# POSTECH-CVLab/PyTorch-StudioGAN

Hardware: AMD Instinct MI355X
Metric: images/sec (G+D step) BigGAN ImageNet-128 bs256 (higher is better)
Workload: dtype bf16

## Files before the change

include/sgamd.h:

```cpp
#ifndef SGAMD_H
#define SGAMD_H
#include <stdint.h>
#ifdef __cplusplus
extern "C" {
#endif

typedef void* sg_stream_t;

#define SG_DTYPE_F32 0
#define SG_DTYPE_BF16 1
#define SG_DTYPE_F64 2

#define SG_PIX_RELU 1
#define SG_PIX_UPSAMPLE 2
#define SG_PIX_QUAD 4
#define SG_PIX_TRANSPOSED 8
#define SG_EPI_OUT_F32 1
#define SG_EPI_ATOMIC 2
#define SG_EPI_POOL 4
#define SG_EPI_RELU 8
#define SG_EPI_RES_F32 16

const char* sg_last_error(void);
int sg_version(void);
int sg_prof_enable(int on);
int sg_prof_collect(double* out, int nkinds);

typedef struct {
  int dtype;
  int N, Hs, Ws, C, ldx;
  int Ho, Wo, Cout;
  int R, S, stride, pad_h, pad_w;
  int pix_flags, epi_flags;
  float alpha, beta;
  const void* x; const void* w;
  const float* bias; const void* res; const void* mask; void* out; const float* alpha_ptr;
  int ldo, ldr, ldm;
} sg_conv_fwd_desc;
int sg_conv2d_fwd(const sg_conv_fwd_desc* d, sg_stream_t stream);
int sg_set_f32_mode(int mode);
int sg_get_f32_mode(void);
long long sg_f32_split_launches(int mode);
long long sg_ew_vec_launches(void);

typedef struct {
  sg_conv_fwd_desc main;
  const void* x2; const void* w2; const float* bias2;
  int C2, ldx2, x2_up;
  float* stats;
} sg_conv_skip_desc;
int sg_conv2d_fwd_skip_stat_rows(const sg_conv_skip_desc* d);
int sg_conv2d_fwd_skip(const sg_conv_skip_desc* d, sg_stream_t stream);
int sg_conv2d_fwd_skip_ok(const sg_conv_skip_desc* d);
long long sg_conv_rs_launches(void);

typedef struct {
  sg_conv_fwd_desc conv;
  const float* pre; const float* post; const float* noise;
  long long noise_stride;
} sg_modconv_desc;
int sg_modconv2d_fwd(const sg_modconv_desc* d, sg_stream_t stream);
int sg_modconv2d_ok(const sg_modconv_desc* d);
long long sg_modconv_launches(void);
int sg_modconv_dcoef(const float* w, const float* s, float* Q, float* d, int N, int C, int Cout, int RS, sg_stream_t stream);
int sg_modconv_reduce_slabs(int P);
int sg_modconv_reduce(int dtype, const void* a, const void* b, const float* rowsub, long long rowsub_stride, const float* scale, void* out, float* part,
                      float* rowsum, int N, int P, int C, int lda, int ldb, sg_stream_t stream);

#define SG_Q_POOL 0
#define SG_Q_UP 1
typedef struct {
  int dtype, form;
  int N, Hl, Wl;
  int C, ldx, Cout;
  int pix_flags, epi_flags;
  float alpha, beta;
  const void* x; const void* wq;
  const float* bias; const void* res; const void* mask; void* out; const float* alpha_ptr;
  int ldo, ldr, ldm;
  const void* x2; const void* w2q; const float* bias2;
  int C2, ldx2;
  float* stats;
  int x2_norelu;
} sg_convq_desc;
int sg_conv2d_q_stat_rows(const sg_convq_desc* d);
int sg_conv2d_q(const sg_convq_desc* d, sg_stream_t stream);
int sg_conv2d_q_ok(const sg_convq_desc* d);
int sg_quad_pack(int dtype, int mode, const void* src, void* dst, int M, int Cs, sg_stream_t stream);
typedef struct { const void* src; void* dst; int M, Cs, mode, pad_; } sg_quad_item;
int sg_quad_pack_batch(int dtype, const sg_quad_item* items_dev, const sg_quad_item* items_host, int n, sg_stream_t stream);
typedef struct {
  int dtype, form;
  int N, Hl, Wl;
  int C, ldx, x_flags;
  int Cout, ldg;
  float alpha; const float* alpha_ptr;
  const void* x; const void* dy; float* dw; float* dbias;
  float* work; long long work_floats;
  int splits;
} sg_convq_wgrad_desc;
int sg_conv2d_q_wgrad_plan(const sg_convq_wgrad_desc* d, int* splits, long long* work_floats);
int sg_conv2d_q_wgrad(const sg_convq_wgrad_desc* d, sg_stream_t stream);
int sg_prof_collect_ex(double* out, int nkinds);
int sg_prof_collect_tags(double* out, int ntags);

typedef struct {
  int dtype;
  int N;
  int xHs, xWs, C, ldx, x_flags;
  int gHs, gWs, Cout, ldg, g_flags;
  int Ho, Wo;
  int R, S, stride, pad_h, pad_w;
  float alpha;
  const void* x; const void* dy; float* dw;
  const float* alpha_ptr;
  int splits;
// ... 319 lines not shown
```

pytorch-studiogan_amd/_lib.py:

```python
import ctypes as C
import os
import subprocess
import sys

import torch

_HERE = os.path.dirname(os.path.abspath(__file__))
LIB_PATH = os.path.join(_HERE, "libsgamd.so")
if os.environ.get("SG_LIBSGAMD"):
    LIB_PATH = os.path.abspath(os.environ["SG_LIBSGAMD"])
CSRC = os.path.join(_HERE, "csrc")

F32, BF16, F64 = 0, 1, 2
PIX_RELU, PIX_UPSAMPLE, PIX_QUAD, PIX_TRANSPOSED = 1, 2, 4, 8
Q_POOL, Q_UP = 0, 1
EPI_OUT_F32, EPI_ATOMIC, EPI_POOL, EPI_RELU, EPI_RES_F32 = 1, 2, 4, 8, 16

_vp, _i, _f, _ll = C.c_void_p, C.c_int, C.c_float, C.c_longlong


class ConvFwdDesc(C.Structure):
    _fields_ = [("dtype", _i), ("N", _i), ("Hs", _i), ("Ws", _i), ("C", _i), ("ldx", _i), ("Ho", _i), ("Wo", _i), ("Cout", _i),
                ("R", _i), ("S", _i), ("stride", _i), ("pad_h", _i), ("pad_w", _i), ("pix_flags", _i), ("epi_flags", _i),
                ("alpha", _f), ("beta", _f), ("x", _vp), ("w", _vp), ("bias", _vp), ("res", _vp), ("mask", _vp), ("out", _vp),
                ("alpha_ptr", _vp), ("ldo", _i), ("ldr", _i), ("ldm", _i)]


class ConvSkipDesc(C.Structure):
    _fields_ = [("main", ConvFwdDesc), ("x2", _vp), ("w2", _vp), ("bias2", _vp), ("C2", _i), ("ldx2", _i), ("x2_up", _i), ("stats", _vp)]


class ModConvDesc(C.Structure):
    _fields_ = [("conv", ConvFwdDesc), ("pre", _vp), ("post", _vp), ("noise", _vp), ("noise_stride", _ll)]


class ConvWgradDesc(C.Structure):
    _fields_ = [("dtype", _i), ("N", _i), ("xHs", _i), ("xWs", _i), ("C", _i), ("ldx", _i), ("x_flags", _i), ("gHs", _i), ("gWs", _i),
                ("Cout", _i), ("ldg", _i), ("g_flags", _i), ("Ho", _i), ("Wo", _i), ("R", _i), ("S", _i), ("stride", _i),
                ("pad_h", _i), ("pad_w", _i), ("alpha", _f), ("x", _vp), ("dy", _vp), ("dw", _vp), ("alpha_ptr", _vp),
                ("splits", _i), ("no_tr", _i), ("work", _vp), ("work_floats", _ll), ("dbias", _vp)]


class ConvQDesc(C.Structure):
    _fields_ = [("dtype", _i), ("form", _i), ("N", _i), ("Hl", _i), ("Wl", _i), ("C", _i), ("ldx", _i), ("Cout", _i),
                ("pix_flags", _i), ("epi_flags", _i), ("alpha", _f), ("beta", _f), ("x", _vp), ("wq", _vp), ("bias", _vp), ("res", _vp),
                ("mask", _vp), ("out", _vp), ("alpha_ptr", _vp), ("ldo", _i), ("ldr", _i), ("ldm", _i),
                ("x2", _vp), ("w2q", _vp), ("bias2", _vp), ("C2", _i), ("ldx2", _i), ("stats", _vp), ("x2_norelu", _i)]


class ConvQWgradDesc(C.Structure):
    _fields_ = [("dtype", _i), ("form", _i), ("N", _i), ("Hl", _i), ("Wl", _i), ("C", _i), ("ldx", _i), ("x_flags", _i), ("Cout", _i),
                ("ldg", _i), ("alpha", _f), ("alpha_ptr", _vp), ("x", _vp), ("dy", _vp), ("dw", _vp), ("dbias", _vp), ("work", _vp),
                ("work_floats", _ll), ("splits", _i)]


class QuadItem(C.Structure):
    _fields_ = [("src", _vp), ("dst", _vp), ("M", _i), ("Cs", _i), ("mode", _i), ("pad_", _i)]


class LinearItem(C.Structure):
    _fields_ = [("w", _vp), ("y", _vp), ("bias", _vp), ("out", _vp), ("rows", _i), ("K", _i), ("ldy", _i), ("ldo", _i)]


class LinearItemScaled(C.Structure):
    _fields_ = [("w", _vp), ("y", _vp), ("bias", _vp), ("out", _vp), ("rows", _i), ("K", _i), ("ldy", _i), ("ldo", _i),
                ("wscale", _f), ("bscale", _f), ("oscale", _f), ("pad_", _i)]


class GemmDesc(C.Structure):
    _fields_ = [("dtype", _i), ("p_form", _i), ("q_form", _i), ("I", _i), ("J", _i), ("K", _i), ("batch", _i),
                ("p", _vp), ("p_bstride", _ll), ("ldp", _i), ("q", _vp), ("q_bstride", _ll), ("ldq", _i),
                ("out", _vp), ("out_bstride", _ll), ("ldo", _i), ("bias", _vp), ("res", _vp), ("res_bstride", _ll), ("ldr", _i),
                ("beta", _f), ("alpha", _f), ("alpha_ptr", _vp), ("epi_flags", _i), ("splits", _i), ("no_tr", _i)]


class SnLayer(C.Structure):
    _fields_ = [("w", _vp), ("u", _vp), ("v", _vp), ("sigma", _vp), ("u_snap", _vp), ("v_snap", _vp), ("w_fwd", _vp), ("w_dgrad", _vp),
                ("w_f32", _vp), ("rows", _i), ("cols", _i), ("Cin", _i), ("RS", _i), ("do_power_iter", _i), ("apply_sn", _i),
                ("rows_pad", _i), ("work_off", _ll), ("trans", _i), ("dgrad_noflip", _i), ("Cin_pad", _i)]

# ... 1 lines not shown
class SnBwdLayer(C.Structure):
    _fields_ = [("dwt", _vp), ("w", _vp), ("u", _vp), ("v", _vp), ("sigma", _vp), ("dw", _vp), ("rows", _i), ("cols", _i),
                ("Cin", _i), ("RS", _i), ("natural", _i), ("apply_sn", _i), ("trans", _i), ("Cin_pad", _i)]


class AugDesc(C.Structure):
    _fields_ = [("N", _i), ("C", _i), ("H", _i), ("W", _i), ("ops", _i), ("cut_h", _i), ("cut_w", _i), ("max_t", _i), ("color", _vp), ("geom", _vp)]


AUG_BRIGHTNESS, AUG_SATURATION, AUG_CONTRAST, AUG_FLIP, AUG_TRANSLATE, AUG_TRANSLATE_REFLECT, AUG_CUTOUT = 1, 2, 4, 8, 16, 32, 64

_lib = None


def build(force=False, verbose=False):
    cmd = ["make", "-C", CSRC, "-j", str(max(2, os.cpu_count() or 2))]
    if force:
        subprocess.run(["make", "-C", CSRC, "clean"], check=True, stdout=subprocess.DEVNULL)
    res = subprocess.run(cmd, stdout=subprocess.PIPE, stderr=subprocess.STDOUT, text=True)
    if verbose or res.returncode != 0:
        sys.stderr.write(res.stdout)
    if res.returncode != 0:
        raise RuntimeError("building libsgamd.so failed")
    return LIB_PATH


_PROTOS = {
    "sg_prof_enable": [_i],
    "sg_prof_collect": [C.POINTER(C.c_double), _i],
    "sg_conv2d_fwd": [C.POINTER(ConvFwdDesc), _vp],
    "sg_conv2d_fwd_skip": [C.POINTER(ConvSkipDesc), _vp],
    "sg_conv2d_fwd_skip_ok": [C.POINTER(ConvSkipDesc)],
    "sg_conv_rs_launches": [],
    "sg_modconv2d_fwd": [C.POINTER(ModConvDesc), _vp],
    "sg_modconv2d_ok": [C.POINTER(ModConvDesc)],
    "sg_modconv_launches": [],
    "sg_modconv_dcoef": [_vp, _vp, _vp, _vp, _i, _i, _i, _i, _vp],
    "sg_modconv_reduce_slabs": [_i],
    "sg_modconv_reduce": [_i, _vp, _vp, _vp, _ll, _vp, _vp, _vp, _vp, _i, _i, _i, _i, _i, _vp],
    "sg_conv2d_q": [C.POINTER(ConvQDesc), _vp],
    "sg_conv2d_q_ok": [C.POINTER(ConvQDesc)],
    "sg_conv2d_q_stat_rows": [C.POINTER(ConvQDesc)],
    "sg_conv2d_fwd_skip_stat_rows": [C.POINTER(ConvSkipDesc)],
    "sg_bn_stats_from_tiles": [_vp, _i, _i, _vp, _vp],
    "sg_quad_pack": [_i, _i, _vp, _vp, _i, _i, _vp],
    "sg_quad_pack_batch": [_i, _vp, C.POINTER(QuadItem), _i, _vp],
    "sg_linear_group": [_vp, C.POINTER(LinearItem), _i, _i, _vp],
    "sg_linear_group_scaled": [_vp, C.POINTER(LinearItemScaled), _i, _i, _vp],
    "sg_linear_group_scaled_launches": [],
    "sg_conv2d_q_wgrad_plan": [C.POINTER(ConvQWgradDesc), C.POINTER(_i), C.POINTER(_ll)],
    "sg_conv2d_q_wgrad": [C.POINTER(ConvQWgradDesc), _vp],
    "sg_prof_collect_ex": [C.POINTER(C.c_double), _i],
    "sg_prof_collect_tags": [C.POINTER(C.c_double), _i],
    "sg_conv2d_wgrad": [C.POINTER(ConvWgradDesc), _vp],
    "sg_conv2d_wgrad_plan": [C.POINTER(ConvWgradDesc), C.POINTER(_i), C.POINTER(_ll)],
    "sg_conv2d_wgrad_fuses_bias": [C.POINTER(ConvWgradDesc)],
    "sg_gemm": [C.POINTER(GemmDesc), _vp],
    "sg_nchw_to_nhwc": [_i, _vp, _vp, _i, _i, _i, _i, _i, _vp],
    "sg_nhwc_to_nchw": [_i, _vp, _vp, _i, _i, _i, _i, _i, _i, _vp],
    "sg_nchw_grad_to_nhwc": [_i, _vp, _vp, _vp, _i, _i, _i, _i, _i, _i, _vp],
    "sg_avgpool2_fwd": [_i, _vp, _vp, _i, _i, _i, _i, _vp],
    "sg_avgpool2_bwd": [_i, _vp, _vp, _i, _i, _i, _i, _vp],
    "sg_maxpool2_fwd": [_i, _vp, _i, _vp, _i, _vp, _i, _i, _i, _i, _vp],
    "sg_maxpool2_bwd": [_i, _vp, _i, _vp, _vp, _i, _i, _i, _i, _i, _vp],
    "sg_softmax_rows": [_i, _vp, _vp, _ll, _i, _vp],
    "sg_softmax_rows_bwd": [_i, _vp, _vp, _vp, _ll, _i, _vp],
# ... 141 lines not shown
    "sg_tanh_bwd2": [_vp, _vp, _vp, _vp, _ll, _vp],
    "sg_clamp_flat": [_vp, _ll, _f, _f, _vp],
    "sg_select_rows": [_vp, _vp, _vp, _vp, _i, _ll, _vp],
    "sg_sign_count": [_vp, _i, _vp, _vp],
    "sg_reflect_pad2d_fwd": [_vp, _vp, _i, _i, _i, _i, _i, _i, _i, _vp],
    "sg_reflect_pad2d_bwd": [_vp, _vp, _i, _i, _i, _i, _i, _i, _i, _vp],
    "sg_affine_sample_fwd": [_vp, _vp, _vp, _i, _i, _i, _i, _i, _i, _vp],
    "sg_affine_sample_bwd": [_vp, _vp, _vp, _i, _i, _i, _i, _i, _i, _vp],
    "sg_color_affine": [_vp, _vp, _vp, _i, _i, _i, _i, _vp],
    "sg_fir_reflect": [_vp, _vp, _vp, _i, _i, _i, _i, _i, _i, _i, _vp],
    "sg_ada_noise_cutout": [_vp, _vp, _vp, _vp, _vp, _i, _i, _i, _i, _vp],
}


def exported_symbols():
    return sorted(list(_PROTOS.keys()) + ["sg_last_error", "sg_version"])


def lib():
    global _lib
    if _lib is None:
        if not os.path.exists(LIB_PATH):
            raise RuntimeError(
                f"{LIB_PATH} is missing: run `python -c 'import __graft_entry__ as g; g.build()'` (make -C {CSRC}). "
                "There is no CPU/eager fallback on the product path.")
        l = C.CDLL(LIB_PATH)
        l.sg_last_error.restype = C.c_char_p
        l.sg_version.restype = _i
        for name, args in _PROTOS.items():
            fn = getattr(l, name)
            fn.argtypes = args
            fn.restype = _i
        l.sg_conv_rs_launches.restype = _ll
        l.sg_modconv_launches.restype = _ll
        l.sg_tok_gemm_launches.restype = _ll
        l.sg_mha_launches.restype = _ll
        l.sg_f32_split_launches.restype = _ll
        l.sg_ew_vec_launches.restype = _ll
        l.sg_bn_path_launches.restype = _ll
        l.sg_linear_group_scaled_launches.restype = _ll
        l.sg_fir_bias_act_launches.restype = _ll
        l.sg_act_fir_launches.restype = _ll
        l.sg_mbstd_launches.restype = _ll
        f32_mode = {"bf16x3": 3, "bf16x6": 6}.get(os.environ.get("SG_F32_MODE", "exact"), 0)
        if f32_mode:
            l.sg_set_f32_mode(f32_mode)
        _lib = l
    return _lib


def check(rc, name=""):
    if rc != 0:
        raise RuntimeError(f"{name}: {lib().sg_last_error().decode()} (rc={rc})")


_STATE_WRITERS = frozenset(("sg_adam_ema", "sg_ema_lerp", "sg_allreduce_flat", "sg_clamp_flat", "sg_allgather_flat"))
write_epoch = [0]


def call(name, *args):
    if name in _STATE_WRITERS:
        write_epoch[0] += 1
    rc = getattr(lib(), name)(*args)
    if rc != 0:
        raise RuntimeError(f"{name}: {lib().sg_last_error().decode()} (rc={rc})")

# ... 33 lines not shown
```

pytorch-studiogan_amd/backbones/big_resnet.py:

```python
import torch
import torch.nn as nn

from .. import functional as F
from .. import ops
from ..bank import get_bank
from .heads import build_heads, apply_heads


def _dtype(mixed_precision):
    return torch.bfloat16 if mixed_precision else torch.float32


def _need_graph(module, *inputs):
    if not torch.is_grad_enabled():
        return False
    for t in inputs:
        if torch.is_tensor(t) and t.requires_grad:
            return True
    return any(p.requires_grad for p in module.parameters())


class GenBlock(nn.Module):
    def __init__(self, in_channels, out_channels, g_cond_mtd, affine_input_dim, MODULES):
        super().__init__()
# ... 119 lines not shown
        nxt = bank.boundaries(self.blocks) if bank.exchange is not None else None
        with ops.bump_batches_tracked(self):
            for bi, blocklist in enumerate(self.blocks):
                for block in blocklist:
                    if isinstance(block, ops.SelfAttention):
                        act = block.forward_nhwc(act, slot)
                    else:
                        act = block.forward_nhwc(act, affines[counter], slot)
                        counter += 1
                if nxt is not None:
                    act = bank.mark(act, nxt[bi])
                act = ops.block_boundary(self, bi, act)
            act = self.bn4.forward_nhwc(act, relu=True)
        act = self.conv2d5.forward_nhwc(act, slot)
        return F.NhwcToNchwFn.apply(act, True, 3)


class DiscOptBlock(nn.Module):
    def __init__(self, in_channels, out_channels, apply_d_sn, MODULES):
        super().__init__()
        self.apply_d_sn = apply_d_sn
        self.conv2d0 = MODULES.d_conv2d(in_channels=in_channels, out_channels=out_channels, kernel_size=1, stride=1, padding=0)
        self.conv2d1 = MODULES.d_conv2d(in_channels=in_channels, out_channels=out_channels, kernel_size=3, stride=1, padding=1)
        self.conv2d2 = MODULES.d_conv2d(in_channels=out_channels, out_channels=out_channels, kernel_size=3, stride=1, padding=1)
        if not apply_d_sn:
            self.bn0 = MODULES.d_bn(in_features=in_channels)
            self.bn1 = MODULES.d_bn(in_features=out_channels)
        self.activation = MODULES.d_act_fn
        self.average_pooling = nn.AvgPool2d(2)
        self.cpad = 8 if (apply_d_sn and in_channels < 8) else 0
        if self.cpad:
            self.conv2d1._sg_cin_pad = self.conv2d0._sg_cin_pad = self.cpad

    def forward_nhwc(self, x, slot):
        h = self.conv2d1.forward_nhwc(x, slot)
        if not self.apply_d_sn:
            h = self.bn1.forward_nhwc(h, relu=True)
            h = self.conv2d2.forward_nhwc(h, slot, out_pool=True)
        else:
            if self.cpad == 8 and h.dtype == torch.bfloat16 and not x.requires_grad:
                return ops.conv_skip_nhwc(self.conv2d2, self.conv2d0, h, x, slot, in_relu=True, out_pool=True, skip_relu=False)
            h = self.conv2d2.forward_nhwc(h, slot, in_relu=True, out_pool=True)
        x0 = F.AvgPool2Fn.apply(x)
        if not self.apply_d_sn:
            x0 = self.bn0.forward_nhwc(x0)
        return self.conv2d0.forward_nhwc(x0, slot, res=h)


class DiscBlock(nn.Module):
    def __init__(self, in_channels, out_channels, apply_d_sn, MODULES, downsample=True):
        super().__init__()
        self.apply_d_sn = apply_d_sn
        self.downsample = downsample
        self.activation = MODULES.d_act_fn
        self.ch_mismatch = in_channels != out_channels
        if self.ch_mismatch or downsample:
            self.conv2d0 = MODULES.d_conv2d(in_channels=in_channels, out_channels=out_channels, kernel_size=1, stride=1, padding=0)
            if not apply_d_sn:
                self.bn0 = MODULES.d_bn(in_features=in_channels)
        self.conv2d1 = MODULES.d_conv2d(in_channels=in_channels, out_channels=out_channels, kernel_size=3, stride=1, padding=1)
        self.conv2d2 = MODULES.d_conv2d(in_channels=out_channels, out_channels=out_channels, kernel_size=3, stride=1, padding=1)
        if not apply_d_sn:
            self.bn1 = MODULES.d_bn(in_features=in_channels)
            self.bn2 = MODULES.d_bn(in_features=out_channels)
        self.average_pooling = nn.AvgPool2d(2)

    def forward_nhwc(self, x, slot):
        if self.apply_d_sn:
            if self.downsample or self.ch_mismatch:
                link = F.GradLink()
                h = self.conv2d1.forward_nhwc(x, slot, in_relu=True, link=link)
                return ops.conv_skip_nhwc(self.conv2d2, self.conv2d0, h, x, slot, in_relu=True, out_pool=self.downsample, link=link)
            h = self.conv2d1.forward_nhwc(x, slot, in_relu=True)
            h = self.conv2d2.forward_nhwc(h, slot, in_relu=True, out_pool=False)
            return F.AddReluFn.apply(h, x)
        h = self.bn1.forward_nhwc(x, relu=True)
        h = self.conv2d1.forward_nhwc(h, slot)
        h = self.bn2.forward_nhwc(h, relu=True)
        h = self.conv2d2.forward_nhwc(h, slot, out_pool=self.downsample)
        if self.downsample or self.ch_mismatch:
            x0 = self.bn0.forward_nhwc(x)
            return self.conv2d0.forward_nhwc(x0, slot, out_pool=self.downsample, res=h)
        return F.AddFn.apply(h, x)


class Discriminator(nn.Module):
    def __init__(self, img_size, d_conv_dim, apply_d_sn, apply_attn, attn_d_loc, d_cond_mtd, aux_cls_type, d_embed_dim, normalize_d_embed,
                 num_classes, d_init, d_depth, mixed_precision, MODULES, MODEL):
        super().__init__()
        d_in_dims_collection = {
            "32": [3] + [d_conv_dim * 2, d_conv_dim * 2, d_conv_dim * 2],
            "64": [3] + [d_conv_dim, d_conv_dim * 2, d_conv_dim * 4, d_conv_dim * 8],
            "128": [3] + [d_conv_dim, d_conv_dim * 2, d_conv_dim * 4, d_conv_dim * 8, d_conv_dim * 16],
            "256": [3] + [d_conv_dim, d_conv_dim * 2, d_conv_dim * 4, d_conv_dim * 8, d_conv_dim * 8, d_conv_dim * 16],
            "512": [3] + [d_conv_dim, d_conv_dim, d_conv_dim * 2, d_conv_dim * 4, d_conv_dim * 8, d_conv_dim * 8, d_conv_dim * 16]
        }
        d_out_dims_collection = {
            "32": [d_conv_dim * 2, d_conv_dim * 2, d_conv_dim * 2, d_conv_dim * 2],
            "64": [d_conv_dim, d_conv_dim * 2, d_conv_dim * 4, d_conv_dim * 8, d_conv_dim * 16],
            "128": [d_conv_dim, d_conv_dim * 2, d_conv_dim * 4, d_conv_dim * 8, d_conv_dim * 16, d_conv_dim * 16],
            "256": [d_conv_dim, d_conv_dim * 2, d_conv_dim * 4, d_conv_dim * 8, d_conv_dim * 8, d_conv_dim * 16, d_conv_dim * 16],
            "512": [d_conv_dim, d_conv_dim, d_conv_dim * 2, d_conv_dim * 4, d_conv_dim * 8, d_conv_dim * 8, d_conv_dim * 16, d_conv_dim * 16]
        }
        d_down = {
            "32": [True, True, False, False],
            "64": [True, True, True, True, False],
            "128": [True, True, True, True, True, False],
            "256": [True, True, True, True, True, True, False],
            "512": [True, True, True, True, True, True, True, False]
        }
        self.d_cond_mtd = d_cond_mtd
        self.aux_cls_type = aux_cls_type
        self.normalize_d_embed = normalize_d_embed
        self.num_classes = num_classes
        self.mixed_precision = mixed_precision
        self.in_dims = d_in_dims_collection[str(img_size)]
        self.out_dims = d_out_dims_collection[str(img_size)]
        self.MODEL = MODEL
        down = d_down[str(img_size)]

        blocks = []
        for index in range(len(self.in_dims)):
            if index == 0:
                blocks += [[DiscOptBlock(in_channels=self.in_dims[index], out_channels=self.out_dims[index], apply_d_sn=apply_d_sn, MODULES=MODULES)]]
            else:
                blocks += [[DiscBlock(in_channels=self.in_dims[index], out_channels=self.out_dims[index], apply_d_sn=apply_d_sn,
                                      MODULES=MODULES, downsample=down[index])]]
            if index + 1 in attn_d_loc and apply_attn:
                blocks += [[ops.SelfAttention(self.out_dims[index], is_generator=False, MODULES=MODULES)]]
        self.blocks = nn.ModuleList([nn.ModuleList(block) for block in blocks])
        self.activation = MODULES.d_act_fn
        build_heads(self, MODULES, self.out_dims[-1], d_cond_mtd, aux_cls_type, d_embed_dim, num_classes, MODEL)
        if d_init:
            ops.init_weights(self.modules, d_init)
        ops.adopt(self, _dtype(mixed_precision))

    def forward(self, x, label, eval=False, adc_fake=False):
        dtype = self.compute_dtype
        bank = get_bank(self, dtype)
        slot = bank.begin_forward(_need_graph(self, x))
        h = ops.to_nhwc(x, dtype, self.blocks[0][0].cpad)
        nxt = bank.boundaries(self.blocks) if bank.exchange is not None else None
        for bi, blocklist in enumerate(self.blocks):
            for block in blocklist:
                h = block.forward_nhwc(h, slot)
            if nxt is not None:
                h = bank.mark(h, nxt[bi])
            h = ops.block_boundary(self, bi, h)
        hw = h.shape[1] * h.shape[2]
        h = F.ReluSumFn.apply(h)
        return apply_heads(self, h, label, slot, adc_fake, hw=hw)
```

pytorch-studiogan_amd/csrc/common.h:

```cpp
#pragma once
#include <hip/hip_runtime.h>
#include <stdint.h>
#include <type_traits>

typedef uint16_t bf16_t;
typedef __attribute__((ext_vector_type(4))) uint32_t u32x4;
typedef __attribute__((ext_vector_type(2))) uint32_t u32x2;
typedef __attribute__((ext_vector_type(4))) float f32x4;
typedef __attribute__((ext_vector_type(16))) float f32x16;
typedef __attribute__((ext_vector_type(8))) __bf16 bf16x8_t;
typedef __attribute__((ext_vector_type(4))) short s16x4;
typedef __attribute__((ext_vector_type(8))) short s16x8;

#define SG_PRIO_UP() __builtin_amdgcn_s_setprio(1)
#define SG_PRIO_DOWN() __builtin_amdgcn_s_setprio(0)

#define SG_DTYPE_F32 0
#define SG_DTYPE_BF16 1

__device__ __forceinline__ float bf2f(bf16_t v) { return __uint_as_float(((uint32_t)v) << 16); }
__device__ __forceinline__ bf16_t f2bf(float f) {
  uint32_t u = __float_as_uint(f);
  if ((u & 0x7fffffffu) > 0x7f800000u) return (bf16_t)((u >> 16) | 0x40u);
  u += 0x7fffu + ((u >> 16) & 1u);
  return (bf16_t)(u >> 16);
}

typedef __bf16 sg_bf16x2_t __attribute__((ext_vector_type(2)));
typedef float sg_f32x2_t __attribute__((ext_vector_type(2)));
__device__ __forceinline__ uint32_t pack2bf(float a, float b) {
  sg_f32x2_t v = {a, b};
  return __builtin_bit_cast(uint32_t, __builtin_convertvector(v, sg_bf16x2_t));
}

template <typename T> __device__ __forceinline__ float to_f(T v);
template <> __device__ __forceinline__ float to_f<float>(float v) { return v; }
template <> __device__ __forceinline__ float to_f<bf16_t>(bf16_t v) { return bf2f(v); }
template <typename T> __device__ __forceinline__ T from_f(float v);
template <> __device__ __forceinline__ float from_f<float>(float v) { return v; }
template <> __device__ __forceinline__ bf16_t from_f<bf16_t>(float v) { return f2bf(v); }

template <typename T> struct ET;
template <> struct ET<float> { static constexpr int VEC = 4, BK = 16; };
template <> struct ET<bf16_t> { static constexpr int VEC = 8, BK = 32; };

__device__ __forceinline__ u32x4 zero16() { u32x4 z = {0u, 0u, 0u, 0u}; return z; }

template <typename T> __device__ __forceinline__ void unpack16(u32x4 v, float* o);
template <> __device__ __forceinline__ void unpack16<float>(u32x4 v, float* o) {
#pragma unroll
  for (int i = 0; i < 4; i++) o[i] = __uint_as_float(v[i]);
}
template <> __device__ __forceinline__ void unpack16<bf16_t>(u32x4 v, float* o) {
#pragma unroll
  for (int i = 0; i < 4; i++) { o[2 * i] = __uint_as_float(v[i] << 16); o[2 * i + 1] = __uint_as_float(v[i] & 0xffff0000u); }
}
template <typename T> __device__ __forceinline__ u32x4 pack16(const float* o);
template <> __device__ __forceinline__ u32x4 pack16<float>(const float* o) {
  u32x4 v;
#pragma unroll
  for (int i = 0; i < 4; i++) v[i] = __float_as_uint(o[i]);
  return v;
}
template <> __device__ __forceinline__ u32x4 pack16<bf16_t>(const float* o) {
  u32x4 v;
#pragma unroll
  for (int i = 0; i < 4; i++) v[i] = (uint32_t)f2bf(o[2 * i]) | ((uint32_t)f2bf(o[2 * i + 1]) << 16);
  return v;
}
template <typename T, int V> using vec_t = std::conditional_t<V == 1, T, u32x4>;
// ... 117 lines not shown
```

pytorch-studiogan_amd/csrc/conv.hip:

```cpp
#include <type_traits>
#include "conv_common.h"
#include "conv_v2.h"

int g_sg_f32_mode = 0;
long long g_sg_f32_split_launches[2] = {0, 0};
extern "C" int sg_set_f32_mode(int mode) {
  SG_CHECK(mode == 0 || mode == 3 || mode == 6, "sg_set_f32_mode: 0 (exact fp32 MFMA), 3 (bf16x3 split) or 6 (bf16x6 split)");
  g_sg_f32_mode = mode;
  return 0;
}
extern "C" int sg_get_f32_mode() { return g_sg_f32_mode; }
extern "C" long long sg_f32_split_launches(int mode) {
  if (mode != 3 && mode != 6) return -1;
  return __atomic_load_n(&g_sg_f32_split_launches[mode == 6], __ATOMIC_RELAXED);
}

template <typename T, bool FAST>
static void conv_fwd_launch(const sg_conv_fwd_desc* d, const Epilogue<T>& e, int I, int J, int K, int pflags, hipStream_t st) {
  typedef StridedKC<T, FAST> LP;
  typedef ConvPixKC<T, FAST> LQ;
  LP lp;
  lp.base = (const T*)d->w; lp.bstride = 0; lp.ld = K; lp.rows = I; lp.K = K;
  lp.vec_ok = (K % ET<T>::VEC == 0) && aligned16(d->w);
  LQ lq;
  fill_geom<T>(lq.g, d->x, d->N, d->Hs, d->Ws, d->C, d->ldx, d->Ho, d->Wo, d->R, d->S, d->stride, d->pad_h, d->pad_w, pflags);
  lq.rows = J; lq.K = K;
  if constexpr (sizeof(T) == 4 && FAST) {
    const int mode = g_sg_f32_mode;
    if (mode == 3) { sg_f32_split_count(3); return conv_fwd_tiles<T, LP, LQ, 3>(lp, lq, e, I, J, K, st); }
    if (mode == 6) { sg_f32_split_count(6); return conv_fwd_tiles<T, LP, LQ, 6>(lp, lq, e, I, J, K, st); }
  }
  conv_fwd_tiles<T, LP, LQ, 0>(lp, lq, e, I, J, K, st);
}

static bool conv_fwd_v2_try(const ConvFwdProblem& pb, hipStream_t st) {
  const sg_conv_fwd_desc* d = pb.d;
  const int I = pb.I, J = pb.J, K = pb.K, pflags = pb.pflags;
  const char mode = env_mode("SG_CONV_V2");
  const bool force = mode == 'f';
  if (mode == '0' || (pflags & SG_PIX_TRANSPOSED)) return false;
  if (d->stride != 1 && (d->stride != 2 || (pflags & (SG_PIX_UPSAMPLE | SG_PIX_QUAD)))) return false;
  if (d->C % 8 || d->ldx % 8 || d->R * d->S > 25 || J < 256) return false;
  if (pb.xbytes >= (1ll << 31) || pb.wbytes >= (1ll << 30)) return false;
  if (!aligned16(d->x) || !aligned16(d->w)) return false;
// ... 41 lines not shown
  const int J = (int)Jll;
  int pflags = d->pix_flags;
  if (d->epi_flags & SG_EPI_POOL) {
    SG_CHECK((d->Ho % 2 == 0) && (d->Wo % 2 == 0), "sg_conv2d_fwd: pooled output needs even Ho, Wo");
    pflags |= SG_PIX_QUAD;
  } else {
    pflags &= ~SG_PIX_QUAD;
  }
  const bool w_vec = (K % ET<T>::VEC == 0) && aligned16(d->w);
  const bool x_vec = (d->C % ET<T>::VEC == 0) && (d->ldx % ET<T>::VEC == 0) && aligned16(d->x);
  const Epilogue<T> e = make_epilogue<T>(d, I, J);
  const int prof = sg_prof_begin(st, 2.0 * (double)I * (double)J * (double)K, 0);
  int eng = SG_ENG_CONV_GEMM;
  if constexpr (std::is_same_v<T, bf16_t>) {
    if (w_vec && x_vec) {
      const ConvFwdProblem pb = conv_fwd_problem(d, e, I, J, K, pflags);
      if (sg_conv_fwd_sk_try(pb, st)) eng = SG_ENG_CONV_SK;
      else if (sg_conv_fwd_rs_try(pb, st)) eng = SG_ENG_CONV_RS;
      else if (sg_conv_fwd_v4_try(pb, st)) eng = SG_ENG_CONV_V4;
      else if (sg_conv_fwd_v3_try(pb, st)) eng = SG_ENG_CONV_V3;
      else if (conv_fwd_v2_try(pb, st)) eng = SG_ENG_CONV_V2;
    }
  }
  if (eng == SG_ENG_CONV_GEMM) {
    if (w_vec && x_vec) conv_fwd_launch<T, true>(d, e, I, J, K, pflags, st);
    else conv_fwd_launch<T, false>(d, e, I, J, K, pflags, st);
  }
  {
    const double es = sizeof(T), jout = (d->epi_flags & SG_EPI_POOL) ? (double)J / 4.0 : (double)J;
    const double b = es * ((double)d->N * d->Hs * d->Ws * d->C + (double)I * K + jout * I * (1.0 + (d->mask ? 1.0 : 0.0) + (d->res ? 1.0 : 0.0)));
    sg_prof_tag(prof, eng, b);
  }
  sg_prof_end(st, prof);
  SG_LAUNCH_CHECK();
  return 0;
}

static int conv_fwd_skip(const sg_conv_skip_desc* sk, hipStream_t st, bool dry) {
  const sg_conv_fwd_desc* d = &sk->main;
  if (d->dtype != SG_DTYPE_BF16 || d->R != 3 || d->S != 3 || d->stride != 1 || (d->pix_flags & (SG_PIX_UPSAMPLE | SG_PIX_TRANSPOSED))) return 0;
  const int K = 9 * d->C, I = d->Cout;
  const long long Jll = (long long)d->N * d->Ho * d->Wo;
  if (Jll >= (1ll << 31) || (long long)d->N * d->Hs * d->Ws * d->ldx >= (1ll << 31)) return 0;
  const int J = (int)Jll;
  int pflags = d->pix_flags;
  if (d->epi_flags & SG_EPI_POOL) { if ((d->Ho & 1) || (d->Wo & 1)) return 0; pflags |= SG_PIX_QUAD; } else pflags &= ~SG_PIX_QUAD;
  const ConvFwdProblem pb = conv_fwd_problem(d, make_epilogue<bf16_t>(d, I, J), I, J, K, pflags);
  if (dry) return sg_conv_fwd_v4_skip_try(pb, sk, st, true) ? 1 : 0;
  const int prof = sg_prof_begin(st, 2.0 * (double)I * (double)J * ((double)K + (double)sk->C2), 0);
  const bool ok = sg_conv_fwd_v4_skip_try(pb, sk, st, false);
  {
    const double jout = (d->epi_flags & SG_EPI_POOL) ? (double)J / 4.0 : (double)J;
    const double x2 = (double)d->N * (sk->x2_up ? (d->Ho / 2) * (d->Wo / 2) : d->Ho * d->Wo) * sk->C2;
    sg_prof_tag(prof, SG_ENG_CONV_V4_SKIP, 2.0 * ((double)d->N * d->Hs * d->Ws * d->C + x2 + (double)I * (K + sk->C2) + jout * I));
  }
  sg_prof_end(st, prof);
  return ok ? 1 : 0;
}
extern "C" int sg_conv2d_fwd_skip_stat_rows(const sg_conv_skip_desc* d) {
  if (!d) return 0;
  const long long J = (long long)d->main.N * d->main.Ho * d->main.Wo;
  return (int)((J + 255) / 256);
}
extern "C" int sg_conv2d_fwd_skip_ok(const sg_conv_skip_desc* d) {
  if (!d || !d->main.x || !d->main.w || !d->main.out || !d->x2 || !d->w2) return 0;
  return conv_fwd_skip(d, nullptr, true);
}
extern "C" int sg_conv2d_fwd_skip(const sg_conv_skip_desc* d, sg_stream_t stream) {
  SG_CHECK(d && d->main.x && d->main.w && d->main.out && d->x2 && d->w2, "sg_conv2d_fwd_skip: null pointer");
  SG_CHECK(conv_fwd_skip(d, (hipStream_t)stream, false) == 1, "sg_conv2d_fwd_skip: problem not eligible for the fused kernel (ask sg_conv2d_fwd_skip_ok first)");
  SG_LAUNCH_CHECK();
  return 0;
}

extern "C" int sg_conv2d_fwd(const sg_conv_fwd_desc* d, sg_stream_t stream) {
  SG_CHECK(d && d->x && d->w && d->out, "sg_conv2d_fwd: null pointer");
  SG_CHECK(d->N > 0 && d->C > 0 && d->Cout > 0 && d->R > 0 && d->S > 0 && d->stride > 0, "sg_conv2d_fwd: bad shape");
  SG_CHECK(!(d->epi_flags & SG_EPI_ATOMIC), "sg_conv2d_fwd: atomic epilogue not supported");
  if (d->dtype == SG_DTYPE_F32) return conv_fwd_t<float>(d, (hipStream_t)stream);
  if (d->dtype == SG_DTYPE_BF16) return conv_fwd_t<bf16_t>(d, (hipStream_t)stream);
  sg_set_error("sg_conv2d_fwd: bad dtype");
  return -1;
}
```

pytorch-studiogan_amd/csrc/conv_common.h:

```cpp
#pragma once
#include <stdlib.h>
#include "gemm_core.h"
#include "../../include/sgamd.h"

static inline int ilog2_exact(int v) {
  if (v <= 0 || (v & (v - 1))) return -1;
  int s = 0;
  while ((1 << s) < v) s++;
  return s;
}
static inline bool aligned16(const void* p) { return (((uintptr_t)p) & 15) == 0; }

template <typename T>
static void fill_geom(PixGeom<T>& g, const void* x, int N, int Hs, int Ws, int C, int ldx, int Ho, int Wo, int R, int S,
                      int stride, int pad_h, int pad_w, int flags) {
  g.x = (const T*)x; g.N = N; g.Hs = Hs; g.Ws = Ws;
  const int up = (flags & SG_PIX_UPSAMPLE) ? 2 : 1;
  g.Hin = Hs * up; g.Win = Ws * up; g.C = C; g.ldx = ldx; g.Ho = Ho; g.Wo = Wo;
  g.R = R; g.S = S; g.stride = stride; g.pad_h = pad_h; g.pad_w = pad_w; g.flags = flags;
  g.vec_ok = (C % ET<T>::VEC == 0) && (ldx % ET<T>::VEC == 0) && aligned16(x);
  g.wshift = ilog2_exact(Wo); g.hshift = ilog2_exact(Ho);
}

static inline char env_mode(const char* name) { const char* m = getenv(name); return m ? m[0] : 0; }

static inline long long bf16_extent(long long npix, int ld, int C) { return ((npix - 1) * ld + C) * 2; }

template <typename D> static inline bool is_3x3_s1_p1(const D* d) { return d->R == 3 && d->S == 3 && d->stride == 1 && d->pad_h == 1 && d->pad_w == 1; }

static inline int cout_blocks(int Cout) { return Cout % 96 == 0 ? 3 : Cout % 64 == 0 ? 2 : 0; }

static const int kCoutTiles[3] = {192, 128, 96};
static inline int cout_tile_search(int I, int tj, int& best_tiles) {
  int best = 0;
  best_tiles = 0;
  for (int c = 0; c < 3; c++) {
    if (I % kCoutTiles[c]) continue;
    const int tiles = (I / kCoutTiles[c]) * tj;
    if (tiles >= 512) { best = kCoutTiles[c]; best_tiles = tiles; break; }
    if (tiles > best_tiles) { best = kCoutTiles[c]; best_tiles = tiles; }
  }
  return best;
}

template <typename T, class LP, class LQ, int SPLIT, class EPI = Epilogue<T>>
static void conv_fwd_tiles(const LP& lp, const LQ& lq, const EPI& e, int I, int J, int K, hipStream_t st) {
  if (I <= 32) sg_launch_gemm<T, LP, LQ, 32, 256, 1, 4, true, SPLIT, EPI>(lp, lq, e, I, J, K, 1, 1, st);
  else if (I % 128 != 0 && (I % 96 == 0 || (I < 128 && I > 64))) sg_launch_gemm<T, LP, LQ, 96, 256, 1, 4, true, SPLIT, EPI>(lp, lq, e, I, J, K, 1, 1, st);
  else sg_launch_gemm<T, LP, LQ, 128, 128, 2, 2, true, SPLIT, EPI>(lp, lq, e, I, J, K, 1, 1, st);
}

template <typename T, typename D> static Epilogue<T> make_epilogue(const D* d, int I, int J) {
  Epilogue<T> e;
  e.out = d->out; e.out_bstride = 0; e.ldo = d->ldo; e.bias = d->bias;
  e.res = d->res; e.res_bstride = 0; e.ldr = d->ldr; e.beta = d->beta;
  e.mask = (const T*)d->mask; e.mask_bstride = 0; e.ldm = d->ldm; e.split_stride = 0;
  e.alpha = d->alpha; e.alpha_ptr = d->alpha_ptr; e.flags = d->epi_flags; e.I = I; e.J = J;
  return e;
}
static inline bool epi_bf16_rows_ok(const Epilogue<bf16_t>& e) {
  if ((e.flags & (SG_EPI_ATOMIC | SG_EPI_OUT_F32)) || (e.ldo & 7) || !aligned16(e.out)) return false;
  if (e.mask && ((e.ldm & 7) || !aligned16(e.mask))) return false;
  if (e.res && ((e.flags & SG_EPI_RES_F32) || (e.ldr & 7) || !aligned16(e.res))) return false;
  return true;
}

struct ConvFwdProblem {
  const sg_conv_fwd_desc* d;
  Epilogue<bf16_t> e;
  int I, J, K, pflags;
  bool up, quad;
  int wshift, hshift;
  long long xbytes, wbytes;
  bool out_is_in_times_up() const { return d->Ho == d->Hs * (up ? 2 : 1) && d->Wo == d->Ws * (up ? 2 : 1); }
};
static inline ConvFwdProblem conv_fwd_problem(const sg_conv_fwd_desc* d, const Epilogue<bf16_t>& e, int I, int J, int K, int pflags) {
  ConvFwdProblem pb;
  pb.d = d; pb.e = e; pb.I = I; pb.J = J; pb.K = K; pb.pflags = pflags;
  pb.up = (pflags & SG_PIX_UPSAMPLE) != 0; pb.quad = (pflags & SG_PIX_QUAD) != 0;
  pb.wshift = ilog2_exact(d->Wo); pb.hshift = ilog2_exact(d->Ho);
  pb.xbytes = bf16_extent((long long)d->N * d->Hs * d->Ws, d->ldx, d->C); pb.wbytes = (long long)I * K * 2;
  return pb;
}

bool sg_conv_fwd_sk_try(const ConvFwdProblem& pb, hipStream_t st);
bool sg_conv_fwd_rs_try(const ConvFwdProblem& pb, hipStream_t st);
bool sg_conv_fwd_v4_try(const ConvFwdProblem& pb, hipStream_t st);
bool sg_conv_fwd_v3_try(const ConvFwdProblem& pb, hipStream_t st);
bool sg_conv_fwd_v4_skip_try(const ConvFwdProblem& pb, const sg_conv_skip_desc* sk, hipStream_t st, bool dry);
```

pytorch-studiogan_amd/csrc/conv_q.hip:

```cpp
#include "conv_common.h"
#include "conv_q.h"
#include "wgrad_q.h"

__device__ __host__ static inline int quad_pat(int pool_like, int a, int t) {
  const int P[2][2] = {{3, 4}, {1, 6}};
  const int U[2][2] = {{1, 6}, {3, 4}};
  return pool_like ? P[a][t] : U[a][t];
}
static inline bool quad_mode_pool_like(int mode) { return mode == 0 || mode == 3; }
static inline float quad_mode_scale(int mode) { return (mode == 0 || mode == 2) ? 0.25f : 1.f; }

template <typename T>
__global__ __launch_bounds__(256) void k_quad_pack(const T* src, T* dst, long long nvec, int cv, int pool_like, float scale) {
  constexpr int V = ET<T>::VEC;
  const long long i = (long long)blockIdx.x * 256 + threadIdx.x;
  if (i >= nvec) return;
  const long long m = i / cv;
  const int c = (int)(i - m * cv) * V;
  const int Cs = cv * V;
  const T* s0 = src + m * 9 * Cs + c;
  float w[9][V];
#pragma unroll
  for (int k = 0; k < 9; k++) unpack16<T>(*(const u32x4*)(s0 + (long long)k * Cs), w[k]);
  T* d0 = dst + m * 16 * Cs + c;
// ... 100 lines not shown
      }
#pragma unroll
  for (int e = 0; e < V; e++) o[e] *= scale;
  *(u32x4*)((T*)q.dst + (m * 16 + vt) * q.Cs + c) = pack16<T>(o);
}
extern "C" int sg_quad_pack_batch(int dtype, const sg_quad_item* items_dev, const sg_quad_item* items_host, int n, sg_stream_t stream) {
  SG_CHECK(items_dev && items_host && n > 0 && n <= 64, "sg_quad_pack_batch: bad arguments");
  const int V = dtype == SG_DTYPE_BF16 ? 8 : 4;
  long long blocks = 0;
  for (int i = 0; i < n; i++) {
    const sg_quad_item& q = items_host[i];
    SG_CHECK(q.src && q.dst && q.M > 0 && q.Cs > 0 && q.Cs % V == 0 && q.mode >= 0 && q.mode <= 5 && (q.mode != 5 || (q.Cs == 8 && dtype == SG_DTYPE_BF16)) && aligned16(q.src) && aligned16(q.dst), "sg_quad_pack_batch: bad item");
    blocks += ((q.mode == 5 ? (long long)q.M * 4 : (long long)q.M * (q.Cs / V) * (q.mode == 4 ? 1 : 16)) + 255) / 256;
  }
  hipStream_t st = (hipStream_t)stream;
  if (dtype == SG_DTYPE_BF16) hipLaunchKernelGGL(k_quad_pack_batch<bf16_t>, dim3((unsigned)blocks), dim3(256), 0, st, items_dev, n);
  else if (dtype == SG_DTYPE_F32) hipLaunchKernelGGL(k_quad_pack_batch<float>, dim3((unsigned)blocks), dim3(256), 0, st, items_dev, n);
  else { sg_set_error("sg_quad_pack_batch: bad dtype"); return -1; }
  SG_LAUNCH_CHECK();
  return 0;
}

static bool convq_plan(const sg_convq_desc* d, ConvQParams& p, Epilogue<bf16_t>& e, int& NB) {
  if (d->dtype != SG_DTYPE_BF16 || (d->form != SG_Q_POOL && d->form != SG_Q_UP)) return false;
  if (env_mode("SG_CONV_Q") == '0') return false;
  if (d->C < 32 || d->C % 32 || d->ldx % 8 || !aligned16(d->x) || !aligned16(d->wq)) return false;
  const int wlog = ilog2_exact(d->Wl), hlog = ilog2_exact(d->Hl);
  if (wlog < 2 || hlog < 1) return false;
  const long long J = (long long)d->N * d->Hl * d->Wl;
  const long long npix_x = d->form == SG_Q_POOL ? 4 * J : J;
  if (4 * J >= (1ll << 29)) return false;
  const long long xbytes = bf16_extent(npix_x, d->ldx, d->C), wbytes = (long long)d->Cout * 16 * d->C * 2;
  if (xbytes >= (1ll << 31) || wbytes >= (1ll << 31)) return false;
  if ((d->epi_flags & ~SG_EPI_RELU) || (d->pix_flags & ~SG_PIX_RELU)) return false;
  e = make_epilogue<bf16_t>(d, d->Cout, (int)J);
  if (!epi_bf16_rows_ok(e)) return false;
  NB = cout_blocks(d->Cout);
  if (!NB) return false;
  p.x = (const bf16_t*)d->x; p.w = (const bf16_t*)d->wq;
  p.form = d->form; p.Wl = d->Wl; p.wlog = wlog; p.hlog = hlog;
  p.C = d->C; p.ldx = d->ldx; p.I = d->Cout; p.J = (int)J; p.K = 16 * d->C; p.nslice = d->C / 32;
  {
    const int nph = d->form == SG_Q_POOL ? 1 : 4;
    const long long tiles256 = (long long)(d->Cout / (32 * NB)) * ((J + 255) / 256) * nph;
    p.bj = tiles256 < 512 ? 128 : 256;
    if (const char* bj = getenv("SG_CONV_Q_BJ")) { if (bj[0] == '1') p.bj = 128; else if (bj[0] == '2') p.bj = 256; }
  }
  p.npx = ((p.bj + 2 * d->Wl + 16) + 15) & ~15;
  p.gj = wbytes > (2ll << 20) ? 8 : 1;
  if (const char* gj = getenv("SG_CONV_Q_GJ")) { const int v = atoi(gj); if (v >= 1 && v <= 64) p.gj = v; }
  p.flags = d->pix_flags;
  p.xbytes = (unsigned)xbytes; p.wbytes = (unsigned)wbytes;
  p.wgt_off = p.zero_off = p.bias_off = 0;
  p.x2 = nullptr; p.w2 = nullptr; p.bias2 = nullptr; p.C2 = p.ldx2 = p.nslice2 = 0; p.x2bytes = p.w2bytes = 0; p.c2x8 = p.skip_norelu = 0;
  if (d->x2) {
    const bool c8 = d->C2 == 8;
    if (d->form != SG_Q_POOL || !d->w2q || (!c8 && (d->C2 < 32 || d->C2 % 32)) || d->ldx2 % 8 || !aligned16(d->x2) || !aligned16(d->w2q)) return false;
    if (d->bias2 && !d->bias) return false;
    const int c2w = c8 ? 32 : d->C2;
    const long long x2bytes = bf16_extent(4 * J, d->ldx2, d->C2), w2bytes = (long long)d->Cout * c2w * 2;
    if (x2bytes >= (1ll << 31) || w2bytes >= (1ll << 31)) return false;
    p.x2 = (const bf16_t*)d->x2; p.w2 = (const bf16_t*)d->w2q; p.bias2 = d->bias2;
    p.C2 = c2w; p.ldx2 = d->ldx2; p.nslice2 = c2w / 32; p.x2bytes = (unsigned)x2bytes; p.w2bytes = (unsigned)w2bytes;
    p.c2x8 = c8 ? 1 : 0; p.skip_norelu = d->x2_norelu ? 1 : 0;
  }
  p.stats = d->stats;
  return true;
}
extern "C" int sg_conv2d_q_ok(const sg_convq_desc* d) {
  if (!d || !d->x || !d->wq || !d->out) return 0;
  ConvQParams p; Epilogue<bf16_t> e; int NB;
  return convq_plan(d, p, e, NB) ? 1 : 0;
}
extern "C" int sg_conv2d_q_stat_rows(const sg_convq_desc* d) {
  if (!d || !d->x || !d->wq || !d->out) return 0;
  ConvQParams p; Epilogue<bf16_t> e; int NB;
  if (!convq_plan(d, p, e, NB)) return 0;
  const int sbj = p.bj > 256 ? 256 : p.bj;
  return ((p.J + sbj - 1) / sbj) * (d->form == SG_Q_POOL ? 1 : 4);
}
extern "C" int sg_conv2d_q(const sg_convq_desc* d, sg_stream_t stream) {
  SG_CHECK(d && d->x && d->wq && d->out, "sg_conv2d_q: null pointer");
  ConvQParams p; Epilogue<bf16_t> e; int NB = 0;
  SG_CHECK(convq_plan(d, p, e, NB), "sg_conv2d_q: problem not eligible for the quad kernel (ask sg_conv2d_q_ok first)");
  hipStream_t st = (hipStream_t)stream;
  const double c2 = d->x2 ? (double)d->C2 : 0.0;
  const int prof = sg_prof_begin_q(st, 2.0 * (double)d->Cout * 4.0 * (double)p.J * (9.0 * (double)d->C + c2), 0);
  sg_prof_set_executed(prof, 2.0 * (double)d->Cout * (double)p.J * (16.0 * (double)d->C + 4.0 * c2));
  const char* ev_db = getenv("SG_CONV_Q_DB");
  int db_mode = ev_db ? (ev_db[0] == '1' ? 1 : 0) : ((d->Wl == 4 && d->form == SG_Q_UP) ? 1 : 0);
  const int rc = NB == 3 ? sg_launch_conv_q<3>(p, e, db_mode, st) : sg_launch_conv_q<2>(p, e, db_mode, st);
  {
    const double J = (double)p.J, jin = d->form == SG_Q_POOL ? 4.0 * J : J, jout = d->form == SG_Q_POOL ? J : 4.0 * J;
    sg_prof_tag(prof, d->x2 ? SG_ENG_CONV_Q_SKIP : SG_ENG_CONV_Q,
                2.0 * (jin * d->C + (d->x2 ? 4.0 * J * d->C2 + (double)d->Cout * d->C2 : 0.0) + 16.0 * d->C * d->Cout + jout * d->Cout * (1.0 + (d->mask ? 1.0 : 0.0) + (d->res ? 1.0 : 0.0))));
  }
  sg_prof_end(st, prof);
  SG_CHECK(rc == 0, "sg_conv2d_q: launch failed");
  SG_LAUNCH_CHECK();
  return 0;
}

struct QPlan { bool ok; int NB, S, nci, nco, splits, nchunk; long long n, stride; };
static QPlan wgradq_plan(const sg_convq_wgrad_desc* d) {
  QPlan s; s.ok = false; s.NB = s.S = s.nci = s.nco = s.splits = s.nchunk = 0; s.n = s.stride = 0;
  if (env_mode("SG_WGRAD_Q") == '0') return s;
  if (d->dtype != SG_DTYPE_BF16 || (d->form != SG_Q_POOL && d->form != SG_Q_UP)) return s;
  if (ilog2_exact(d->Wl) < 2 || ilog2_exact(d->Hl) < 0) return s;
  if (d->Wl == 4 && (d->Hl != 4 || d->N % 4)) return s;
  if (d->Wl < 64 && d->Wl > 4 && d->Hl % (64 / d->Wl)) return s;
  if (d->C % 32 || d->ldx % 8 || d->ldg % 8 || !aligned16(d->x) || !aligned16(d->dy)) return s;
  if (d->x_flags & ~SG_PIX_RELU) return s;
  s.NB = cout_blocks(d->Cout);
  if (!s.NB) return s;
  const long long K = (long long)d->N * d->Hl * d->Wl;
  if (K % 64 || 4 * K >= (1ll << 29)) return s;
  const long long xpix = d->form == SG_Q_POOL ? 4 * K : K, gpix = d->form == SG_Q_POOL ? K : 4 * K;
  if (xpix * d->ldx * 2 >= (1ll << 31) || gpix * d->ldg * 2 >= (1ll << 31)) return s;
  s.S = (d->C % 64 == 0) ? 2 : 1;
  s.nci = d->C / (32 * s.S); s.nco = d->Cout / (32 * s.NB); s.nchunk = (int)(K / 64);
  s.n = 16ll * d->C * d->Cout;
  s.stride = s.n + (d->dbias ? 4ll * d->Cout : 0);
  const int tiles = 4 * s.nci * s.nco;
  int sp = d->splits > 0 ? d->splits : (512 >= tiles ? 512 / tiles : 1);
  const int maxs = s.nchunk / 8 > 0 ? s.nchunk / 8 : 1;
  if (sp > maxs) sp = maxs;
  if (sp > 512) sp = 512;
  s.splits = sp;
  s.ok = true;
  return s;
// ... 93 lines not shown
```

pytorch-studiogan_amd/csrc/conv_sk.h:

```cpp
#pragma once
#include "conv_v2.h"

struct ConvSkParams {
  const bf16_t* x; const bf16_t* w;
  int C, ldx, Hs, Ws;
  int Ho, Wo, wshift, hshift;
  int mode3;
  int flags;
  int I, J, K;
  unsigned xbytes;
  unsigned obytes, sbytes;
  int nrb;
};

template <int TI, int NP, int TJ, int KS, int NW, bool POOL>
__global__ __launch_bounds__(64 * NW) void sg_conv_sk_kernel(ConvSkParams p, Epilogue<bf16_t> epi) {
  constexpr int BI = TI * NP * 32;
  constexpr int NCH = 2 * KS;
  constexpr int WP = KS * 32 + 16;
  constexpr int CP = TI * 64 + 16;
  constexpr int ROWS = 32 * TJ;
  constexpr int CPR = TI * 4;
  extern __shared__ __attribute__((aligned(16))) char smem[];
  char* const wsm = smem;
  float* const sbias = (float*)(smem + BI * WP);
  const int tid = threadIdx.x, lane = tid & 63;
  const int wave = __builtin_amdgcn_readfirstlane(tid >> 6);
  char* const stg = smem + BI * WP + BI * 4 + wave * (ROWS * CP);
  const int i0 = blockIdx.y * BI;

  for (int idx = tid; idx < BI * NCH; idx += 64 * NW) {
    const int row = idx / NCH, c = idx - row * NCH;
    u32x4 v = {0u, 0u, 0u, 0u};
    if (i0 + row < p.I && c * 8 < p.K) v = *(const u32x4*)(p.w + (long long)(i0 + row) * p.K + c * 8);
    *(u32x4*)(wsm + row * WP + c * 16) = v;
  }
  for (int i = tid; i < BI; i += 64 * NW) sbias[i] = (epi.bias && i0 + i < epi.I) ? epi.bias[i0 + i] : 0.f;
  __syncthreads();

  const auto rsx = __builtin_amdgcn_make_buffer_rsrc((void*)p.x, 0, (int)p.xbytes, 0x00020000);
  const auto rso = __builtin_amdgcn_make_buffer_rsrc(epi.out, 0, (int)p.obytes, 0x00020000);
  const auto rss = __builtin_amdgcn_make_buffer_rsrc((void*)(epi.mask ? (const void*)epi.mask : epi.res), 0, (int)p.sbytes, 0x00020000);
  constexpr int NIT = ((POOL ? ROWS / 4 : ROWS) * CPR + 63) / 64;
  const int frow = lane & 31, fhi = lane >> 5;
  const unsigned ldx2 = 2u * (unsigned)p.ldx;
  const bool up = (p.flags & SG_PIX_UPSAMPLE) != 0, quad = (p.flags & SG_PIX_QUAD) != 0;
  typedef short s16x2_t __attribute__((ext_vector_type(2)));
  const short fl = (p.flags & SG_PIX_RELU) ? (short)0 : (short)-32768;
  const s16x2_t floor2 = {fl, fl};

  int ctr[KS], cts[KS];
  unsigned cdelta[KS];
  bool cok[KS];
#pragma unroll
  for (int ks = 0; ks < KS; ks++) {
    const int c = 2 * ks + fhi;
    const int tr3 = (c * 11) >> 5;
    const int ts3 = c - 3 * tr3;
    ctr[ks] = p.mode3 ? tr3 : 1;
    cts[ks] = p.mode3 ? ts3 : 1;
    cdelta[ks] = p.mode3 ? (unsigned)((tr3 - 1) * p.Ws + (ts3 - 1)) * ldx2 : (unsigned)c * 16u;
    cok[ks] = p.mode3 ? (c < 9) : (c * 8 < p.C);
  }

  auto fetch = [&](int rb, u32x4 (&q)[TJ][KS]) {
#pragma unroll
    for (int b = 0; b < TJ; b++) {
      const int row = rb * ROWS + b * 32 + frow;
      int n, ho, wo;
      if (quad) {
        const int qd = row >> 2, dy = (row >> 1) & 1, dx = row & 1;
        const int wq = qd & ((p.Wo >> 1) - 1);
        const int t = qd >> (p.wshift - 1);
        const int hq = t & ((p.Ho >> 1) - 1);
        n = t >> (p.hshift - 1);
        ho = 2 * hq + dy; wo = 2 * wq + dx;
// ... 121 lines not shown
              if (pre_mask) {
                const u32x2 m = *(const u32x2*)loc;
#pragma unroll
                for (int e = 0; e < 4; e++) { const bf16_t h = (bf16_t)((m[e >> 1] >> (16 * (e & 1))) & 0xffffu); if (!(bf2f(h) > 0.f)) v[e] = 0.f; }
              }
              if (pre_res) {
                const u32x2 r = *(const u32x2*)loc;
#pragma unroll
                for (int e = 0; e < 4; e++) { const bf16_t h = (bf16_t)((r[e >> 1] >> (16 * (e & 1))) & 0xffffu); v[e] += epi.beta * bf2f(h); }
              }
              if (relu_out) {
#pragma unroll
                for (int e = 0; e < 4; e++) v[e] = fmaxf(v[e], 0.f);
              }
              u32x2 t;
              t[0] = pack2bf(v[0], v[1]);
              t[1] = pack2bf(v[2], v[3]);
              *(u32x2*)loc = t;
            }
          }
        }
      asm volatile("s_waitcnt lgkmcnt(0)" ::: "memory");
#pragma unroll
      for (int it = 0; it < NIT; it++) {
        const int idx = lane + 64 * it;
        const int r = idx / CPR, c = idx - r * CPR;
        const int jg = jbase + r;
        const bool ok = idx < rows_out * CPR && jg < Jout && c < ncp;
        const unsigned off = ok ? ((unsigned)jg * (unsigned)epi.ldo + (unsigned)(i0 + ic0 + c * 8)) * 2u : 0x80000000u;
        const int rr = idx < rows_out * CPR ? r : 0;
        const u32x4 v = *(const u32x4*)(stg + rr * CP + c * 16);
        __builtin_amdgcn_raw_buffer_store_b128(v, rso, (int)off, 0, 0);
      }
    }
  };

  const int stride = gridDim.x * NW;
  int rb = blockIdx.x * NW + wave;
  u32x4 qa[TJ][KS], qb[TJ][KS];
  if (rb >= p.nrb) return;
  fetch(rb, qa);
#pragma unroll
  for (int it = 0; it < NP * NIT; it++) {
    const u32x4 z = {0u, 0u, 0u, 0u};
    __builtin_amdgcn_raw_buffer_store_b128(z, rso, (int)(0x80000000u + 16u * it), 0, 0);
  }
  while (true) {
    fetch(rb + stride, qb);
    compute_store(rb, qa);
    rb += stride;
    if (rb >= p.nrb) break;
    fetch(rb + stride, qa);
    compute_store(rb, qb);
    rb += stride;
    if (rb >= p.nrb) break;
  }
}

template <int TI, int NP, int TJ, int KS, bool POOL>
static inline int sg_launch_conv_sk_tp(ConvSkParams p, const Epilogue<bf16_t>& e, hipStream_t st) {
  constexpr int BI = TI * NP * 32, WP = KS * 32 + 16, CP = TI * 64 + 16, ROWS = 32 * TJ;
  constexpr int lds4 = BI * WP + BI * 4 + 4 * ROWS * CP;
  constexpr int NW = (2 * lds4 <= 160 * 1024) ? 4 : 8;
  constexpr int lds = BI * WP + BI * 4 + NW * ROWS * CP;
  static_assert(lds <= 160 * 1024, "LDS");
  static bool attr_done = false;
  if (!attr_done) {
    if (hipFuncSetAttribute((const void*)sg_conv_sk_kernel<TI, NP, TJ, KS, NW, POOL>, hipFuncAttributeMaxDynamicSharedMemorySize, lds) != hipSuccess) return -1;
    attr_done = true;
  }
  p.nrb = (p.J + ROWS - 1) / ROWS;
  const int tilesI = (p.I + BI - 1) / BI;
  int gx = (p.nrb + NW - 1) / NW;
  const int cap = (256 * (8 / NW) + tilesI - 1) / tilesI;
  if (gx > cap) gx = cap;
  hipLaunchKernelGGL((sg_conv_sk_kernel<TI, NP, TJ, KS, NW, POOL>), dim3(gx, tilesI), dim3(64 * NW), lds, st, p, e);
  return 0;
}
template <int TI, int NP, int TJ, int KS>
static inline int sg_launch_conv_sk_t(const ConvSkParams& p, const Epilogue<bf16_t>& e, hipStream_t st) {
  return (e.flags & SG_EPI_POOL) ? sg_launch_conv_sk_tp<TI, NP, TJ, KS, true>(p, e, st) : sg_launch_conv_sk_tp<TI, NP, TJ, KS, false>(p, e, st);
}

static inline int sg_launch_conv_sk(const ConvSkParams& p, const Epilogue<bf16_t>& e, hipStream_t st) {
  const int ti = p.I <= 32 ? 1 : p.I <= 64 ? 2 : p.I <= 96 ? 3 : p.I <= 128 ? 4 : 6;
  const int ks = p.K <= 16 ? 1 : p.K <= 48 ? 3 : p.K <= 96 ? 6 : 12;
#define SG_SK_CASE(T_, TI_, NP_, KS_, TJ_) if (ti == T_ && ks == KS_) return sg_launch_conv_sk_t<TI_, NP_, TJ_, KS_>(p, e, st);
  SG_SK_CASE(1, 1, 1, 1, 2) SG_SK_CASE(1, 1, 1, 3, 2) SG_SK_CASE(1, 1, 1, 6, 2) SG_SK_CASE(1, 1, 1, 12, 1)
  SG_SK_CASE(2, 2, 1, 1, 2) SG_SK_CASE(2, 2, 1, 3, 2) SG_SK_CASE(2, 2, 1, 6, 1) SG_SK_CASE(2, 2, 1, 12, 1)
  SG_SK_CASE(3, 3, 1, 1, 1) SG_SK_CASE(3, 3, 1, 3, 1) SG_SK_CASE(3, 3, 1, 6, 1) SG_SK_CASE(3, 3, 1, 12, 1)
  SG_SK_CASE(4, 2, 2, 1, 2) SG_SK_CASE(4, 2, 2, 3, 2) SG_SK_CASE(4, 2, 2, 6, 1) SG_SK_CASE(4, 2, 2, 12, 1)
  SG_SK_CASE(6, 3, 2, 1, 1) SG_SK_CASE(6, 3, 2, 3, 1) SG_SK_CASE(6, 3, 2, 6, 1) SG_SK_CASE(6, 2, 3, 12, 1)
#undef SG_SK_CASE
  return -1;
}
```

pytorch-studiogan_amd/csrc/conv_sk.hip:

```cpp
#include "conv_common.h"
#include "conv_sk.h"

bool sg_conv_fwd_sk_try(const ConvFwdProblem& pb, hipStream_t st) {
  const sg_conv_fwd_desc* d = pb.d;
  const Epilogue<bf16_t>& e = pb.e;
  const int I = pb.I, J = pb.J;
  const char mode = env_mode("SG_CONV_SK");
  if (mode == '0') return false;
  const bool force = mode == 'f';
  if (d->stride != 1 || (pb.pflags & SG_PIX_TRANSPOSED)) return false;
  const bool one = d->R == 1 && d->S == 1 && d->pad_h == 0 && d->pad_w == 0 && d->C <= 192;
  const bool stem = is_3x3_s1_p1(d) && d->C == 8 && !pb.up;
  if (!one && !stem) return false;
  if (d->C % 8 || d->ldx % 8 || I % 8 || I > 384 || !aligned16(d->x) || !aligned16(d->w)) return false;
  if (!pb.out_is_in_times_up()) return false;
  if (pb.wshift < 1 || pb.hshift < 1) return false;
  if (pb.xbytes >= (1ll << 31) || J >= (1 << 30)) return false;
  if (!epi_bf16_rows_ok(e) || (e.mask && e.res)) return false;
  if (J < 16384 && !force) return false;
  const long long jout = (e.flags & SG_EPI_POOL) ? (J >> 2) : J;
  const long long obytes = bf16_extent(jout, e.ldo, I);
  const long long sbytes = e.mask ? bf16_extent(jout, e.ldm, I) : (e.res ? bf16_extent(jout, e.ldr, I) : 16);
  if (obytes >= (1ll << 31) || sbytes >= (1ll << 31)) return false;
  ConvSkParams p;
  p.obytes = (unsigned)obytes; p.sbytes = (unsigned)sbytes;
  p.x = (const bf16_t*)d->x; p.w = (const bf16_t*)d->w;
  p.C = d->C; p.ldx = d->ldx; p.Hs = d->Hs; p.Ws = d->Ws;
  p.Ho = d->Ho; p.Wo = d->Wo; p.wshift = pb.wshift; p.hshift = pb.hshift;
  p.mode3 = stem ? 1 : 0; p.flags = pb.pflags;
  p.I = I; p.J = J; p.K = pb.K; p.xbytes = (unsigned)pb.xbytes; p.nrb = 0;
  return sg_launch_conv_sk(p, e, st) == 0;
}
```

pytorch-studiogan_amd/csrc/conv_v2.h:

```cpp
#pragma once
#include "gemm_core.h"

struct ConvV2Params {
  const bf16_t* x; const bf16_t* w;
  int N, Hs, Ws, C, ldx;
  int Hin, Win, Ho, Wo;
  int R, S, pad_h, pad_w;
  int stride;
  int flags;
  int I, J, K;
  int cpt;
  int ntap;
  unsigned xbytes, wbytes;
  int wshift, hshift;
};

typedef __attribute__((address_space(1))) const void* sg_gptr_t;
typedef __attribute__((address_space(3))) void* sg_lptr_t;

template <int BI, int BJ, int NW, int TI, int TJ, bool VMAP = false, bool NOSTORE = false>
__device__ __forceinline__ void sg_conv_epilogue(f32x16 (&acc)[TI][TJ], char* smem, const float* sbias, const Epilogue<bf16_t>& epi,
                                                 int i0, int j0, int wi0, int wj0, float al, int vlog = 0, int vadd = 0,
                                                 float* stats = nullptr, int stats_C = 0, int stats_row = 0) {
  auto grow = [&](int jg) -> long long {
    if (VMAP) return (long long)(((jg >> vlog) << (vlog + 2)) + ((jg & ((1 << vlog) - 1)) << 1) + vadd);
    return (long long)jg;
  };
  const int tid = threadIdx.x, lane = tid & 63;
  const bool pool = (epi.flags & SG_EPI_POOL) != 0;
  constexpr int CP = BI * 2 + 16;
  __syncthreads();
  const int rows_out = pool ? BJ / 4 : BJ;
  const int jbase = pool ? (j0 >> 2) : j0, Jout = pool ? (epi.J >> 2) : epi.J;
  constexpr int CPR = BI / 8;
  const bool pre_mask = epi.mask != nullptr, pre_res = epi.res != nullptr;
  const bool pre_both = pre_mask && pre_res;
  const int ncr = ((epi.I - i0 < BI ? epi.I - i0 : BI) + 7) >> 3;
  auto stage_tile = [&](const bf16_t* src, int ld) {
    for (int idx = tid; idx < rows_out * CPR; idx += 64 * NW) {
      const int r = idx / CPR, c = idx - r * CPR;
      const int jg = jbase + r;
      u32x4 t = {0u, 0u, 0u, 0u};
      if (jg < Jout && c < ncr) t = *(const u32x4*)(src + grow(jg) * ld + i0 + c * 8);
      *(u32x4*)(smem + r * CP + c * 16) = t;
    }
  };
  uint32_t mbits[TI * TJ];
#pragma unroll
  for (int q = 0; q < TI * TJ; q++) mbits[q] = 0u;
  if (pre_both) {
    stage_tile(epi.mask, epi.ldm);
    __syncthreads();
#pragma unroll
    for (int ta = 0; ta < TI; ta++)
#pragma unroll
      for (int tb = 0; tb < TJ; tb++) {
        const int jl = wj0 + tb * 32 + (lane & 31);
        const int jo = pool ? (jl >> 2) : jl;
        uint32_t bits = 0u;
#pragma unroll
        for (int g4 = 0; g4 < 4; g4++) {
          const int il = wi0 + ta * 32 + 8 * g4 + 4 * (lane >> 5);
          const u32x2 m = *(const u32x2*)(smem + jo * CP + il * 2);
#pragma unroll
          for (int e = 0; e < 4; e++) { const bf16_t h = (bf16_t)((m[e >> 1] >> (16 * (e & 1))) & 0xffffu); if (bf2f(h) > 0.f) bits |= 1u << (4 * g4 + e); }
        }
        mbits[ta * TJ + tb] = bits;
      }
    __syncthreads();
    stage_tile((const bf16_t*)epi.res, epi.ldr);
    __syncthreads();
  } else if (pre_mask || pre_res) {
    stage_tile(pre_mask ? epi.mask : (const bf16_t*)epi.res, pre_mask ? epi.ldm : epi.ldr);
    __syncthreads();
  }
  const bool relu_out = (epi.flags & SG_EPI_RELU) != 0;
#pragma unroll
  for (int ta = 0; ta < TI; ta++)
#pragma unroll
    for (int tb = 0; tb < TJ; tb++) {
      const int jl = wj0 + tb * 32 + (lane & 31);
#pragma unroll
      for (int g4 = 0; g4 < 4; g4++) {
        const int il = wi0 + ta * 32 + 8 * g4 + 4 * (lane >> 5);
        float v[4] = {acc[ta][tb][4 * g4 + 0], acc[ta][tb][4 * g4 + 1], acc[ta][tb][4 * g4 + 2], acc[ta][tb][4 * g4 + 3]};
        if (pool) {
#pragma unroll
          for (int e = 0; e < 4; e++) v[e] = quad_sum(v[e]);
        }
        const int jo = pool ? (jl >> 2) : jl;
        const bool act = (!pool || (lane & 3) == 0) && (jbase + jo < Jout);
        if (act) {
          char* loc = smem + jo * CP + il * 2;
#pragma unroll
          for (int e = 0; e < 4; e++) v[e] *= al;
          if (epi.bias) {
            const f32x4 b = *(const f32x4*)(sbias + il);
#pragma unroll
            for (int e = 0; e < 4; e++) v[e] += b[e];
          }
          if (pre_both) {
            const uint32_t bits = mbits[ta * TJ + tb] >> (4 * g4);
#pragma unroll
            for (int e = 0; e < 4; e++) if (!((bits >> e) & 1u)) v[e] = 0.f;
          } else if (pre_mask) {
            const u32x2 m = *(const u32x2*)loc;
#pragma unroll
            for (int e = 0; e < 4; e++) { const bf16_t h = (bf16_t)((m[e >> 1] >> (16 * (e & 1))) & 0xffffu); if (!(bf2f(h) > 0.f)) v[e] = 0.f; }
          }
          if (pre_res) {
            const u32x2 r = *(const u32x2*)loc;
#pragma unroll
            for (int e = 0; e < 4; e++) { const bf16_t h = (bf16_t)((r[e >> 1] >> (16 * (e & 1))) & 0xffffu); v[e] += epi.beta * bf2f(h); }
          }
          if (relu_out) {
#pragma unroll
            for (int e = 0; e < 4; e++) v[e] = fmaxf(v[e], 0.f);
          }
          u32x2 t;
          t[0] = pack2bf(v[0], v[1]);
          t[1] = pack2bf(v[2], v[3]);
          *(u32x2*)loc = t;
        }
      }
    }
  __syncthreads();
  if (stats) {
    constexpr int PWV = BI / 2 / NW, RG = 64 / PWV;
    const int wv = tid >> 6, pl = lane % PWV, rg = lane / PWV;
    int rows_valid = Jout - jbase;
    if (rows_valid > rows_out) rows_valid = rows_out;
    float s1a = 0.f, s2a = 0.f, s1b = 0.f, s2b = 0.f;
    const int c2 = wv * PWV + pl;
    if (rg < RG) {
      constexpr int NIT = (BJ + RG - 1) / RG;
      const char* base = smem + rg * CP + c2 * 4;
#pragma unroll 8
      for (int k = 0; k < NIT; k++) {
        const int r = rg + k * RG;
        uint32_t v = *(const uint32_t*)(base + (r < BJ ? k * (RG * CP) : 0));
        v = r < rows_valid ? v : 0u;
        const float a = __uint_as_float(v << 16), b = __uint_as_float(v & 0xffff0000u);
        s1a += a; s2a += a * a; s1b += b; s2b += b * b;
      }
    }
    float t1a = s1a, t2a = s2a, t1b = s1b, t2b = s2b;
#pragma unroll
    for (int k = 1; k < RG; k++) {
      t1a += __shfl(s1a, lane + k * PWV, 64); t2a += __shfl(s2a, lane + k * PWV, 64);
      t1b += __shfl(s1b, lane + k * PWV, 64); t2b += __shfl(s2b, lane + k * PWV, 64);
    }
    const int c = i0 + 2 * c2;
    if (rg == 0 && c < epi.I) {
      f32x4 o4 = {t1a, t2a, t1b, t2b};
      *(f32x4*)(stats + ((long long)stats_row * stats_C + c) * 2) = o4;
    }
  }
  {
    bf16_t* o = (bf16_t*)epi.out;
    for (int idx = tid; idx < rows_out * CPR; idx += 64 * NW) {
      const int r = idx / CPR, c = idx - r * CPR;
      const int jg = jbase + r;
      if (NOSTORE) {
        const u32x4 v = *(const u32x4*)(smem + r * CP + c * 16);
        if (v[0] == 0x12345678u && v[1] == 0x9abcdef0u) *(u32x4*)(o + grow(jg) * epi.ldo + i0 + c * 8) = v;
      } else if (jg < Jout && c < ncr) *(u32x4*)(o + grow(jg) * epi.ldo + i0 + c * 8) = *(const u32x4*)(smem + r * CP + c * 16);
    }
  }
}

template <int BI, int WJ, int WI, int BJ, int SCHED, bool RELU, bool UP>
__global__ __launch_bounds__(64 * WJ * WI) void sg_conv_v2_kernel(ConvV2Params p, Epilogue<bf16_t> epi, int tilesI, int tilesJ) {
  constexpr int NW = WJ * WI;
  constexpr int QB = BJ * 128, PB = BI * 128, BUF = QB + PB;
  constexpr int NQ = BJ / 8 / NW;
  constexpr int NPI = (BI / 8 + NW - 1) / NW;
  constexpr int TJ = BJ / WJ / 32, TI = BI / WI / 32;
  static_assert(NW == 8 || NW == 4, "4 or 8 waves");
  static_assert(BJ % (8 * NW) == 0, "pixel tile / DMA groups");
  static_assert(BJ % (WJ * 32) == 0 && BI % (WI * 32) == 0, "tile/wave mismatch");
  extern __shared__ __attribute__((aligned(16))) char smem[];

  const int tid = threadIdx.x, lane = tid & 63;
  const int wave = __builtin_amdgcn_readfirstlane(tid >> 6);
  const int bid = sg_xcd_tile(blockIdx.x, tilesI * tilesJ);
  const int tI = bid % tilesI, tJ = bid / tilesI;
  const int i0 = tI * BI, j0 = tJ * BJ;
  float* sbias = (float*)(smem + 2 * BUF);
  if (epi.bias) {
    for (int i = tid; i < BI; i += 64 * NW) sbias[i] = (i0 + i < epi.I) ? epi.bias[i0 + i] : 0.f;
  }

  const auto rsx = __builtin_amdgcn_make_buffer_rsrc((void*)p.x, 0, (int)p.xbytes, 0x00020000);
  const auto rsw = __builtin_amdgcn_make_buffer_rsrc((void*)p.w, 0, (int)p.wbytes, 0x00020000);
  const int sub = lane >> 3;
  const int lc = (lane & 7) ^ ((4 * wave + (lane >> 4)) & 7);
  const unsigned ldx2 = 2u * (unsigned)p.ldx;
  unsigned qoff[NQ];
  unsigned qinv[NQ];
  bool qph[NQ], qpw[NQ];
#pragma unroll
// ... 219 lines not shown
```

pytorch-studiogan_amd/csrc/conv_v3.h:

```cpp
#pragma once
#include <type_traits>
#include "halo_tile.h"

struct ConvV3Params {
  const bf16_t* x; const bf16_t* w;
  int W;
  int wlog;
  int C, ldx;
  int Ho, Wo, wshift, hshift;
  int flags;
  int I, J, K;
  int nslice;
  int npix_src;
  int npx;
  unsigned xbytes, wbytes;
  int zero_off, bias_off;
  int dump_off;
  int pm4, psh;
};

template <int BI, int WJ, int WI, int BJ, bool RELU, bool UP, bool PB2, bool W3 = false, int NKL = 0>
__global__ __launch_bounds__(64 * WJ * WI) void sg_conv_v3_kernel(ConvV3Params p, Epilogue<bf16_t> epi, int tilesI, int tilesJ) {
  static_assert(!W3 || PB2, "W3 needs the double patch buffer");
  constexpr int NW = WJ * WI;
// ... 168 lines not shown
              if (ks == 0 && a * TJ + b < NPI + 2) {
                __builtin_amdgcn_sched_barrier(0);
                dma_piece(a * TJ + b);
                __builtin_amdgcn_sched_barrier(0);
              }
            }
          if (ks == 0) {
#pragma unroll
            for (int k = TI * TJ; k < NPI + 2; k++) dma_piece(k);
          }
        }
        __builtin_amdgcn_sched_barrier(0);
      }
      if constexpr (W3) {
        if (t < 8) { tap_addresses(f, t + 1, poff_cur); load(f, 0, 0, pbufs + ((t + 1) % 3) * PB); }
        else if (next_slice) { tap_addresses(f, 0, poff_nxt); load(f, 0, 0, pbufs); }
      }
      __syncthreads();
    }
    if (!PB2 && next_slice) {
      for (int i = 0; i < npw; i++) patch_piece(0, s + 1, i, true);
      __syncthreads();
    }
  };
  if constexpr (NKL == 4) {
    for (int s = 0; s < nslice; s++) run_slice(s, std::integral_constant<int, 4>{});
  } else {
    for (int s = 0; s + 1 < nslice; s++) run_slice(s, std::integral_constant<int, 4>{});
    run_slice(nslice - 1, std::integral_constant<int, NKL>{});
  }

  float al = epi.alpha;
  if (epi.alpha_ptr) al *= *epi.alpha_ptr;
  sg_conv_epilogue<BI, BJ, NW, TI, TJ>(acc, smem, sbias, epi, i0, j0, wi0, wj0, al);
}

static inline int sg_conv_v3_lds(int BI, int BJ, int npx, bool pb2, bool w3 = false, int* zero_off = nullptr, int* bias_off = nullptr, int* dump_off = nullptr) {
  int body = (pb2 ? 2 : 1) * npx * 128 + (w3 ? 3 : 2) * BI * 128;
  const int stage = BJ * (BI * 2 + 16);
  if (stage > body) body = stage;
  if (zero_off) *zero_off = body;
  if (bias_off) *bias_off = body + 128;
  if (dump_off) *dump_off = body + 128 + BI * 4;
  const int lds = body + 128 + BI * 4 + 1024;
  return lds <= 160 * 1024 ? lds : -1;
}
template <int BI, int WJ, int WI, int BJ, bool RELU, bool UP, bool PB2, bool W3, int NKL>
static inline int sg_launch_conv_v3r(ConvV3Params p, const Epilogue<bf16_t>& e, hipStream_t st) {
  const int lds = sg_conv_v3_lds(BI, BJ, p.npx, PB2, W3, &p.zero_off, &p.bias_off, &p.dump_off);
  if (lds < 0) return -1;
  static bool attr_done = false;
  if (!ht_allow_lds(attr_done, sg_conv_v3_kernel<BI, WJ, WI, BJ, RELU, UP, PB2, W3, NKL>, 160 * 1024)) return -1;
  const int tilesI = (p.I + BI - 1) / BI, tilesJ = (p.J + BJ - 1) / BJ;
  hipLaunchKernelGGL((sg_conv_v3_kernel<BI, WJ, WI, BJ, RELU, UP, PB2, W3, NKL>), dim3(tilesI * tilesJ), dim3(64 * WJ * WI), lds, st, p, e, tilesI, tilesJ);
  return 0;
}
template <int BI, int WJ, int WI, int BJ, int NKL>
static inline int sg_launch_conv_v3(const ConvV3Params& p, const Epilogue<bf16_t>& e, hipStream_t st) {
  const bool up = (p.flags & SG_PIX_UPSAMPLE) != 0, relu = (p.flags & SG_PIX_RELU) != 0;
  const bool pb2 = p.nslice > 1 && sg_conv_v3_lds(BI, BJ, p.npx, true) > 0;
  if (!pb2 && sg_conv_v3_lds(BI, BJ, p.npx, false) < 0) return -1;
  if constexpr (BJ == 256 && (BI == 192 || BI == 128)) {
    if (pb2 && sg_conv_v3_lds(BI, BJ, p.npx, true, true) > 0 && (((p.npx >> 3) + WJ * WI - 1) / (WJ * WI) + 7) / 8 <= 2) {
      if (relu) return up ? sg_launch_conv_v3r<BI, WJ, WI, BJ, true, true, true, true, NKL>(p, e, st) : sg_launch_conv_v3r<BI, WJ, WI, BJ, true, false, true, true, NKL>(p, e, st);
      return up ? sg_launch_conv_v3r<BI, WJ, WI, BJ, false, true, true, true, NKL>(p, e, st) : sg_launch_conv_v3r<BI, WJ, WI, BJ, false, false, true, true, NKL>(p, e, st);
    }
  }
// ... 15 lines not shown
```

pytorch-studiogan_amd/csrc/conv_wgrad.hip:

```cpp
#include <type_traits>
#include "conv_common.h"
#include "wgrad_v2.h"
#include "wgrad_sk.h"
#include "wgrad_v3.h"

static bool wgrad_bf16_ok(const sg_conv_wgrad_desc* d) {
  if (d->dtype != SG_DTYPE_BF16 || d->stride != 1 || d->no_tr) return false;
  if ((d->x_flags | d->g_flags) & SG_PIX_TRANSPOSED) return false;
  return (long long)d->N * d->xHs * d->xWs * d->ldx * 2 < (1ll << 31) && (long long)d->N * d->gHs * d->gWs * d->ldg * 2 < (1ll << 31);
}
static inline unsigned wgrad_xbytes(const sg_conv_wgrad_desc* d) { return (unsigned)bf16_extent((long long)d->N * d->xHs * d->xWs, d->ldx, d->C); }
static inline unsigned wgrad_gbytes(const sg_conv_wgrad_desc* d) { return (unsigned)bf16_extent((long long)d->N * d->gHs * d->gWs, d->ldg, d->Cout); }

struct SkPlan { bool ok, taps; int NI, NJ, swap, nw; long long n; };
static SkPlan wgrad_sk_plan(const sg_conv_wgrad_desc* d) {
  SkPlan s; s.ok = false; s.taps = false; s.NI = s.NJ = s.swap = s.nw = 0; s.n = 0;
  if (env_mode("SG_WGRAD_SK") == '0' || !wgrad_bf16_ok(d)) return s;
  if (ilog2_exact(d->Wo) < 0 || ilog2_exact(d->Ho) < 0) return s;
  if (d->C % 8 || d->ldx % 8 || d->Cout % 8 || d->ldg % 8 || !aligned16(d->x) || !aligned16(d->dy)) return s;
  const long long K = (long long)d->N * d->Ho * d->Wo;
  if (K % 32 || K / 32 >= (1ll << 30)) return s;
  const bool xup = d->x_flags & SG_PIX_UPSAMPLE, gup = d->g_flags & SG_PIX_UPSAMPLE, xrelu = d->x_flags & SG_PIX_RELU;
  if (d->R == 1 && d->S == 1 && d->pad_h == 0 && d->pad_w == 0) {
    if (d->C > 192 || d->Cout > 96) return s;
// ... 250 lines not shown
  if constexpr (sizeof(T) == 4 && FAST) {
    const int mode = g_sg_f32_mode;
    if (mode == 3) { sg_f32_split_count(3); return conv_wgrad_tiles<T, LM, TR, 3>(lp, lq, e, I, J, K, BI, BJ, splits, st); }
    if (mode == 6) { sg_f32_split_count(6); return conv_wgrad_tiles<T, LM, TR, 6>(lp, lq, e, I, J, K, BI, BJ, splits, st); }
  }
  conv_wgrad_tiles<T, LM, TR, 0>(lp, lq, e, I, J, K, BI, BJ, splits, st);
}

template <typename T> static double wgrad_alg_bytes(const sg_conv_wgrad_desc* d) {
  return sizeof(T) * ((double)d->N * d->xHs * d->xWs * d->C + (double)d->N * d->gHs * d->gWs * d->Cout) + 8.0 * (double)d->R * d->S * d->C * d->Cout;
}
template <typename T, bool TR> static int conv_wgrad_t(const sg_conv_wgrad_desc* d, hipStream_t st) {
  const int I = d->R * d->S * d->C;
  const int J = d->Cout;
  const long long Kll = (long long)d->N * d->Ho * d->Wo;
  SG_CHECK(Kll < (1ll << 31), "sg_conv2d_wgrad: too many pixels");
  SG_CHECK((long long)d->N * d->xHs * d->xWs * d->ldx < (1ll << 31) && (long long)d->N * d->gHs * d->gWs * d->ldg < (1ll << 31),
           "sg_conv2d_wgrad: tensor too large for 32-bit element offsets");
  const int K = (int)Kll;
  const WgradChoice c = wgrad_choose(d, true);
  const int prof = sg_prof_begin(st, 2.0 * (double)I * (double)J * (double)K, 1);
  int eng = SG_ENG_WGRAD_GEMM;
  bool two_stage = true;
  if (c.engine == WG_SK) {
    if (wgrad_sk_launch(d, c.sk, st) != 0) { sg_set_error("sg_conv2d_wgrad: streaming kernel launch failed"); return -2; }
    eng = SG_ENG_WGRAD_SK;
  } else if (c.engine == WG_V3) {
    if (wgrad_v3_launch(d, c.v3, st) != 0) { sg_set_error("sg_conv2d_wgrad: halo kernel launch failed"); return -2; }
    eng = SG_ENG_WGRAD_V3;
  } else {
    two_stage = c.work_floats > 0 && d->work && d->work_floats >= c.work_floats;
    Epilogue<T> e;
    e.out = d->dw; e.out_bstride = 0; e.ldo = I; e.bias = nullptr; e.res = nullptr; e.res_bstride = 0; e.ldr = 0; e.beta = 0.f;
    e.mask = nullptr; e.mask_bstride = 0; e.ldm = 0; e.alpha = d->alpha; e.alpha_ptr = d->alpha_ptr; e.split_stride = 0;
    e.flags = SG_EPI_OUT_F32; e.I = I; e.J = J;
    if (c.splits == 1) { e.res = d->dw; e.ldr = I; e.beta = 1.f; e.flags |= SG_EPI_RES_F32; }
    else if (two_stage) { e.out = d->work; e.split_stride = c.n; }
    else e.flags |= SG_EPI_ATOMIC;
    if constexpr (std::is_same_v<T, bf16_t>) {
      if (c.engine == WG_V2 && wgrad_v2_launch(d, e, I, J, K, c.splits, st) == 0) eng = SG_ENG_WGRAD_V2;
    }
    if (eng == SG_ENG_WGRAD_GEMM) {
      const bool fast = (d->C % ET<T>::VEC == 0) && (d->ldx % ET<T>::VEC == 0) && aligned16(d->x) &&
                        (d->Cout % ET<T>::VEC == 0) && (d->ldg % ET<T>::VEC == 0) && aligned16(d->dy);
      if (fast) conv_wgrad_launch<T, TR, true>(d, e, I, J, K, c.BI, c.BJ, c.splits, st);
      else conv_wgrad_launch<T, TR, false>(d, e, I, J, K, c.BI, c.BJ, c.splits, st);
    }
  }
  if (two_stage) {
    splitk_reduce_launch((const float*)d->work, d->dw, c.splits, c.n, c.stride, c.fuses_bias ? d->dbias : nullptr, c.fuses_bias ? d->Cout : 0, st);
  }
  sg_prof_tag(prof, eng, wgrad_alg_bytes<T>(d));
  sg_prof_end(st, prof);
  SG_LAUNCH_CHECK();
  return 0;
}

extern "C" int sg_conv2d_wgrad(const sg_conv_wgrad_desc* d, sg_stream_t stream) {
  SG_CHECK(d && d->x && d->dy && d->dw, "sg_conv2d_wgrad: null pointer");
  SG_CHECK(d->N > 0 && d->C > 0 && d->Cout > 0 && d->R > 0 && d->S > 0 && d->stride > 0, "sg_conv2d_wgrad: bad shape");
  if (d->dtype == SG_DTYPE_F32) return conv_wgrad_t<float, true>(d, (hipStream_t)stream);
  if (d->dtype == SG_DTYPE_BF16) {
    if (d->no_tr) return conv_wgrad_t<bf16_t, false>(d, (hipStream_t)stream);
    return conv_wgrad_t<bf16_t, true>(d, (hipStream_t)stream);
  }
  sg_set_error("sg_conv2d_wgrad: bad dtype");
  return -1;
// ... 2 lines not shown
```

pytorch-studiogan_amd/csrc/gemm.hip:

```cpp
#include "gemm_core.h"
#include "../../include/sgamd.h"

static inline bool aligned16(const void* p) { return (((uintptr_t)p) & 15) == 0; }

template <typename T, class LP, class LQ, bool TR, int SPLIT>
static void gemm_tiles(const LP& lp, const LQ& lq, const Epilogue<T>& e, int I, int J, int K, int splits, int batch, hipStream_t st) {
  if (I <= 32) sg_launch_gemm<T, LP, LQ, 32, 256, 1, 4, TR, SPLIT>(lp, lq, e, I, J, K, splits, batch, st);
  else if (I % 128 != 0 && (I % 96 == 0 || (I < 128 && I > 64))) sg_launch_gemm<T, LP, LQ, 96, 256, 1, 4, TR, SPLIT>(lp, lq, e, I, J, K, splits, batch, st);
  else sg_launch_gemm<T, LP, LQ, 128, 128, 2, 2, TR, SPLIT>(lp, lq, e, I, J, K, splits, batch, st);
}

template <typename T, class LP, class LQ, bool TR, bool FAST>
static int gemm_launch(const LP& lp, const LQ& lq, const Epilogue<T>& e, const sg_gemm_desc* d, hipStream_t st) {
  const int I = d->I, J = d->J, K = d->K;
  const int splits = d->splits > 1 ? d->splits : 1;
  const int prof = sg_prof_begin(st, 2.0 * (double)I * (double)J * (double)K * (double)d->batch, 2);
  const int mode = (sizeof(T) == 4 && FAST && g_sg_f32_mode == 6) ? 6 : 0;
  if (mode == 6) {
    if constexpr (sizeof(T) == 4 && FAST) { sg_f32_split_count(6); gemm_tiles<T, LP, LQ, TR, 6>(lp, lq, e, I, J, K, splits, d->batch, st); }
  } else {
    gemm_tiles<T, LP, LQ, TR, 0>(lp, lq, e, I, J, K, splits, d->batch, st);
  }
  sg_prof_end(st, prof);
  SG_LAUNCH_CHECK();
// ... 1 lines not shown
}

template <typename T, bool F> static void fill_kc(StridedKC<T, F>& l, const void* p, long long bs, int ld, int rows, int K) {
  l.base = (const T*)p; l.bstride = bs; l.ld = ld; l.rows = rows; l.K = K;
  l.vec_ok = (K % ET<T>::VEC == 0) && (ld % ET<T>::VEC == 0) && (bs % ET<T>::VEC == 0) && aligned16(p);
}
template <typename T, bool F> static void fill_mc(StridedMC<T, F>& l, const void* p, long long bs, int ld, int rows, int K) {
  l.base = (const T*)p; l.bstride = bs; l.ld = ld; l.rows = rows; l.K = K;
  l.vec_ok = (rows % ET<T>::VEC == 0) && (ld % ET<T>::VEC == 0) && (bs % ET<T>::VEC == 0) && aligned16(p);
}

template <typename T, bool TR, bool FAST> static int gemm_forms(const Epilogue<T>& e, const sg_gemm_desc* d, hipStream_t st) {
  typedef StridedKC<T, FAST> KCL;
  typedef StridedMC<T, FAST> MCL;
  if (d->p_form == 0 && d->q_form == 0) {
    KCL lp, lq; fill_kc<T>(lp, d->p, d->p_bstride, d->ldp, d->I, d->K); fill_kc<T>(lq, d->q, d->q_bstride, d->ldq, d->J, d->K);
    return gemm_launch<T, KCL, KCL, TR, FAST>(lp, lq, e, d, st);
  } else if (d->p_form == 0 && d->q_form == 1) {
    KCL lp; MCL lq; fill_kc<T>(lp, d->p, d->p_bstride, d->ldp, d->I, d->K); fill_mc<T>(lq, d->q, d->q_bstride, d->ldq, d->J, d->K);
    return gemm_launch<T, KCL, MCL, TR, FAST>(lp, lq, e, d, st);
  } else if (d->p_form == 1 && d->q_form == 0) {
    MCL lp; KCL lq; fill_mc<T>(lp, d->p, d->p_bstride, d->ldp, d->I, d->K); fill_kc<T>(lq, d->q, d->q_bstride, d->ldq, d->J, d->K);
    return gemm_launch<T, MCL, KCL, TR, FAST>(lp, lq, e, d, st);
  } else {
    MCL lp, lq; fill_mc<T>(lp, d->p, d->p_bstride, d->ldp, d->I, d->K); fill_mc<T>(lq, d->q, d->q_bstride, d->ldq, d->J, d->K);
    return gemm_launch<T, MCL, MCL, TR, FAST>(lp, lq, e, d, st);
  }
}

template <typename T, bool TR> static int gemm_t(const sg_gemm_desc* d, hipStream_t st) {
  Epilogue<T> e;
  e.out = d->out; e.out_bstride = d->out_bstride; e.ldo = d->ldo; e.bias = d->bias;
  e.res = d->res; e.res_bstride = d->res_bstride; e.ldr = d->ldr; e.beta = d->beta;
  e.mask = nullptr; e.mask_bstride = 0; e.ldm = 0; e.split_stride = 0;
  e.alpha = d->alpha; e.alpha_ptr = d->alpha_ptr; e.flags = d->epi_flags; e.I = d->I; e.J = d->J;
  if (d->splits > 1) SG_CHECK(d->epi_flags & SG_EPI_ATOMIC, "sg_gemm: split-K needs the atomic epilogue");
  const int V = ET<T>::VEC;
  auto vec = [&](int form, const void* p, long long bs, int ld, int rows) {
    const bool common = (ld % V == 0) && (bs % V == 0) && aligned16(p);
    return common && (form == 0 ? (d->K % V == 0) : (rows % V == 0));
  };
  if (vec(d->p_form, d->p, d->p_bstride, d->ldp, d->I) && vec(d->q_form, d->q, d->q_bstride, d->ldq, d->J))
    return gemm_forms<T, TR, true>(e, d, st);
  return gemm_forms<T, TR, false>(e, d, st);
}

extern "C" int sg_gemm(const sg_gemm_desc* d, sg_stream_t stream) {
  SG_CHECK(d && d->p && d->q && d->out, "sg_gemm: null pointer");
  SG_CHECK(d->I > 0 && d->J > 0 && d->K > 0 && d->batch > 0, "sg_gemm: bad shape");
  SG_CHECK((d->p_form | d->q_form | 1) == 1, "sg_gemm: operand form must be 0 (KC) or 1 (MC)");
  SG_CHECK(!(d->epi_flags & SG_EPI_POOL), "sg_gemm: pooling epilogue is convolution-only");
  if (d->dtype == SG_DTYPE_F32) return gemm_t<float, true>(d, (hipStream_t)stream);
  if (d->dtype == SG_DTYPE_BF16) {
    if (d->no_tr) return gemm_t<bf16_t, false>(d, (hipStream_t)stream);
    return gemm_t<bf16_t, true>(d, (hipStream_t)stream);
  }
  sg_set_error("sg_gemm: bad dtype");
  return -1;
}
```

pytorch-studiogan_amd/csrc/gemm_core.h:

```cpp
#pragma once
#include "common.h"

#define SG_KC_STRIDE 80

__host__ __device__ constexpr int sg_mc_stride(int B, int es) {
  int s = B * es;
  if (es == 2) {
    while ((s % 128) != 64) s += 16;
    return s;
  }
  return s + 16;
}

template <typename T> __device__ __forceinline__ void set_elem(u32x4& v, int e, T x);
template <> __device__ __forceinline__ void set_elem<float>(u32x4& v, int e, float x) { v[e] = __float_as_uint(x); }
template <> __device__ __forceinline__ void set_elem<bf16_t>(u32x4& v, int e, bf16_t x) {
  v[e >> 1] |= ((uint32_t)x) << (16 * (e & 1));
}

template <typename T, bool FAST = false> struct StridedKC {
  static constexpr bool KC = true;
  static constexpr int VEC = ET<T>::VEC, BK = ET<T>::BK;
  const T* base; long long bstride; int ld; int rows; int K; int vec_ok;
  struct Chunk { const T* p; int k; bool valid; };
// ... 164 lines not shown
    int n, ho, wo;
    if (FAST || g.vec_ok) {
      const bool inb = ch.valid & (ch.pix < K);
      g.pix_decompose(inb ? ch.pix : 0, n, ho, wo);
      bool ok;
      const unsigned off = g.tap_off(n, ho, wo, ch.r, ch.s, ok);
      ok = ok & inb;
      const u32x4 t = *(const u32x4*)(g.x + (ok ? off + (unsigned)ch.c : 0u));
      v = ok ? t : v;
    } else if constexpr (!FAST) {
      if (!ch.valid || ch.pix >= K) return v;
      g.pix_decompose(ch.pix, n, ho, wo);
      int r = ch.r, s = ch.s, c = ch.c;
#pragma unroll
      for (int e = 0; e < VEC; e++) {
        if (r < g.R) {
          const T* p;
          if (g.tap(n, ho, wo, r, s, p)) set_elem<T>(v, e, p[c]);
        }
        c++; if (c == g.C) { c = 0; s++; if (s == g.S) { s = 0; r++; } }
      }
    }
    if (g.flags & SG_PIX_RELU) v = relu16<T>(v);
    return v;
  }
  __device__ __forceinline__ void advance(Chunk& ch) const { ch.pix += BK; }
};

#define SG_EPI_OUT_F32 1
#define SG_EPI_ATOMIC 2
#define SG_EPI_POOL 4
#define SG_EPI_RELU 8
#define SG_EPI_RES_F32 16

template <typename T> struct Epilogue {
  void* out; long long out_bstride; int ldo;
  const float* bias;
  const void* res; long long res_bstride; int ldr; float beta;
  const T* mask; long long mask_bstride; int ldm;
  float alpha; const float* alpha_ptr;
  int flags; int I; int J;
  long long split_stride;

  __device__ __forceinline__ void set_batch(int b) {
    if (flags & (SG_EPI_OUT_F32 | SG_EPI_ATOMIC)) out = (float*)out + (long long)b * out_bstride;
    else out = (T*)out + (long long)b * out_bstride;
    if (res) {
      if (flags & SG_EPI_RES_F32) res = (const float*)res + (long long)b * res_bstride;
      else res = (const T*)res + (long long)b * res_bstride;
    }
    if (mask) mask += (long long)b * mask_bstride;
  }

  __device__ __forceinline__ void store(int j, int i0, float v[4], float a) const {
    if (prep(j, i0, v, a)) write(j, i0, v);
  }
  __device__ __forceinline__ bool prep(int& j, int i0, float v[4], float a) const {
    const int lane = threadIdx.x & 63;
    if (flags & SG_EPI_POOL) {
#pragma unroll
      for (int e = 0; e < 4; e++) v[e] = quad_sum(v[e]);
      if (lane & 3) return false;
      j >>= 2;
    }
    const int Jout = (flags & SG_EPI_POOL) ? (J >> 2) : J;
    if (j >= Jout || i0 >= I) return false;
    const int ne = (I - i0) < 4 ? (I - i0) : 4;
#pragma unroll
    for (int e = 0; e < 4; e++) {
      float x = v[e] * a;
      if (bias && e < ne) x += bias[i0 + e];
      v[e] = x;
    }
    if (mask) {
      const T* m = mask + (long long)j * ldm + i0;
// ... 356 lines not shown
```

pytorch-studiogan_amd/functional/_base.py:

```python
import os

import torch
import torch.distributed as dist

from .. import _lib as L
from .. import comm as _comm
from ..bank import ensure_grad


_SECOND_ORDER = [0]
_SECOND_ORDER_LIFTS = ("act_fir", "conv2d_resample", "minibatch_std")


class second_order:

    def __enter__(self):
        _SECOND_ORDER[0] += 1
        return self

    def __exit__(self, *exc):
        _SECOND_ORDER[0] -= 1
        return False


# ... 43 lines not shown
    step = (nbytes + 255) & ~255
    if ent is None or ent[1] + step > _ZERO_POOL_BYTES:
        ent = _ZERO_POOL[key] = [torch.zeros(_ZERO_POOL_BYTES, dtype=torch.uint8, device=device), 0]
    off = ent[1]
    ent[1] = off + step
    return ent[0][off:off + nbytes].view(dtype).view(shape)


def zeros_like_small(t):
    return zeros_small(tuple(t.shape), t.dtype, t.device)


_SEQ = [0]
_STATS_OFFER = [None]
_BN_FUSED_STATS = [os.environ.get("SG_BN_FUSED_STATS", "1") != "0"]
_CBN_MERGED = [os.environ.get("SG_CBN_MERGED", "1") != "0"]


def _tick():
    _SEQ[0] += 1


def _offer_stats(out, st, rows, C):
    _STATS_OFFER[0] = (_SEQ[0], out.data_ptr(), tuple(out.shape), st, rows, C, out._version)


def _take_stats(x):
    ent, _STATS_OFFER[0] = _STATS_OFFER[0], None
    if ent is None or ent[0] != _SEQ[0] - 1 or ent[1] != x.data_ptr() or ent[2] != tuple(x.shape) or ent[5] != x.shape[3] or ent[6] != x._version:
        return None
    return ent[3], ent[4]


class f32_mode:
    MODES = {"exact": 0, "bf16x3": 3, "bf16x6": 6}

    def __init__(self, mode):
        if mode not in self.MODES:
            raise ValueError(f"f32_mode: {mode!r} (one of {sorted(self.MODES)})")
        self.mode = self.MODES[mode]

    def __enter__(self):
        self.saved = L.lib().sg_get_f32_mode()
        L.call("sg_set_f32_mode", self.mode)
        return self

    def __exit__(self, *exc):
        L.call("sg_set_f32_mode", self.saved)
        return False


def conv2d_raw(x, w_ptr, Cin, Cout, R, S, stride=1, pad_h=0, pad_w=0, pix_flags=0, epi_flags=0, bias=None, res=None, mask=None,
               alpha=1.0, beta=1.0, alpha_ptr=None, out=None, ldx=None, transposed_out_hw=None, out_coff=0, x_coff=0, desc=None):
    N, Hs, Ws = x.shape[0], x.shape[1], x.shape[2]
    ldx = x.shape[3] if ldx is None else ldx
    up = 2 if (pix_flags & L.PIX_UPSAMPLE) else 1
    Hin, Win = Hs * up, Ws * up
    if pix_flags & L.PIX_TRANSPOSED:
        Ho, Wo = transposed_out_hw
    else:
        Ho = (Hin + 2 * pad_h - R) // stride + 1
        Wo = (Win + 2 * pad_w - S) // stride + 1
    pool = bool(epi_flags & L.EPI_POOL)
    Hy, Wy = (Ho // 2, Wo // 2) if pool else (Ho, Wo)
    if out is None:
        odt = torch.float32 if (epi_flags & L.EPI_OUT_F32) else x.dtype
        out = torch.empty((N, Hy, Wy, Cout), dtype=odt, device=x.device)
    d = desc if desc is not None else L.ConvFwdDesc()
    d.dtype = L.dt(x)
    d.N, d.Hs, d.Ws, d.C, d.ldx = N, Hs, Ws, Cin, ldx
    d.Ho, d.Wo, d.Cout = Ho, Wo, Cout
    d.R, d.S, d.stride, d.pad_h, d.pad_w = R, S, stride, pad_h, pad_w
    d.pix_flags, d.epi_flags = pix_flags, epi_flags
    d.alpha, d.beta = alpha, beta
    d.x, d.w = L.ptr(x) + x_coff * x.element_size(), w_ptr
    d.bias = L.ptr(bias)
    d.res = L.ptr(res)
    d.mask = L.ptr(mask)
    d.out = L.ptr(out) + out_coff * out.element_size()
    d.alpha_ptr = L.ptr(alpha_ptr)
    d.ldo = out.shape[-1]
    d.ldr = res.shape[-1] if res is not None else 0
    d.ldm = mask.shape[-1] if mask is not None else 0
    if desc is not None:
        return out
    L.call("sg_conv2d_fwd", d, L.stream())
    return out


def conv2d_skip_raw(x, w_ptr, Cin, Cout, x2, w2_ptr, C2, x2_up=False, pix_flags=0, epi_flags=0, bias=None, bias2=None, alpha=1.0, dry=False, stats=False):
    sk = L.ConvSkipDesc()
    out = conv2d_raw(x, w_ptr, Cin, Cout, 3, 3, 1, 1, 1, pix_flags, epi_flags, bias=bias, alpha=alpha, desc=sk.main)
    sk.x2, sk.w2, sk.bias2 = L.ptr(x2), w2_ptr, L.ptr(bias2)
    sk.C2, sk.ldx2, sk.x2_up = C2, x2.shape[3], 1 if x2_up else 0
    if L.lib().sg_conv2d_fwd_skip_ok(L.C.byref(sk)) != 1:
        return None
    if dry:
        return out
    if stats and not (epi_flags & L.EPI_POOL):
        rows = L.lib().sg_conv2d_fwd_skip_stat_rows(L.C.byref(sk))
        st = torch.empty((rows, Cout, 2), dtype=torch.float32, device=x.device)
        sk.stats = st.data_ptr()
        L.call("sg_conv2d_fwd_skip", sk, L.stream())
        _offer_stats(out, st, rows, Cout)
        return out
    L.call("sg_conv2d_fwd_skip", sk, L.stream())
    return out


def conv2d_wgrad_raw(x, dy, dw_ptr, Cin, Cout, R, S, Ho, Wo, stride=1, pad_h=0, pad_w=0, x_flags=0, g_flags=0, alpha=1.0,
                     alpha_ptr=None, splits=0, no_tr=0, ldg=None, dy_coff=0, dbias=None):
    d = L.ConvWgradDesc()
    d.dtype = L.dt(x)
    d.N = x.shape[0]
    d.xHs, d.xWs, d.C, d.ldx, d.x_flags = x.shape[1], x.shape[2], Cin, x.shape[3], x_flags
    d.gHs, d.gWs, d.Cout, d.ldg, d.g_flags = dy.shape[1], dy.shape[2], Cout, (dy.shape[3] if ldg is None else ldg), g_flags
    d.Ho, d.Wo = Ho, Wo
    d.R, d.S, d.stride, d.pad_h, d.pad_w = R, S, stride, pad_h, pad_w
    d.alpha = alpha
    d.x, d.dy, d.dw = L.ptr(x), L.ptr(dy) + dy_coff * dy.element_size(), dw_ptr
    d.alpha_ptr = L.ptr(alpha_ptr)
    d.splits, d.no_tr = splits, no_tr
    fused = False
    if dbias is not None:
        d.dbias = L.ptr(dbias)
        fused = L.lib().sg_conv2d_wgrad_fuses_bias(L.C.byref(d)) == 1
        if not fused:
            d.dbias = None
    sp, wf = L.C.c_int(0), L.C.c_longlong(0)
    L.call("sg_conv2d_wgrad_plan", d, L.C.byref(sp), L.C.byref(wf))
    work = None
    if wf.value > 0:
        work = torch.empty(wf.value, dtype=torch.float32, device=x.device)
        d.splits, d.work, d.work_floats = sp.value, work.data_ptr(), wf.value
    L.call("sg_conv2d_wgrad", d, L.stream())
    return fused


def quad_pack_raw(src_ptr, dst, mode, M, Cs):
    L.call("sg_quad_pack", L.dt(dst), mode, src_ptr, L.ptr(dst), M, Cs, L.stream())
    return dst


def conv2d_q_raw(x, wq_ptr, form, Cin, Cout, pix_flags=0, epi_flags=0, bias=None, res=None, mask=None, alpha=1.0, beta=1.0, dry=False,
                 x2=None, w2q_ptr=None, bias2=None, stats=False, x2_norelu=False):
    N = x.shape[0]
    if form == L.Q_POOL:
        if x.shape[1] % 2 or x.shape[2] % 2:
            return None
        Hl, Wl = x.shape[1] // 2, x.shape[2] // 2
        oshape = (N, Hl, Wl, Cout)
    else:
        Hl, Wl = x.shape[1], x.shape[2]
        oshape = (N, 2 * Hl, 2 * Wl, Cout)
    if x.dtype != torch.bfloat16:
        return None
    d = L.ConvQDesc()
    d.dtype, d.form = L.dt(x), form
    d.N, d.Hl, d.Wl, d.C, d.ldx, d.Cout = N, Hl, Wl, Cin, x.shape[3], Cout
    d.pix_flags, d.epi_flags, d.alpha, d.beta = pix_flags, epi_flags, alpha, beta
    out = torch.empty(oshape, dtype=x.dtype, device=x.device)
    d.x, d.wq, d.bias, d.res, d.mask, d.out = L.ptr(x), wq_ptr, L.ptr(bias), L.ptr(res), L.ptr(mask), L.ptr(out)
    d.ldo = Cout
    d.ldr = res.shape[-1] if res is not None else 0
    d.ldm = mask.shape[-1] if mask is not None else 0
    if x2 is not None:
        d.x2, d.w2q, d.bias2, d.C2, d.ldx2 = L.ptr(x2), w2q_ptr, L.ptr(bias2), x2.shape[3], x2.shape[3]
        d.x2_norelu = 1 if x2_norelu else 0
    if L.lib().sg_conv2d_q_ok(L.C.byref(d)) != 1:
        return None
    if not dry:
        st = None
        if stats:
            rows = L.lib().sg_conv2d_q_stat_rows(L.C.byref(d))
            st = torch.empty((rows, Cout, 2), dtype=torch.float32, device=x.device)
            d.stats = st.data_ptr()
        L.call("sg_conv2d_q", d, L.stream())
        if st is not None:
            _offer_stats(out, st, rows, Cout)
    return out


def conv2d_q_wgrad_raw(x, dy, dw_ptr, form, Cin, Cout, x_flags=0, alpha=1.0, dbias=None, splits=0):
    if x.dtype != torch.bfloat16:
        return False
    d = L.ConvQWgradDesc()
    d.dtype, d.form = L.dt(x), form
    lo = dy if form == L.Q_POOL else x
    d.N, d.Hl, d.Wl = lo.shape[0], lo.shape[1], lo.shape[2]
    d.C, d.ldx, d.x_flags, d.Cout, d.ldg = Cin, x.shape[3], x_flags, Cout, dy.shape[3]
    d.alpha = alpha
    d.x, d.dy, d.dw, d.dbias = L.ptr(x), L.ptr(dy), dw_ptr, L.ptr(dbias)
    d.splits = splits
    sp, wf = L.C.c_int(0), L.C.c_longlong(0)
    L.call("sg_conv2d_q_wgrad_plan", d, L.C.byref(sp), L.C.byref(wf))
    if sp.value == 0:
        return False
    work = torch.empty(wf.value, dtype=torch.float32, device=x.device)
    d.work, d.work_floats, d.splits = work.data_ptr(), wf.value, sp.value
    L.call("sg_conv2d_q_wgrad", d, L.stream())
    return True


def gemm_raw(dtype, p, p_form, ldp, q, q_form, ldq, out, ldo, I, J, K, batch=1, p_bs=0, q_bs=0, out_bs=0, bias=None, res=None,
             res_bs=0, ldr=0, beta=1.0, alpha=1.0, alpha_ptr=None, epi_flags=0, splits=1, no_tr=0):
    d = L.GemmDesc()
    d.dtype, d.p_form, d.q_form = dtype, p_form, q_form
    d.I, d.J, d.K, d.batch = I, J, K, batch
    d.p = p if isinstance(p, int) else L.ptr(p)
    d.q = q if isinstance(q, int) else L.ptr(q)
    d.out = out if isinstance(out, int) else L.ptr(out)
    d.p_bstride, d.ldp, d.q_bstride, d.ldq, d.out_bstride, d.ldo = p_bs, ldp, q_bs, ldq, out_bs, ldo
    d.bias = bias if (bias is None or isinstance(bias, int)) else L.ptr(bias)
    d.res = res if (res is None or isinstance(res, int)) else L.ptr(res)
    d.res_bstride, d.ldr, d.beta = res_bs, ldr, beta
    d.alpha = alpha
    d.alpha_ptr = L.ptr(alpha_ptr)
    d.epi_flags, d.splits, d.no_tr = epi_flags, splits, no_tr
    L.call("sg_gemm", d, L.stream())


_DGRAD_SPLITK = [os.environ.get("SG_DGRAD_SPLITK", "1") != "0"]


def gemm_dgrad_rows(w_ptr, dy, dx, B, K, O):
    S = 1
    tiles = ((K + 127) // 128) * ((B + 127) // 128)
    if _DGRAD_SPLITK[0] and tiles < 64:
        while S < 32 and tiles * S < 256 and O % (2 * S) == 0 and O // (2 * S) >= 96:
            S *= 2
    if S == 1:
        gemm_raw(L.F32, w_ptr, 1, K, dy, 0, dy.shape[1] if torch.is_tensor(dy) else O, dx, K, K, B, O)
        return dx
    ldq = dy.shape[1]
    ws = torch.empty((S, B, K), dtype=torch.float32, device=dx.device)
    gemm_raw(L.F32, w_ptr, 1, K, dy, 0, ldq, ws, K, K, B, O // S, batch=S, p_bs=(O // S) * K, q_bs=O // S, out_bs=B * K)
    torch.sum(ws, dim=0, out=dx)
    return dx


__all__ = ['L', 'zeros_small', 'zeros_like_small', '_BN_FUSED_STATS', '_CBN_MERGED', '_DGRAD_SPLITK', '_SEQ', '_STATS_OFFER', '_c', '_comm', '_first_order_only', '_offer_stats', '_param_grad_wanted', '_take_stats', '_tick', 'conv2d_q_raw', 'conv2d_q_wgrad_raw', 'conv2d_raw', 'conv2d_skip_raw', 'conv2d_wgrad_raw', 'dist', 'ensure_grad', 'f32_mode', 'gemm_dgrad_rows', 'gemm_raw', 'os', 'quad_pack_raw', 'second_order', 'torch']
```

pytorch-studiogan_amd/functional/conv.py:

```python
import ctypes

from ._base import *

class ConvCfg:
    __slots__ = ("R", "S", "stride", "pad_h", "pad_w", "in_relu", "in_upsample", "out_pool", "stats")

    def __init__(self, R, S, stride=1, pad_h=0, pad_w=0, in_relu=False, in_upsample=False, out_pool=False, stats=False):
        self.R, self.S, self.stride, self.pad_h, self.pad_w = R, S, stride, pad_h, pad_w
        self.in_relu, self.in_upsample, self.out_pool = in_relu, in_upsample, out_pool
        self.stats = stats

    def out_hw(self, Hs, Ws):
        up = 2 if self.in_upsample else 1
        return (Hs * up + 2 * self.pad_h - self.R) // self.stride + 1, (Ws * up + 2 * self.pad_w - self.S) // self.stride + 1

    def pix_flags(self):
        return (L.PIX_RELU if self.in_relu else 0) | (L.PIX_UPSAMPLE if self.in_upsample else 0)

    def epi_flags(self):
        return L.EPI_POOL if self.out_pool else 0

    @property
    def scale(self):
        return 0.25 if self.out_pool else 1.0


class GradLink:
    __slots__ = ("dx", "chain", "pending")

    def __init__(self, chain=False):
        self.dx = None
        self.chain = chain
        self.pending = 0

    def take(self):
        t, self.dx = self.dx, None
        return t


_GRAD_LINK = [os.environ.get("SG_GRAD_LINK", "1") != "0"]


_QUAD = [os.environ.get("SG_QUAD", "1") != "0"]


def _quad_form(rt, cfg, x):
    if not _QUAD[0] or x.dtype != torch.bfloat16 or cfg.R != 3 or cfg.S != 3 or cfg.stride != 1 or cfg.pad_h != 1 or cfg.pad_w != 1:
        return None
    if cfg.out_pool == cfg.in_upsample or rt.trans or rt.RS != 9:
        return None
    if rt.cin_pad % 32 or (rt.rows_pad % 64 and rt.rows_pad % 96):
        return None
    return L.Q_POOL if cfg.out_pool else L.Q_UP


def _conv_fwd(x, rt, slot, cfg, bias, res=None, stats=False):
    bank = rt.bank()
    Cin = x.shape[3]
    form = _quad_form(rt, cfg, x)
    if form is not None:
        y = conv2d_q_raw(x, bank.w_quad(slot, rt, form), form, Cin, rt.rows_pad, L.PIX_RELU if cfg.in_relu else 0, 0, bias=bias, res=res,
                         stats=stats and _BN_FUSED_STATS[0] and rt.rows_pad == rt.rows)
        if y is not None:
            return y
    return conv2d_raw(x, bank.w_fwd(slot, rt), Cin, rt.rows_pad, cfg.R, cfg.S, cfg.stride, cfg.pad_h, cfg.pad_w, cfg.pix_flags(), cfg.epi_flags(),
                      bias=bias, res=res, alpha=cfg.scale)


def _conv_wgrad(x, dy, rt, slot, cfg, dbias=None):
    bank = rt.bank()
    N, Hs, Ws, Cin = x.shape
    form = _quad_form(rt, cfg, x)
    if form is not None and conv2d_q_wgrad_raw(x, dy, bank.dwt(slot, rt), form, Cin, rt.rows_pad, L.PIX_RELU if cfg.in_relu else 0, dbias=dbias):
        return dbias is not None
    Ho, Wo = cfg.out_hw(Hs, Ws)
    return conv2d_wgrad_raw(x, dy, bank.dwt(slot, rt), Cin, rt.rows_pad, cfg.R, cfg.S, Ho, Wo, cfg.stride, cfg.pad_h, cfg.pad_w, cfg.pix_flags(),
                            L.PIX_UPSAMPLE if cfg.out_pool else 0, alpha=cfg.scale, dbias=dbias)


def _conv_dgrad(dy, x, rt, slot, cfg, res=None):
    bank = rt.bank()
    N, Hs, Ws, Cin = x.shape
    form = _quad_form(rt, cfg, x)
    if form is not None and dy.shape[3] == rt.rows_pad:
        dx = conv2d_q_raw(dy, bank.w_quad(slot, rt, 2 + form), 1 - form, rt.rows_pad, Cin, 0, 0, mask=x if cfg.in_relu else None, res=res)
        if dx is not None:
            return dx
    up = 2 if cfg.in_upsample else 1
    Hin, Win = Hs * up, Ws * up
    pool = cfg.out_pool
    if cfg.stride != 1:
        assert not (pool or cfg.in_upsample), "upsample / pooling fusion is stride-1 only"
        return conv2d_raw(dy, bank.w_dgrad(slot, rt), rt.rows_pad, Cin, cfg.R, cfg.S, cfg.stride, cfg.pad_h, cfg.pad_w, L.PIX_TRANSPOSED, 0,
                          mask=x if cfg.in_relu else None, res=res, transposed_out_hw=(Hin, Win), ldx=dy.shape[3])
    pf = L.PIX_UPSAMPLE if pool else 0
    ef = L.EPI_POOL if cfg.in_upsample else 0
    return conv2d_raw(dy, bank.w_dgrad(slot, rt), rt.rows_pad, Cin, cfg.R, cfg.S, 1, cfg.R - 1 - cfg.pad_h, cfg.S - 1 - cfg.pad_w, pf, ef,
                      mask=x if cfg.in_relu else None, res=res, alpha=cfg.scale, ldx=dy.shape[3])


class ConvDgradFn(torch.autograd.Function):

    @staticmethod
    def forward(ctx, dy, x, weight, rt, slot, cfg):
        dy = _c(dy)
        ctx.save_for_backward(dy, x)
        ctx.rt, ctx.slot, ctx.cfg = rt, slot, cfg
        return _conv_dgrad(dy, x, rt, slot, cfg)

    @staticmethod
    def backward(ctx, ddx):
        dy, x = ctx.saved_tensors
        rt, slot, cfg = ctx.rt, ctx.slot, ctx.cfg
        bank = rt.bank()
        t = _c(ddx)
        if cfg.in_relu:
            m = torch.empty_like(t)
            L.call("sg_relu_mask", L.dt(t), L.ptr(t), L.ptr(x), L.ptr(m), t.numel(), L.stream())
            t = m
        N, Hs, Ws, Cin = x.shape
        Ho, Wo = cfg.out_hw(Hs, Ws)
        g_dy = None
        if ctx.needs_input_grad[0]:
            g_dy = conv2d_raw(t, bank.w_fwd(slot, rt), Cin, rt.rows_pad, cfg.R, cfg.S, cfg.stride, cfg.pad_h, cfg.pad_w,
                              L.PIX_UPSAMPLE if cfg.in_upsample else 0, cfg.epi_flags(), alpha=cfg.scale)
        if ctx.needs_input_grad[2]:
            conv2d_wgrad_raw(t, dy, bank.dwt(slot, rt), Cin, rt.rows_pad, cfg.R, cfg.S, Ho, Wo, cfg.stride, cfg.pad_h, cfg.pad_w,
                             L.PIX_UPSAMPLE if cfg.in_upsample else 0, L.PIX_UPSAMPLE if cfg.out_pool else 0, alpha=cfg.scale)
        return g_dy, None, None, None, None, None


class ConvFn(torch.autograd.Function):

    @staticmethod
    def forward(ctx, x, weight, bias, res, rt, slot, cfg, link=None):
        bank = rt.bank()
        x = _c(x)
        N, Hs, Ws, Cin = x.shape
        assert Cin == rt.cin_pad, f"conv input channels {Cin} != {rt.cin_pad}"
        ctx.link = link
        if link is not None and link.chain:
            link.pending += 1
        if res is not None:
            res = _c(res)
        bias_k = bias
        if bias is not None and rt.rows_pad != rt.rows:
            bias_k = zeros_small(rt.rows_pad, torch.float32, x.device)
            bias_k[:rt.rows].copy_(bias.detach())
        _tick()
        y = _conv_fwd(x, rt, slot, cfg, bias_k, res, stats=cfg.stats)
        ctx.save_for_backward(x)
        ctx.rt, ctx.slot, ctx.cfg = rt, slot, cfg
        ctx.bias = bias
        ctx.weight = weight
        ctx.has_res = res is not None
        return y

    @staticmethod
    def backward(ctx, dy):
        (x,) = ctx.saved_tensors
        rt, slot, cfg = ctx.rt, ctx.slot, ctx.cfg
        bank = rt.bank()
        if torch.is_grad_enabled():
            if _param_grad_wanted(ctx.weight, ctx.bias):
                raise NotImplementedError("create_graph=True is supported for input gradients only (WGAN-GP path)")
            dx = ConvDgradFn.apply(dy, x, ctx.weight, rt, slot, cfg) if ctx.needs_input_grad[0] else None
            return dx, None, None, (dy if ctx.has_res else None), None, None, None, None
        dy = _c(dy)
        dx = None
        skip_dx = ctx.link.take() if ctx.link is not None else None
        if ctx.needs_input_grad[0]:
            dx = _conv_dgrad(dy, x, rt, slot, cfg, res=skip_dx)
        elif skip_dx is not None:
            raise RuntimeError("GradLink: a skip gradient was handed over but this convolution's input needs no gradient")
        if ctx.link is not None and ctx.link.chain:
            ctx.link.pending -= 1
            if ctx.link.pending > 0 and dx is not None:
                ctx.link.dx, dx = dx, None
        want_db = ctx.bias is not None and ctx.needs_input_grad[2]
        db_done = False
        if ctx.needs_input_grad[1]:
            g = ensure_grad(ctx.bias) if (want_db and rt.rows_pad == rt.rows) else None
            db_done = _conv_wgrad(x, dy, rt, slot, cfg, dbias=g)
        if want_db and not db_done:
            g = ensure_grad(ctx.bias)
            rows = dy.shape[0] * dy.shape[1] * dy.shape[2]
            L.call("sg_colsum", L.dt(dy), L.ptr(dy), dy.shape[3], None, 0, rows, rt.rows, L.ptr(g), 1.0, L.stream())
        dres = dy if ctx.has_res else None
        return dx, None, None, dres, None, None, None, None


class ConvSkipFn(torch.autograd.Function):

    @staticmethod
    def forward(ctx, h, x, w2, b2, w0, b0, rt2, rt0, slot, cfg2, cfg0, link=None):
        bank = rt2.bank()
        ctx.link = link
        h, x = _c(h), _c(x)
        _tick()
        assert cfg2.R == 3 and cfg0.R == 1 and cfg2.out_pool == cfg0.out_pool and not cfg2.in_upsample and (cfg0.in_relu == cfg2.in_relu or not cfg0.in_relu)
        pf, ef, al = cfg2.pix_flags(), cfg2.epi_flags(), cfg2.scale
        same_relu = cfg0.in_relu == cfg2.in_relu
        y = None
        plain = rt2.rows_pad == rt2.rows and rt0.rows_pad == rt0.rows and b2 is not None and b0 is not None
        if plain and same_relu and h.dtype == torch.bfloat16 and _SKIP_FUSION[0] and (h.shape[1] >= 16 or _SKIP_FUSION[0] == "all") and _quad_form(rt2, cfg2, h) is None:
            y = conv2d_skip_raw(h, bank.w_fwd(slot, rt2), h.shape[3], rt2.rows, x, bank.w_fwd(slot, rt0), x.shape[3], cfg0.in_upsample, pf, ef,
                                bias=b2, bias2=b0, alpha=al, stats=cfg2.stats and _BN_FUSED_STATS[0])
        if y is None and plain and _quad_form(rt2, cfg2, h) == L.Q_POOL and _SKIP_FUSION[0] and (rt0.cin_pad % 32 == 0 or rt0.cin_pad == 8) and not cfg0.in_upsample:
            y = conv2d_q_raw(h, bank.w_quad(slot, rt2, L.Q_POOL), L.Q_POOL, h.shape[3], rt2.rows, pf, 0, bias=b2,
                             x2=x, w2q_ptr=bank.w_quad(slot, rt0, 5 if rt0.cin_pad == 8 else 4), bias2=b0, x2_norelu=not same_relu)
        if y is None:
            hh = _conv_fwd(h, rt2, slot, cfg2, b2)
            y = conv2d_raw(x, bank.w_fwd(slot, rt0), x.shape[3], rt0.rows_pad, 1, 1, 1, 0, 0, cfg0.pix_flags(), ef, bias=b0, res=hh, alpha=al)
        ctx.save_for_backward(h, x)
        ctx.rt2, ctx.rt0, ctx.slot, ctx.cfg2, ctx.cfg0 = rt2, rt0, slot, cfg2, cfg0
        ctx.w2, ctx.b2, ctx.w0, ctx.b0 = w2, b2, w0, b0
        return y

    @staticmethod
    def backward(ctx, dy):
        h, x = ctx.saved_tensors
        rt2, rt0, slot, cfg2, cfg0 = ctx.rt2, ctx.rt0, ctx.slot, ctx.cfg2, ctx.cfg0
        if torch.is_grad_enabled():
            if _param_grad_wanted(ctx.w2, ctx.b2, ctx.w0, ctx.b0):
                raise NotImplementedError("create_graph=True is supported for input gradients only (WGAN-GP path)")
            dh = ConvDgradFn.apply(dy, h, ctx.w2, rt2, slot, cfg2) if ctx.needs_input_grad[0] else None
            dx = ConvDgradFn.apply(dy, x, ctx.w0, rt0, slot, cfg0) if ctx.needs_input_grad[1] else None
            return (dh, dx) + (None,) * 10
        dy = _c(dy)
        bank = rt2.bank()
        outs = []
        want2 = ctx.b2 is not None and ctx.needs_input_grad[3]
        want0 = ctx.b0 is not None and ctx.needs_input_grad[5]
        shared_db = None
        if want2 and want0 and ctx.needs_input_grad[2] and ctx.needs_input_grad[4] and rt2.rows_pad == rt2.rows and rt0.rows == rt2.rows:
            shared_db = zeros_small(rt2.rows, torch.float32, dy.device)
        for inp, rt, cfg, w_i, b_i, wp, bp in ((h, rt2, cfg2, 2, 3, ctx.w2, ctx.b2), (x, rt0, cfg0, 4, 5, ctx.w0, ctx.b0)):
            k = 0 if inp is h else 1
            outs.append(_conv_dgrad(dy, inp, rt, slot, cfg) if ctx.needs_input_grad[k] else None)
            want_db = bp is not None and ctx.needs_input_grad[b_i]
            db_done = False
            if ctx.needs_input_grad[w_i]:
                g = ensure_grad(bp) if (want_db and rt.rows_pad == rt.rows) else None
                if k == 0 and shared_db is not None:
                    g = shared_db
                elif k == 1 and shared_db is not None:
                    g = None
                db_done = _conv_wgrad(inp, dy, rt, slot, cfg, dbias=g)
                if k == 0 and shared_db is not None:
                    if db_done:
                        for bq in (ctx.b2, ctx.b0):
                            L.call("sg_axpby", L.F32, L.ptr(shared_db), L.ptr(ensure_grad(bq)), rt2.rows, 1.0, 1.0, L.stream())
                        continue
                    shared_db = None
                elif k == 1 and shared_db is not None:
                    continue
            if want_db and not db_done:
                g = ensure_grad(bp)
                L.call("sg_colsum", L.dt(dy), L.ptr(dy), dy.shape[3], None, 0, dy.shape[0] * dy.shape[1] * dy.shape[2], rt.rows, L.ptr(g), 1.0, L.stream())
        if ctx.link is not None and outs[1] is not None and _GRAD_LINK[0]:
            ctx.link.dx = outs[1]
            outs[1] = None
        return (outs[0], outs[1]) + (None,) * 10


_SKIP_FUSION = [{"0": False, "all": "all"}.get(os.environ.get("SG_SKIP_FUSION", "1"), True)]


class SliceUpFn(torch.autograd.Function):

    @staticmethod
    def forward(ctx, x, C, up, link=None):
        x = _c(x)
        N, Hs, Ws, ld = x.shape
        ctx.dims = (N, Hs, Ws, ld, C, up)
        ctx.link = link
        if C == ld and up == 1:
            return x.view_as(x)
        y = torch.empty((N, Hs * up, Ws * up, C), dtype=x.dtype, device=x.device)
        L.call("sg_slice_up_fwd", L.dt(x), L.ptr(x), L.ptr(y), N, Hs, Ws, ld, C, up, L.stream())
        return y

    @staticmethod
    def backward(ctx, dy):
        N, Hs, Ws, ld, C, up = ctx.dims
        if torch.is_grad_enabled():
            return (dy if (C == ld and up == 1) else SliceUpBwdFn.apply(dy, ctx.dims)), None, None, None
        dy = _c(dy)
        if C == ld and up == 1:
            dx = dy
        else:
            dx = torch.empty((N, Hs, Ws, ld), dtype=dy.dtype, device=dy.device)
            L.call("sg_slice_up_bwd", L.dt(dy), L.ptr(dy), L.ptr(dx), N, Hs, Ws, ld, C, up, L.stream())
        if ctx.link is not None and _GRAD_LINK[0]:
            ctx.link.dx, dx = dx, None
        return dx, None, None, None
# ... 426 lines not shown
        (idx,) = ctx.saved_tensors
        w = ctx.weight
        if ctx.needs_input_grad[0]:
            g = ensure_grad(w)
            dout = _c(dout.float())
            L.call("sg_embedding_bwd", L.ptr(dout), L.ptr(idx), L.ptr(g), idx.numel(), w.shape[1], w.shape[0], L.stream())
        return None, None


class SNEmbeddingFn(torch.autograd.Function):

    @staticmethod
    def forward(ctx, weight, idx, rt, slot):
        bank = rt.bank()
        idx = _c(idx.long())
        B = idx.numel()
        out = torch.empty((B, rt.cols), dtype=torch.float32, device=weight.device)
        L.call("sg_embedding_fwd", bank.w_f32(slot, rt), L.ptr(idx), L.ptr(out), B, rt.cols, rt.rows, L.stream())
        ctx.save_for_backward(idx)
        ctx.rt, ctx.slot = rt, slot
        return out

    @staticmethod
    def backward(ctx, dout):
        _first_order_only("SNEmbeddingFn")
        (idx,) = ctx.saved_tensors
        rt, slot = ctx.rt, ctx.slot
        if ctx.needs_input_grad[0]:
            dout = _c(dout.float())
            L.call("sg_embedding_bwd", L.ptr(dout), L.ptr(idx), rt.bank().dwt(slot, rt), idx.numel(), rt.cols, rt.rows, L.stream())
        return None, None, None, None


__all__ = ['CatConvDgradFn', 'CatConvFn', 'CbnAffineDgradFn', 'CbnAffineFn', 'CbnAffineGroupFn', 'cbn_prefetch', '_CBN_GROUP', 'ConvCfg', 'ConvDgradFn', 'ConvFn', 'ConvSkipFn', 'ConvTransposeFn', 'EmbeddingFn', 'GradLink', 'LinearDgradFn', 'LinearFn', 'SNEmbeddingFn', 'SliceUpBwdFn', 'SliceUpFn', '_GRAD_LINK', '_QUAD', '_SKIP_FUSION', '_conv_dgrad', '_conv_fwd', '_conv_wgrad', '_quad_form']
```

pytorch-studiogan_amd/ops.py:

```python
import torch
import torch.nn as nn
from torch.nn import init
import torch.nn.functional as F_

from . import functional as F
from .bank import get_bank

COMPUTE_DTYPE = torch.float32


def to_nhwc(x, dtype, cpad=0):
    if x.dim() != 4:
        raise RuntimeError("expected a 4-D NCHW tensor")
    if x.dtype == torch.uint8:
        return F.u8_to_nhwc(x, dtype, max(cpad, 3))
    if cpad > x.shape[1]:
        return F.NchwToNhwcFn.apply(x.float(), dtype, cpad)
    if x.dtype == dtype and x.is_contiguous(memory_format=torch.channels_last) and not (x.shape[1] > 1 and x.is_contiguous() and x.shape[2] * x.shape[3] > 1):
        return x.permute(0, 2, 3, 1)
    if x.dtype == torch.float32 and x.is_contiguous():
        return F.NchwToNhwcFn.apply(x, dtype)
    y = x.permute(0, 2, 3, 1).contiguous()
    if y.dtype != dtype:
        y = F.ConvertFn.apply(y, dtype)
# ... 42 lines not shown
            w = self.weight
            del self._parameters["weight"]
            self.register_parameter("weight_orig", w)
            with torch.no_grad():
                mat = w.reshape(rows, cols)
                u = F_.normalize(w.new_empty(rows).normal_(0, 1), dim=0, eps=eps)
                v = F_.normalize(w.new_empty(cols).normal_(0, 1), dim=0, eps=eps)
            self.register_buffer("weight_u", u)
            self.register_buffer("weight_v", v)

    @property
    def master_weight(self):
        return self.weight_orig if self._sg_sn else self.weight

    def __getattr__(self, name):
        if name == "weight" and "weight_orig" in self.__dict__.get("_parameters", {}):
            return self._parameters["weight_orig"].data
        return super().__getattr__(name)


class Conv2d(_WeightLayerMixin, nn.Conv2d):
    def __init__(self, in_channels, out_channels, kernel_size, stride=1, padding=0, dilation=1, groups=1, bias=True, sn=False,
                 cout_pad=0):
        nn.Conv2d.__init__(self, in_channels, out_channels, kernel_size, stride, padding, dilation, groups, bias)
        if self.dilation != (1, 1) or self.groups != 1:
            raise NotImplementedError("dilation/groups are not on the StudioGAN hot path")
        if self.kernel_size[0] != self.kernel_size[1] and self.stride != (1, 1):
            raise NotImplementedError
        kh, kw = self.kernel_size
        self._sg_rows_pad = cout_pad
        self._sg_dgrad_noflip = self.stride[0] != 1
        self._sg_setup("conv", out_channels, in_channels * kh * kw, in_channels, kh * kw, sn)

    def forward_nhwc(self, x, slot=None, in_relu=False, in_upsample=False, out_pool=False, res=None, link=None, stats=False):
        rt = self._sg_rt
        slot = slot if slot is not None else rt.bank().current
        kh, kw = self.kernel_size
        cfg = F.ConvCfg(kh, kw, self.stride[0], self.padding[0], self.padding[1], in_relu, in_upsample, out_pool, stats and self.training)
        return F.ConvFn.apply(x, self.master_weight, self.bias, res, rt, slot, cfg, link)

    def forward(self, x):
        slot = _standalone_slot(self, x)
        _, bank = _root_and_bank(self)
        y = self.forward_nhwc(to_nhwc(x, bank.dtype, getattr(self, "_sg_cin_pad", 0)), slot)
        if self._sg_rows_pad and self._sg_rows_pad != self.out_channels:
            y = y[..., :self.out_channels]
        return to_nchw(y)


def conv_skip_nhwc(conv_main, conv_skip, h, x, slot=None, in_relu=False, out_pool=False, skip_upsample=False, link=None, stats=False, skip_relu=None):
    rt2, rt0 = conv_main._sg_rt, conv_skip._sg_rt
    slot = slot if slot is not None else rt2.bank().current
    cfg2 = F.ConvCfg(3, 3, 1, 1, 1, in_relu, False, out_pool, stats)
    cfg0 = F.ConvCfg(1, 1, 1, 0, 0, in_relu if skip_relu is None else skip_relu, skip_upsample, out_pool)
    return F.ConvSkipFn.apply(h, x, conv_main.master_weight, conv_main.bias, conv_skip.master_weight, conv_skip.bias, rt2, rt0, slot, cfg2, cfg0, link)


class ConvTranspose2d(_WeightLayerMixin, nn.ConvTranspose2d):

    def __init__(self, in_channels, out_channels, kernel_size, stride=2, padding=0, dilation=1, groups=1, bias=True, sn=False):
        nn.ConvTranspose2d.__init__(self, in_channels, out_channels, kernel_size, stride, padding, 0, groups, bias, dilation)
        if self.dilation != (1, 1) or self.groups != 1 or self.output_padding != (0, 0):
            raise NotImplementedError
        kh, kw = self.kernel_size
        self._sg_trans = True
        self._sg_dgrad_noflip = True
        self._sg_setup("conv", out_channels, in_channels * kh * kw, in_channels, kh * kw, sn)

    def forward_nhwc(self, x, slot=None):
        rt = self._sg_rt
        slot = slot if slot is not None else rt.bank().current
        kh, kw = self.kernel_size
        cfg = F.ConvCfg(kh, kw, self.stride[0], self.padding[0], self.padding[1])
        return F.ConvTransposeFn.apply(x, self.master_weight, self.bias, rt, slot, cfg)

    def forward(self, x, output_size=None):
        slot = _standalone_slot(self, x)
        _, bank = _root_and_bank(self)
        return to_nchw(self.forward_nhwc(to_nhwc(x, bank.dtype), slot))


class Linear(_WeightLayerMixin, nn.Linear):
    def __init__(self, in_features, out_features, bias=True, sn=False):
        nn.Linear.__init__(self, in_features, out_features, bias)
        self._sg_setup("linear", out_features, in_features, in_features, 1, sn)

    def forward_rt(self, x, slot=None, const_bias=None):
        rt = self._sg_rt
# ... 259 lines not shown
```

Baseline: 2070.

## Emit ReLU sign bit-planes in discriminator conv epilogues for backward masking

The forward conv epilogues in the discriminator now also write a packed 1-bit-per-element plane recording where each output is positive. The backward dgrad then reads these bits as the ReLU mask instead of re-reading the full bf16 activation. This is meant to cut memory traffic for the ReLU masking in backward. In exchange the forward kernels do extra stores, there are more kernel template variants, and plane lifetimes must be managed across D blocks.

```diff
diff --git a/include/sgamd.h b/include/sgamd.h
--- a/include/sgamd.h
+++ b/include/sgamd.h
@@ -20,6 +20,7 @@
 #define SG_EPI_POOL 4
 #define SG_EPI_RELU 8
 #define SG_EPI_RES_F32 16
+#define SG_EPI_PLANES 32
 
 const char* sg_last_error(void);
 int sg_version(void);
@@ -36,8 +37,11 @@
   const void* x; const void* w;
   const float* bias; const void* res; const void* mask; void* out; const float* alpha_ptr;
   int ldo, ldr, ldm;
+  const void* mask_bits; void* sign_out;
+  int ldmb, lds;
 } sg_conv_fwd_desc;
 int sg_conv2d_fwd(const sg_conv_fwd_desc* d, sg_stream_t stream);
+long long sg_sign_plane_launches(int what);
 int sg_set_f32_mode(int mode);
 int sg_get_f32_mode(void);
 long long sg_f32_split_launches(int mode);
@@ -82,6 +86,8 @@
   int C2, ldx2;
   float* stats;
   int x2_norelu;
+  const void* mask_bits; void* sign_out;
+  int ldmb, lds;
 } sg_convq_desc;
 int sg_conv2d_q_stat_rows(const sg_convq_desc* d);
 int sg_conv2d_q(const sg_convq_desc* d, sg_stream_t stream);
diff --git a/pytorch-studiogan_amd/_lib.py b/pytorch-studiogan_amd/_lib.py
--- a/pytorch-studiogan_amd/_lib.py
+++ b/pytorch-studiogan_amd/_lib.py
@@ -14,7 +14,7 @@
 F32, BF16, F64 = 0, 1, 2
 PIX_RELU, PIX_UPSAMPLE, PIX_QUAD, PIX_TRANSPOSED = 1, 2, 4, 8
 Q_POOL, Q_UP = 0, 1
-EPI_OUT_F32, EPI_ATOMIC, EPI_POOL, EPI_RELU, EPI_RES_F32 = 1, 2, 4, 8, 16
+EPI_OUT_F32, EPI_ATOMIC, EPI_POOL, EPI_RELU, EPI_RES_F32, EPI_PLANES = 1, 2, 4, 8, 16, 32
 
 _vp, _i, _f, _ll = C.c_void_p, C.c_int, C.c_float, C.c_longlong
 
@@ -23,7 +23,8 @@
     _fields_ = [("dtype", _i), ("N", _i), ("Hs", _i), ("Ws", _i), ("C", _i), ("ldx", _i), ("Ho", _i), ("Wo", _i), ("Cout", _i),
                 ("R", _i), ("S", _i), ("stride", _i), ("pad_h", _i), ("pad_w", _i), ("pix_flags", _i), ("epi_flags", _i),
                 ("alpha", _f), ("beta", _f), ("x", _vp), ("w", _vp), ("bias", _vp), ("res", _vp), ("mask", _vp), ("out", _vp),
-                ("alpha_ptr", _vp), ("ldo", _i), ("ldr", _i), ("ldm", _i)]
+                ("alpha_ptr", _vp), ("ldo", _i), ("ldr", _i), ("ldm", _i),
+                ("mask_bits", _vp), ("sign_out", _vp), ("ldmb", _i), ("lds", _i)]
 
 
 class ConvSkipDesc(C.Structure):
@@ -45,7 +46,8 @@
     _fields_ = [("dtype", _i), ("form", _i), ("N", _i), ("Hl", _i), ("Wl", _i), ("C", _i), ("ldx", _i), ("Cout", _i),
                 ("pix_flags", _i), ("epi_flags", _i), ("alpha", _f), ("beta", _f), ("x", _vp), ("wq", _vp), ("bias", _vp), ("res", _vp),
                 ("mask", _vp), ("out", _vp), ("alpha_ptr", _vp), ("ldo", _i), ("ldr", _i), ("ldm", _i),
-                ("x2", _vp), ("w2q", _vp), ("bias2", _vp), ("C2", _i), ("ldx2", _i), ("stats", _vp), ("x2_norelu", _i)]
+                ("x2", _vp), ("w2q", _vp), ("bias2", _vp), ("C2", _i), ("ldx2", _i), ("stats", _vp), ("x2_norelu", _i),
+                ("mask_bits", _vp), ("sign_out", _vp), ("ldmb", _i), ("lds", _i)]
 
 
 class ConvQWgradDesc(C.Structure):
@@ -113,6 +115,7 @@
     "sg_conv2d_fwd_skip": [C.POINTER(ConvSkipDesc), _vp],
     "sg_conv2d_fwd_skip_ok": [C.POINTER(ConvSkipDesc)],
     "sg_conv_rs_launches": [],
+    "sg_sign_plane_launches": [_i],
     "sg_modconv2d_fwd": [C.POINTER(ModConvDesc), _vp],
     "sg_modconv2d_ok": [C.POINTER(ModConvDesc)],
     "sg_modconv_launches": [],
@@ -320,6 +323,7 @@
             fn.argtypes = args
             fn.restype = _i
         l.sg_conv_rs_launches.restype = _ll
+        l.sg_sign_plane_launches.restype = _ll
         l.sg_modconv_launches.restype = _ll
         l.sg_tok_gemm_launches.restype = _ll
         l.sg_mha_launches.restype = _ll
diff --git a/pytorch-studiogan_amd/backbones/big_resnet.py b/pytorch-studiogan_amd/backbones/big_resnet.py
--- a/pytorch-studiogan_amd/backbones/big_resnet.py
+++ b/pytorch-studiogan_amd/backbones/big_resnet.py
@@ -175,19 +175,20 @@
         if self.cpad:
             self.conv2d1._sg_cin_pad = self.conv2d0._sg_cin_pad = self.cpad
 
-    def forward_nhwc(self, x, slot):
-        h = self.conv2d1.forward_nhwc(x, slot)
+    def forward_nhwc(self, x, slot, planes=False, x_plane=None, out_plane=None):
+        hp = F.SignPlane() if (planes and self.apply_d_sn) else None
+        h = self.conv2d1.forward_nhwc(x, slot, out_plane=hp)
         if not self.apply_d_sn:
             h = self.bn1.forward_nhwc(h, relu=True)
             h = self.conv2d2.forward_nhwc(h, slot, out_pool=True)
         else:
             if self.cpad == 8 and h.dtype == torch.bfloat16 and not x.requires_grad:
-                return ops.conv_skip_nhwc(self.conv2d2, self.conv2d0, h, x, slot, in_relu=True, out_pool=True, skip_relu=False)
-            h = self.conv2d2.forward_nhwc(h, slot, in_relu=True, out_pool=True)
+                return ops.conv_skip_nhwc(self.conv2d2, self.conv2d0, h, x, slot, in_relu=True, out_pool=True, skip_relu=False, h_plane=hp, out_plane=out_plane)
+            h = self.conv2d2.forward_nhwc(h, slot, in_relu=True, out_pool=True, x_plane=hp)
         x0 = F.AvgPool2Fn.apply(x)
         if not self.apply_d_sn:
             x0 = self.bn0.forward_nhwc(x0)
-        return self.conv2d0.forward_nhwc(x0, slot, res=h)
+        return self.conv2d0.forward_nhwc(x0, slot, res=h, out_plane=out_plane if self.apply_d_sn else None)
 
 
 class DiscBlock(nn.Module):
@@ -208,14 +209,16 @@
             self.bn2 = MODULES.d_bn(in_features=out_channels)
         self.average_pooling = nn.AvgPool2d(2)
 
-    def forward_nhwc(self, x, slot):
+    def forward_nhwc(self, x, slot, planes=False, x_plane=None, out_plane=None):
         if self.apply_d_sn:
+            hp = F.SignPlane() if planes else None
             if self.downsample or self.ch_mismatch:
                 link = F.GradLink()
-                h = self.conv2d1.forward_nhwc(x, slot, in_relu=True, link=link)
-                return ops.conv_skip_nhwc(self.conv2d2, self.conv2d0, h, x, slot, in_relu=True, out_pool=self.downsample, link=link)
-            h = self.conv2d1.forward_nhwc(x, slot, in_relu=True)
-            h = self.conv2d2.forward_nhwc(h, slot, in_relu=True, out_pool=False)
+                h = self.conv2d1.forward_nhwc(x, slot, in_relu=True, link=link, x_plane=x_plane, out_plane=hp)
+                return ops.conv_skip_nhwc(self.conv2d2, self.conv2d0, h, x, slot, in_relu=True, out_pool=self.downsample, link=link,
+                                          h_plane=hp, x_plane=x_plane, out_plane=out_plane)
+            h = self.conv2d1.forward_nhwc(x, slot, in_relu=True, x_plane=x_plane, out_plane=hp)
+            h = self.conv2d2.forward_nhwc(h, slot, in_relu=True, out_pool=False, x_plane=hp)
             return F.AddReluFn.apply(h, x)
         h = self.bn1.forward_nhwc(x, relu=True)
         h = self.conv2d1.forward_nhwc(h, slot)
@@ -281,12 +284,23 @@
     def forward(self, x, label, eval=False, adc_fake=False):
         dtype = self.compute_dtype
         bank = get_bank(self, dtype)
-        slot = bank.begin_forward(_need_graph(self, x))
+        need_graph = _need_graph(self, x)
+        slot = bank.begin_forward(need_graph)
         h = ops.to_nhwc(x, dtype, self.blocks[0][0].cpad)
         nxt = bank.boundaries(self.blocks) if bank.exchange is not None else None
+        planes = dtype == torch.bfloat16 and need_graph and F.sign_planes_on()
+        flat = [b for bl in self.blocks for b in bl]
+        plane, k = None, 0
         for bi, blocklist in enumerate(self.blocks):
             for block in blocklist:
-                h = block.forward_nhwc(h, slot)
+                if isinstance(block, ops.SelfAttention):
+                    h, plane = block.forward_nhwc(h, slot), None
+                else:
+                    follower = flat[k + 1] if k + 1 < len(flat) else None
+                    out_plane = F.SignPlane() if (planes and isinstance(follower, DiscBlock) and follower.apply_d_sn) else None
+                    h = block.forward_nhwc(h, slot, planes=True, x_plane=plane, out_plane=out_plane) if planes else block.forward_nhwc(h, slot)
+                    plane = out_plane
+                k += 1
             if nxt is not None:
                 h = bank.mark(h, nxt[bi])
             h = ops.block_boundary(self, bi, h)
diff --git a/pytorch-studiogan_amd/csrc/common.h b/pytorch-studiogan_amd/csrc/common.h
--- a/pytorch-studiogan_amd/csrc/common.h
+++ b/pytorch-studiogan_amd/csrc/common.h
@@ -36,6 +36,13 @@
 template <typename T> __device__ __forceinline__ float to_f(T v);
 template <> __device__ __forceinline__ float to_f<float>(float v) { return v; }
 template <> __device__ __forceinline__ float to_f<bf16_t>(bf16_t v) { return bf2f(v); }
+__device__ __forceinline__ bool sg_relu_pos(bf16_t h) { return bf2f(h) > 0.f; }
+__device__ __forceinline__ uint32_t sg_relu_pos8(u32x4 v) {
+  uint32_t b = 0u;
+#pragma unroll
+  for (int e = 0; e < 8; e++) b |= sg_relu_pos((bf16_t)((v[e >> 1] >> (16 * (e & 1))) & 0xffffu)) ? (1u << e) : 0u;
+  return b;
+}
 template <typename T> __device__ __forceinline__ T from_f(float v);
 template <> __device__ __forceinline__ float from_f<float>(float v) { return v; }
 template <> __device__ __forceinline__ bf16_t from_f<bf16_t>(float v) { return f2bf(v); }
diff --git a/pytorch-studiogan_amd/csrc/conv.hip b/pytorch-studiogan_amd/csrc/conv.hip
--- a/pytorch-studiogan_amd/csrc/conv.hip
+++ b/pytorch-studiogan_amd/csrc/conv.hip
@@ -10,6 +10,11 @@
   return 0;
 }
 extern "C" int sg_get_f32_mode() { return g_sg_f32_mode; }
+long long g_sg_sign_plane_launches[3] = {0, 0, 0};
+extern "C" long long sg_sign_plane_launches(int what) {
+  if (what < 0 || what > 2) return -1;
+  return __atomic_load_n(&g_sg_sign_plane_launches[what], __ATOMIC_RELAXED);
+}
 extern "C" long long sg_f32_split_launches(int mode) {
   if (mode != 3 && mode != 6) return -1;
   return __atomic_load_n(&g_sg_f32_split_launches[mode == 6], __ATOMIC_RELAXED);
@@ -117,6 +122,7 @@
     sg_prof_tag(prof, eng, b);
   }
   sg_prof_end(st, prof);
+  if constexpr (std::is_same_v<T, bf16_t>) sg_sign_plane_count(e, eng == SG_ENG_CONV_V4 || (eng == SG_ENG_CONV_V3 && I > 32) || eng == SG_ENG_CONV_V2, eng == SG_ENG_CONV_SK);
   SG_LAUNCH_CHECK();
   return 0;
 }
@@ -140,6 +146,7 @@
     sg_prof_tag(prof, SG_ENG_CONV_V4_SKIP, 2.0 * ((double)d->N * d->Hs * d->Ws * d->C + x2 + (double)I * (K + sk->C2) + jout * I));
   }
   sg_prof_end(st, prof);
+  if (ok) sg_sign_plane_count(pb.e, true);
   return ok ? 1 : 0;
 }
 extern "C" int sg_conv2d_fwd_skip_stat_rows(const sg_conv_skip_desc* d) {
diff --git a/pytorch-studiogan_amd/csrc/conv_common.h b/pytorch-studiogan_amd/csrc/conv_common.h
--- a/pytorch-studiogan_amd/csrc/conv_common.h
+++ b/pytorch-studiogan_amd/csrc/conv_common.h
@@ -1,5 +1,6 @@
 #pragma once
 #include <stdlib.h>
+#include <type_traits>
 #include "gemm_core.h"
 #include "../../include/sgamd.h"
 
@@ -55,8 +56,19 @@
   e.out = d->out; e.out_bstride = 0; e.ldo = d->ldo; e.bias = d->bias;
   e.res = d->res; e.res_bstride = 0; e.ldr = d->ldr; e.beta = d->beta;
   e.mask = (const T*)d->mask; e.mask_bstride = 0; e.ldm = d->ldm; e.split_stride = 0;
-  e.alpha = d->alpha; e.alpha_ptr = d->alpha_ptr; e.flags = d->epi_flags; e.I = I; e.J = J;
+  e.alpha = d->alpha; e.alpha_ptr = d->alpha_ptr; e.flags = d->epi_flags & ~SG_EPI_PLANES; e.I = I; e.J = J;
+  const bool planes = std::is_same_v<T, bf16_t> && (d->epi_flags & SG_EPI_PLANES);
+  const int nw = (I + 31) >> 5;
+  const bool mb = planes && d->mask && d->mask_bits && d->ldmb >= nw && !((uintptr_t)d->mask_bits & 3);
+  const bool so = planes && d->sign_out && d->lds >= nw && !((uintptr_t)d->sign_out & 3);
+  e.mask_bits = mb ? (const uint32_t*)d->mask_bits : nullptr; e.ldmb = mb ? d->ldmb : 0;
+  e.sign_out = so ? (uint32_t*)d->sign_out : nullptr; e.lds = so ? d->lds : 0;
   return e;
+}
+extern long long g_sg_sign_plane_launches[3];
+static inline void sg_sign_plane_count(const Epilogue<bf16_t>& e, bool epilogue_planes, bool writes_only = false) {
+  if (e.sign_out && (epilogue_planes || writes_only)) __atomic_fetch_add(&g_sg_sign_plane_launches[0], 1, __ATOMIC_RELAXED);
+  if (e.mask) __atomic_fetch_add(&g_sg_sign_plane_launches[(e.mask_bits && epilogue_planes) ? 1 : 2], 1, __ATOMIC_RELAXED);
 }
 static inline bool epi_bf16_rows_ok(const Epilogue<bf16_t>& e) {
   if ((e.flags & (SG_EPI_ATOMIC | SG_EPI_OUT_F32)) || (e.ldo & 7) || !aligned16(e.out)) return false;
diff --git a/pytorch-studiogan_amd/csrc/conv_q.hip b/pytorch-studiogan_amd/csrc/conv_q.hip
--- a/pytorch-studiogan_amd/csrc/conv_q.hip
+++ b/pytorch-studiogan_amd/csrc/conv_q.hip
@@ -156,7 +156,7 @@
   if (4 * J >= (1ll << 29)) return false;
   const long long xbytes = bf16_extent(npix_x, d->ldx, d->C), wbytes = (long long)d->Cout * 16 * d->C * 2;
   if (xbytes >= (1ll << 31) || wbytes >= (1ll << 31)) return false;
-  if ((d->epi_flags & ~SG_EPI_RELU) || (d->pix_flags & ~SG_PIX_RELU)) return false;
+  if ((d->epi_flags & ~(SG_EPI_RELU | SG_EPI_PLANES)) || (d->pix_flags & ~SG_PIX_RELU)) return false;
   e = make_epilogue<bf16_t>(d, d->Cout, (int)J);
   if (!epi_bf16_rows_ok(e)) return false;
   NB = cout_blocks(d->Cout);
@@ -220,6 +220,7 @@
                 2.0 * (jin * d->C + (d->x2 ? 4.0 * J * d->C2 + (double)d->Cout * d->C2 : 0.0) + 16.0 * d->C * d->Cout + jout * d->Cout * (1.0 + (d->mask ? 1.0 : 0.0) + (d->res ? 1.0 : 0.0))));
   }
   sg_prof_end(st, prof);
+  if (rc == 0) sg_sign_plane_count(e, true);
   SG_CHECK(rc == 0, "sg_conv2d_q: launch failed");
   SG_LAUNCH_CHECK();
   return 0;
diff --git a/pytorch-studiogan_amd/csrc/conv_sk.h b/pytorch-studiogan_amd/csrc/conv_sk.h
--- a/pytorch-studiogan_amd/csrc/conv_sk.h
+++ b/pytorch-studiogan_amd/csrc/conv_sk.h
@@ -10,10 +10,11 @@
   int I, J, K;
   unsigned xbytes;
   unsigned obytes, sbytes;
+  unsigned pbytes;
   int nrb;
 };
 
-template <int TI, int NP, int TJ, int KS, int NW, bool POOL>
+template <int TI, int NP, int TJ, int KS, int NW, bool POOL, bool PLANE = false>
 __global__ __launch_bounds__(64 * NW) void sg_conv_sk_kernel(ConvSkParams p, Epilogue<bf16_t> epi) {
   constexpr int BI = TI * NP * 32;
   constexpr int NCH = 2 * KS;
@@ -42,6 +43,15 @@
   const auto rso = __builtin_amdgcn_make_buffer_rsrc(epi.out, 0, (int)p.obytes, 0x00020000);
   const auto rss = __builtin_amdgcn_make_buffer_rsrc((void*)(epi.mask ? (const void*)epi.mask : epi.res), 0, (int)p.sbytes, 0x00020000);
   constexpr int NIT = ((POOL ? ROWS / 4 : ROWS) * CPR + 63) / 64;
+  const auto rsp = __builtin_amdgcn_make_buffer_rsrc((void*)(PLANE ? epi.sign_out : nullptr), 0, PLANE ? (int)p.pbytes : 0, 0x00020000);
+  constexpr int NITP = ((POOL ? ROWS / 4 : ROWS) * TI + 63) / 64;
+  auto plane_store = [&](uint32_t w, unsigned off) {
+#if __has_builtin(__builtin_amdgcn_raw_buffer_store_b32)
+    __builtin_amdgcn_raw_buffer_store_b32(w, rsp, (int)off, 0, 0);
+#else
+    if (off < p.pbytes) *(uint32_t*)((char*)epi.sign_out + off) = w;
+#endif
+  };
   const int frow = lane & 31, fhi = lane >> 5;
   const unsigned ldx2 = 2u * (unsigned)p.ldx;
   const bool up = (p.flags & SG_PIX_UPSAMPLE) != 0, quad = (p.flags & SG_PIX_QUAD) != 0;
@@ -229,6 +239,24 @@
         const u32x4 v = *(const u32x4*)(stg + rr * CP + c * 16);
         __builtin_amdgcn_raw_buffer_store_b128(v, rso, (int)off, 0, 0);
       }
+#pragma unroll
+      for (int it = 0; it < (PLANE ? NITP : 0); it++) {
+        const int idx = lane + 64 * it;
+        const int r = idx / TI, k = idx - r * TI;
+        const int jg = jbase + r;
+        const bool ok = idx < rows_out * TI && jg < Jout && 4 * k < ncp;
+        const int rr = idx < rows_out * TI ? r : 0;
+        uint32_t w = 0u;
+#pragma unroll 1
+        for (int c = 0; c < 4; c++) {
+          const uint32_t b = sg_relu_pos8(*(const u32x4*)(stg + rr * CP + (4 * k + c) * 16));
+          w |= (4 * k + c < ncp) ? b << (8 * c) : 0u;
+        }
+        const int left = epi.I - (i0 + ic0 + 32 * k);
+        w = (left > 0 && left < 32) ? (w & ((1u << left) - 1u)) : w;
+        const unsigned off = ok ? ((unsigned)jg * (unsigned)epi.lds + (unsigned)((i0 + ic0) >> 5) + (unsigned)k) * 4u : 0x80000000u;
+        plane_store(w, off);
+      }
     }
   };
 
@@ -238,9 +266,14 @@
   if (rb >= p.nrb) return;
   fetch(rb, qa);
 #pragma unroll
-  for (int it = 0; it < NP * NIT; it++) {
-    const u32x4 z = {0u, 0u, 0u, 0u};
-    __builtin_amdgcn_raw_buffer_store_b128(z, rso, (int)(0x80000000u + 16u * it), 0, 0);
+  for (int it = 0; it < NP; it++) {
+#pragma unroll
+    for (int k = 0; k < NIT; k++) {
+      const u32x4 z = {0u, 0u, 0u, 0u};
+      __builtin_amdgcn_raw_buffer_store_b128(z, rso, (int)(0x80000000u + 16u * (it * NIT + k)), 0, 0);
+    }
+#pragma unroll
+    for (int k = 0; k < (PLANE ? NITP : 0); k++) plane_store(0u, 0x80000000u + 4u * (unsigned)(it * NITP + k));
   }
   while (true) {
     fetch(rb + stride, qb);
@@ -254,7 +287,7 @@
   }
 }
 
-template <int TI, int NP, int TJ, int KS, bool POOL>
+template <int TI, int NP, int TJ, int KS, bool POOL, bool PLANE>
 static inline int sg_launch_conv_sk_tp(ConvSkParams p, const Epilogue<bf16_t>& e, hipStream_t st) {
   constexpr int BI = TI * NP * 32, WP = KS * 32 + 16, CP = TI * 64 + 16, ROWS = 32 * TJ;
   constexpr int lds4 = BI * WP + BI * 4 + 4 * ROWS * CP;
@@ -263,7 +296,7 @@
   static_assert(lds <= 160 * 1024, "LDS");
   static bool attr_done = false;
   if (!attr_done) {
-    if (hipFuncSetAttribute((const void*)sg_conv_sk_kernel<TI, NP, TJ, KS, NW, POOL>, hipFuncAttributeMaxDynamicSharedMemorySize, lds) != hipSuccess) return -1;
+    if (hipFuncSetAttribute((const void*)sg_conv_sk_kernel<TI, NP, TJ, KS, NW, POOL, PLANE>, hipFuncAttributeMaxDynamicSharedMemorySize, lds) != hipSuccess) return -1;
     attr_done = true;
   }
   p.nrb = (p.J + ROWS - 1) / ROWS;
@@ -271,12 +304,13 @@
   int gx = (p.nrb + NW - 1) / NW;
   const int cap = (256 * (8 / NW) + tilesI - 1) / tilesI;
   if (gx > cap) gx = cap;
-  hipLaunchKernelGGL((sg_conv_sk_kernel<TI, NP, TJ, KS, NW, POOL>), dim3(gx, tilesI), dim3(64 * NW), lds, st, p, e);
+  hipLaunchKernelGGL((sg_conv_sk_kernel<TI, NP, TJ, KS, NW, POOL, PLANE>), dim3(gx, tilesI), dim3(64 * NW), lds, st, p, e);
   return 0;
 }
 template <int TI, int NP, int TJ, int KS>
 static inline int sg_launch_conv_sk_t(const ConvSkParams& p, const Epilogue<bf16_t>& e, hipStream_t st) {
-  return (e.flags & SG_EPI_POOL) ? sg_launch_conv_sk_tp<TI, NP, TJ, KS, true>(p, e, st) : sg_launch_conv_sk_tp<TI, NP, TJ, KS, false>(p, e, st);
+  if (e.sign_out) return (e.flags & SG_EPI_POOL) ? sg_launch_conv_sk_tp<TI, NP, TJ, KS, true, true>(p, e, st) : sg_launch_conv_sk_tp<TI, NP, TJ, KS, false, true>(p, e, st);
+  return (e.flags & SG_EPI_POOL) ? sg_launch_conv_sk_tp<TI, NP, TJ, KS, true, false>(p, e, st) : sg_launch_conv_sk_tp<TI, NP, TJ, KS, false, false>(p, e, st);
 }
 
 static inline int sg_launch_conv_sk(const ConvSkParams& p, const Epilogue<bf16_t>& e, hipStream_t st) {
diff --git a/pytorch-studiogan_amd/csrc/conv_sk.hip b/pytorch-studiogan_amd/csrc/conv_sk.hip
--- a/pytorch-studiogan_amd/csrc/conv_sk.hip
+++ b/pytorch-studiogan_amd/csrc/conv_sk.hip
@@ -21,9 +21,10 @@
   const long long jout = (e.flags & SG_EPI_POOL) ? (J >> 2) : J;
   const long long obytes = bf16_extent(jout, e.ldo, I);
   const long long sbytes = e.mask ? bf16_extent(jout, e.ldm, I) : (e.res ? bf16_extent(jout, e.ldr, I) : 16);
-  if (obytes >= (1ll << 31) || sbytes >= (1ll << 31)) return false;
+  const long long pbytes = e.sign_out ? ((jout - 1) * e.lds + ((I + 31) >> 5)) * 4 : 0;
+  if (obytes >= (1ll << 31) || sbytes >= (1ll << 31) || pbytes >= (1ll << 31)) return false;
   ConvSkParams p;
-  p.obytes = (unsigned)obytes; p.sbytes = (unsigned)sbytes;
+  p.obytes = (unsigned)obytes; p.sbytes = (unsigned)sbytes; p.pbytes = (unsigned)pbytes;
   p.x = (const bf16_t*)d->x; p.w = (const bf16_t*)d->w;
   p.C = d->C; p.ldx = d->ldx; p.Hs = d->Hs; p.Ws = d->Ws;
   p.Ho = d->Ho; p.Wo = d->Wo; p.wshift = pb.wshift; p.hshift = pb.hshift;
diff --git a/pytorch-studiogan_amd/csrc/conv_v2.h b/pytorch-studiogan_amd/csrc/conv_v2.h
--- a/pytorch-studiogan_amd/csrc/conv_v2.h
+++ b/pytorch-studiogan_amd/csrc/conv_v2.h
@@ -18,7 +18,7 @@
 typedef __attribute__((address_space(1))) const void* sg_gptr_t;
 typedef __attribute__((address_space(3))) void* sg_lptr_t;
 
-template <int BI, int BJ, int NW, int TI, int TJ, bool VMAP = false, bool NOSTORE = false>
+template <int BI, int BJ, int NW, int TI, int TJ, bool VMAP = false, bool NOSTORE = false, bool PLANES = true>
 __device__ __forceinline__ void sg_conv_epilogue(f32x16 (&acc)[TI][TJ], char* smem, const float* sbias, const Epilogue<bf16_t>& epi,
                                                  int i0, int j0, int wi0, int wj0, float al, int vlog = 0, int vadd = 0,
                                                  float* stats = nullptr, int stats_C = 0, int stats_row = 0) {
@@ -29,7 +29,6 @@
   const int tid = threadIdx.x, lane = tid & 63;
   const bool pool = (epi.flags & SG_EPI_POOL) != 0;
   constexpr int CP = BI * 2 + 16;
-  __syncthreads();
   const int rows_out = pool ? BJ / 4 : BJ;
   const int jbase = pool ? (j0 >> 2) : j0, Jout = pool ? (epi.J >> 2) : epi.J;
   constexpr int CPR = BI / 8;
@@ -48,7 +47,23 @@
   uint32_t mbits[TI * TJ];
 #pragma unroll
   for (int q = 0; q < TI * TJ; q++) mbits[q] = 0u;
-  if (pre_both) {
+  const bool plane = PLANES && pre_mask && epi.mask_bits != nullptr;
+  if (plane) {
+#pragma unroll
+    for (int ta = 0; ta < TI; ta++)
+#pragma unroll
+      for (int tb = 0; tb < TJ; tb++) {
+        const int jl = wj0 + tb * 32 + (lane & 31);
+        const int jg = jbase + (pool ? (jl >> 2) : jl);
+        const int ib = i0 + wi0 + ta * 32;
+        uint32_t w = 0u;
+        if (jg < Jout && ib < epi.I) w = epi.mask_bits[grow(jg) * epi.ldmb + (ib >> 5)];
+        w >>= 4 * (lane >> 5);
+        mbits[ta * TJ + tb] = (w & 0xfu) | ((w >> 4) & 0xf0u) | ((w >> 8) & 0xf00u) | ((w >> 12) & 0xf000u);
+      }
+  }
+  __syncthreads();
+  if (pre_both && !plane) {
     stage_tile(epi.mask, epi.ldm);
     __syncthreads();
 #pragma unroll
@@ -63,15 +78,16 @@
           const int il = wi0 + ta * 32 + 8 * g4 + 4 * (lane >> 5);
           const u32x2 m = *(const u32x2*)(smem + jo * CP + il * 2);
 #pragma unroll
-          for (int e = 0; e < 4; e++) { const bf16_t h = (bf16_t)((m[e >> 1] >> (16 * (e & 1))) & 0xffffu); if (bf2f(h) > 0.f) bits |= 1u << (4 * g4 + e); }
+          for (int e = 0; e < 4; e++) { const bf16_t h = (bf16_t)((m[e >> 1] >> (16 * (e & 1))) & 0xffffu); if (sg_relu_pos(h)) bits |= 1u << (4 * g4 + e); }
         }
         mbits[ta * TJ + tb] = bits;
       }
     __syncthreads();
     stage_tile((const bf16_t*)epi.res, epi.ldr);
     __syncthreads();
-  } else if (pre_mask || pre_res) {
-    stage_tile(pre_mask ? epi.mask : (const bf16_t*)epi.res, pre_mask ? epi.ldm : epi.ldr);
+  } else if ((pre_mask && !plane) || pre_res) {
+    const bool sm = pre_mask && !plane;
+    stage_tile(sm ? epi.mask : (const bf16_t*)epi.res, sm ? epi.ldm : epi.ldr);
     __syncthreads();
   }
   const bool relu_out = (epi.flags & SG_EPI_RELU) != 0;
@@ -99,14 +115,14 @@
 #pragma unroll
             for (int e = 0; e < 4; e++) v[e] += b[e];
           }
-          if (pre_both) {
+          if (pre_both || plane) {
             const uint32_t bits = mbits[ta * TJ + tb] >> (4 * g4);
 #pragma unroll
             for (int e = 0; e < 4; e++) if (!((bits >> e) & 1u)) v[e] = 0.f;
           } else if (pre_mask) {
             const u32x2 m = *(const u32x2*)loc;
 #pragma unroll
-            for (int e = 0; e < 4; e++) { const bf16_t h = (bf16_t)((m[e >> 1] >> (16 * (e & 1))) & 0xffffu); if (!(bf2f(h) > 0.f)) v[e] = 0.f; }
+            for (int e = 0; e < 4; e++) { const bf16_t h = (bf16_t)((m[e >> 1] >> (16 * (e & 1))) & 0xffffu); if (!sg_relu_pos(h)) v[e] = 0.f; }
           }
           if (pre_res) {
             const u32x2 r = *(const u32x2*)loc;
@@ -167,6 +183,22 @@
       } else if (jg < Jout && c < ncr) *(u32x4*)(o + grow(jg) * epi.ldo + i0 + c * 8) = *(const u32x4*)(smem + r * CP + c * 16);
     }
   }
+  if (PLANES && epi.sign_out) {
+    constexpr int NWD = BI / 32;
+    const int nch = epi.I - i0 < BI ? epi.I - i0 : BI;
+    for (int idx = tid; idx < rows_out * NWD; idx += 64 * NW) {
+      const int r = idx / NWD, k = idx - r * NWD;
+      const int jg = jbase + r;
+      if (jg >= Jout || 4 * k >= ncr) continue;
+      uint32_t w = 0u;
+#pragma unroll 1
+      for (int c = 0; c < 4; c++)
+        if (4 * k + c < ncr) w |= sg_relu_pos8(*(const u32x4*)(smem + r * CP + (4 * k + c) * 16)) << (8 * c);
+      const int left = nch - 32 * k;
+      if (left < 32) w &= (1u << left) - 1u;
+      epi.sign_out[grow(jg) * epi.lds + (i0 >> 5) + k] = w;
+    }
+  }
 }
 
 template <int BI, int WJ, int WI, int BJ, int SCHED, bool RELU, bool UP>
diff --git a/pytorch-studiogan_amd/csrc/conv_v3.h b/pytorch-studiogan_amd/csrc/conv_v3.h
--- a/pytorch-studiogan_amd/csrc/conv_v3.h
+++ b/pytorch-studiogan_amd/csrc/conv_v3.h
@@ -224,7 +224,7 @@
 
   float al = epi.alpha;
   if (epi.alpha_ptr) al *= *epi.alpha_ptr;
-  sg_conv_epilogue<BI, BJ, NW, TI, TJ>(acc, smem, sbias, epi, i0, j0, wi0, wj0, al);
+  sg_conv_epilogue<BI, BJ, NW, TI, TJ, false, false, BI != 32>(acc, smem, sbias, epi, i0, j0, wi0, wj0, al);
 }
 
 static inline int sg_conv_v3_lds(int BI, int BJ, int npx, bool pb2, bool w3 = false, int* zero_off = nullptr, int* bias_off = nullptr, int* dump_off = nullptr) {
diff --git a/pytorch-studiogan_amd/csrc/conv_wgrad.hip b/pytorch-studiogan_amd/csrc/conv_wgrad.hip
--- a/pytorch-studiogan_amd/csrc/conv_wgrad.hip
+++ b/pytorch-studiogan_amd/csrc/conv_wgrad.hip
@@ -306,7 +306,7 @@
     two_stage = c.work_floats > 0 && d->work && d->work_floats >= c.work_floats;
     Epilogue<T> e;
     e.out = d->dw; e.out_bstride = 0; e.ldo = I; e.bias = nullptr; e.res = nullptr; e.res_bstride = 0; e.ldr = 0; e.beta = 0.f;
-    e.mask = nullptr; e.mask_bstride = 0; e.ldm = 0; e.alpha = d->alpha; e.alpha_ptr = d->alpha_ptr; e.split_stride = 0;
+    e.mask = nullptr; e.mask_bstride = 0; e.ldm = 0; e.alpha = d->alpha; e.alpha_ptr = d->alpha_ptr; e.split_stride = 0; e.mask_bits = nullptr; e.ldmb = 0; e.sign_out = nullptr; e.lds = 0;
     e.flags = SG_EPI_OUT_F32; e.I = I; e.J = J;
     if (c.splits == 1) { e.res = d->dw; e.ldr = I; e.beta = 1.f; e.flags |= SG_EPI_RES_F32; }
     else if (two_stage) { e.out = d->work; e.split_stride = c.n; }
diff --git a/pytorch-studiogan_amd/csrc/gemm.hip b/pytorch-studiogan_amd/csrc/gemm.hip
--- a/pytorch-studiogan_amd/csrc/gemm.hip
+++ b/pytorch-studiogan_amd/csrc/gemm.hip
@@ -57,7 +57,7 @@
   Epilogue<T> e;
   e.out = d->out; e.out_bstride = d->out_bstride; e.ldo = d->ldo; e.bias = d->bias;
   e.res = d->res; e.res_bstride = d->res_bstride; e.ldr = d->ldr; e.beta = d->beta;
-  e.mask = nullptr; e.mask_bstride = 0; e.ldm = 0; e.split_stride = 0;
+  e.mask = nullptr; e.mask_bstride = 0; e.ldm = 0; e.split_stride = 0; e.mask_bits = nullptr; e.ldmb = 0; e.sign_out = nullptr; e.lds = 0;
   e.alpha = d->alpha; e.alpha_ptr = d->alpha_ptr; e.flags = d->epi_flags; e.I = d->I; e.J = d->J;
   if (d->splits > 1) SG_CHECK(d->epi_flags & SG_EPI_ATOMIC, "sg_gemm: split-K needs the atomic epilogue");
   const int V = ET<T>::VEC;
diff --git a/pytorch-studiogan_amd/csrc/gemm_core.h b/pytorch-studiogan_amd/csrc/gemm_core.h
--- a/pytorch-studiogan_amd/csrc/gemm_core.h
+++ b/pytorch-studiogan_amd/csrc/gemm_core.h
@@ -220,6 +220,7 @@
 #define SG_EPI_POOL 4
 #define SG_EPI_RELU 8
 #define SG_EPI_RES_F32 16
+#define SG_EPI_PLANES 32
 
 template <typename T> struct Epilogue {
   void* out; long long out_bstride; int ldo;
@@ -229,6 +230,8 @@
   float alpha; const float* alpha_ptr;
   int flags; int I; int J;
   long long split_stride;
+  const uint32_t* mask_bits; int ldmb;
+  uint32_t* sign_out; int lds;
 
   __device__ __forceinline__ void set_batch(int b) {
     if (flags & (SG_EPI_OUT_F32 | SG_EPI_ATOMIC)) out = (float*)out + (long long)b * out_bstride;
diff --git a/pytorch-studiogan_amd/functional/_base.py b/pytorch-studiogan_amd/functional/_base.py
--- a/pytorch-studiogan_amd/functional/_base.py
+++ b/pytorch-studiogan_amd/functional/_base.py
@@ -99,6 +99,51 @@
     return ent[3], ent[4]
 
 
+def sign_planes_on():
+    return os.environ.get("SG_SIGN_PLANE", "1") != "0"
+
+
+class SignPlane:
+    __slots__ = ("bits", "ptr", "version", "shape")
+
+    def __init__(self):
+        self.bits = None
+
+    def fill(self, bits, t):
+        self.bits, self.ptr, self.version, self.shape = bits, t.data_ptr(), t._version, tuple(t.shape)
+
+    def bits_for(self, t):
+        if self.bits is None or t.dtype != torch.bfloat16 or self.ptr != t.data_ptr() or self.version != t._version or self.shape != tuple(t.shape):
+            return None
+        return self.bits
+
+
+def plane_like(N, H, W, C, device):
+    return torch.empty((N, H, W, (C + 31) // 32), dtype=torch.int32, device=device)
+
+
+def sign_plane_counts():
+    l = L.lib()
+    return tuple(int(l.sg_sign_plane_launches(k)) for k in range(3))
+
+
+def _plane_args(d, out_plane, out, mask, mask_bits):
+    bits = None
+    if out_plane is not None and out.dtype == torch.bfloat16 and sign_planes_on():
+        bits = plane_like(out.shape[0], out.shape[1], out.shape[2], out.shape[3], out.device)
+        d.sign_out, d.lds = bits.data_ptr(), bits.shape[3]
+        d.epi_flags |= L.EPI_PLANES
+    if mask is not None and mask_bits is not None:
+        d.mask_bits, d.ldmb = mask_bits.data_ptr(), mask_bits.shape[3]
+        d.epi_flags |= L.EPI_PLANES
+    return bits, (L.lib().sg_sign_plane_launches(0) if bits is not None else 0)
+
+
+def _plane_done(out_plane, bits, before, out):
+    if bits is not None and L.lib().sg_sign_plane_launches(0) > before:
+        out_plane.fill(bits, out)
+
+
 class f32_mode:
     MODES = {"exact": 0, "bf16x3": 3, "bf16x6": 6}
 
@@ -118,7 +163,7 @@
 
 
 def conv2d_raw(x, w_ptr, Cin, Cout, R, S, stride=1, pad_h=0, pad_w=0, pix_flags=0, epi_flags=0, bias=None, res=None, mask=None,
-               alpha=1.0, beta=1.0, alpha_ptr=None, out=None, ldx=None, transposed_out_hw=None, out_coff=0, x_coff=0, desc=None):
+               alpha=1.0, beta=1.0, alpha_ptr=None, out=None, ldx=None, transposed_out_hw=None, out_coff=0, x_coff=0, desc=None, mask_bits=None, out_plane=None):
     N, Hs, Ws = x.shape[0], x.shape[1], x.shape[2]
     ldx = x.shape[3] if ldx is None else ldx
     up = 2 if (pix_flags & L.PIX_UPSAMPLE) else 1
@@ -151,11 +196,13 @@
     d.ldm = mask.shape[-1] if mask is not None else 0
     if desc is not None:
         return out
+    bits, before = _plane_args(d, out_plane if out_coff == 0 else None, out, mask, mask_bits)
     L.call("sg_conv2d_fwd", d, L.stream())
+    _plane_done(out_plane, bits, before, out)
     return out
 
 
-def conv2d_skip_raw(x, w_ptr, Cin, Cout, x2, w2_ptr, C2, x2_up=False, pix_flags=0, epi_flags=0, bias=None, bias2=None, alpha=1.0, dry=False, stats=False):
+def conv2d_skip_raw(x, w_ptr, Cin, Cout, x2, w2_ptr, C2, x2_up=False, pix_flags=0, epi_flags=0, bias=None, bias2=None, alpha=1.0, dry=False, stats=False, out_plane=None):
     sk = L.ConvSkipDesc()
     out = conv2d_raw(x, w_ptr, Cin, Cout, 3, 3, 1, 1, 1, pix_flags, epi_flags, bias=bias, alpha=alpha, desc=sk.main)
     sk.x2, sk.w2, sk.bias2 = L.ptr(x2), w2_ptr, L.ptr(bias2)
@@ -164,14 +211,17 @@
         return None
     if dry:
         return out
+    bits, before = _plane_args(sk.main, out_plane, out, None, None)
     if stats and not (epi_flags & L.EPI_POOL):
         rows = L.lib().sg_conv2d_fwd_skip_stat_rows(L.C.byref(sk))
         st = torch.empty((rows, Cout, 2), dtype=torch.float32, device=x.device)
         sk.stats = st.data_ptr()
         L.call("sg_conv2d_fwd_skip", sk, L.stream())
         _offer_stats(out, st, rows, Cout)
+        _plane_done(out_plane, bits, before, out)
         return out
     L.call("sg_conv2d_fwd_skip", sk, L.stream())
+    _plane_done(out_plane, bits, before, out)
     return out
 
 
@@ -210,7 +260,7 @@
 
 
 def conv2d_q_raw(x, wq_ptr, form, Cin, Cout, pix_flags=0, epi_flags=0, bias=None, res=None, mask=None, alpha=1.0, beta=1.0, dry=False,
-                 x2=None, w2q_ptr=None, bias2=None, stats=False, x2_norelu=False):
+                 x2=None, w2q_ptr=None, bias2=None, stats=False, x2_norelu=False, mask_bits=None, out_plane=None):
     N = x.shape[0]
     if form == L.Q_POOL:
         if x.shape[1] % 2 or x.shape[2] % 2:
@@ -242,7 +292,9 @@
             rows = L.lib().sg_conv2d_q_stat_rows(L.C.byref(d))
             st = torch.empty((rows, Cout, 2), dtype=torch.float32, device=x.device)
             d.stats = st.data_ptr()
+        bits, before = _plane_args(d, out_plane, out, mask, mask_bits)
         L.call("sg_conv2d_q", d, L.stream())
+        _plane_done(out_plane, bits, before, out)
         if st is not None:
             _offer_stats(out, st, rows, Cout)
     return out
@@ -306,4 +358,4 @@
     return dx
 
 
-__all__ = ['L', 'zeros_small', 'zeros_like_small', '_BN_FUSED_STATS', '_CBN_MERGED', '_DGRAD_SPLITK', '_SEQ', '_STATS_OFFER', '_c', '_comm', '_first_order_only', '_offer_stats', '_param_grad_wanted', '_take_stats', '_tick', 'conv2d_q_raw', 'conv2d_q_wgrad_raw', 'conv2d_raw', 'conv2d_skip_raw', 'conv2d_wgrad_raw', 'dist', 'ensure_grad', 'f32_mode', 'gemm_dgrad_rows', 'gemm_raw', 'os', 'quad_pack_raw', 'second_order', 'torch']
+__all__ = ['L', 'zeros_small', 'zeros_like_small', 'SignPlane', 'sign_planes_on', 'sign_plane_counts', 'plane_like', '_BN_FUSED_STATS', '_CBN_MERGED', '_DGRAD_SPLITK', '_SEQ', '_STATS_OFFER', '_c', '_comm', '_first_order_only', '_offer_stats', '_param_grad_wanted', '_take_stats', '_tick', 'conv2d_q_raw', 'conv2d_q_wgrad_raw', 'conv2d_raw', 'conv2d_skip_raw', 'conv2d_wgrad_raw', 'dist', 'ensure_grad', 'f32_mode', 'gemm_dgrad_rows', 'gemm_raw', 'os', 'quad_pack_raw', 'second_order', 'torch']
diff --git a/pytorch-studiogan_amd/functional/conv.py b/pytorch-studiogan_amd/functional/conv.py
--- a/pytorch-studiogan_amd/functional/conv.py
+++ b/pytorch-studiogan_amd/functional/conv.py
@@ -54,17 +54,17 @@
     return L.Q_POOL if cfg.out_pool else L.Q_UP
 
 
-def _conv_fwd(x, rt, slot, cfg, bias, res=None, stats=False):
+def _conv_fwd(x, rt, slot, cfg, bias, res=None, stats=False, out_plane=None):
     bank = rt.bank()
     Cin = x.shape[3]
     form = _quad_form(rt, cfg, x)
     if form is not None:
         y = conv2d_q_raw(x, bank.w_quad(slot, rt, form), form, Cin, rt.rows_pad, L.PIX_RELU if cfg.in_relu else 0, 0, bias=bias, res=res,
-                         stats=stats and _BN_FUSED_STATS[0] and rt.rows_pad == rt.rows)
+                         stats=stats and _BN_FUSED_STATS[0] and rt.rows_pad == rt.rows, out_plane=out_plane)
         if y is not None:
             return y
     return conv2d_raw(x, bank.w_fwd(slot, rt), Cin, rt.rows_pad, cfg.R, cfg.S, cfg.stride, cfg.pad_h, cfg.pad_w, cfg.pix_flags(), cfg.epi_flags(),
-                      bias=bias, res=res, alpha=cfg.scale)
+                      bias=bias, res=res, alpha=cfg.scale, out_plane=out_plane)
 
 
 def _conv_wgrad(x, dy, rt, slot, cfg, dbias=None):
@@ -79,11 +79,21 @@
 
 
 def _conv_dgrad(dy, x, rt, slot, cfg, res=None):
+    return _conv_dgrad_bits(dy, x, rt, slot, cfg, res, None)
+
+
+def _dgrad(dy, x, rt, slot, cfg, res=None, x_bits=None):
+    if x_bits is None or not cfg.in_relu:
+        return _conv_dgrad(dy, x, rt, slot, cfg, res=res)
+    return _conv_dgrad_bits(dy, x, rt, slot, cfg, res, x_bits)
+
+
+def _conv_dgrad_bits(dy, x, rt, slot, cfg, res, x_bits):
     bank = rt.bank()
     N, Hs, Ws, Cin = x.shape
     form = _quad_form(rt, cfg, x)
     if form is not None and dy.shape[3] == rt.rows_pad:
-        dx = conv2d_q_raw(dy, bank.w_quad(slot, rt, 2 + form), 1 - form, rt.rows_pad, Cin, 0, 0, mask=x if cfg.in_relu else None, res=res)
+        dx = conv2d_q_raw(dy, bank.w_quad(slot, rt, 2 + form), 1 - form, rt.rows_pad, Cin, 0, 0, mask=x if cfg.in_relu else None, res=res, mask_bits=x_bits)
         if dx is not None:
             return dx
     up = 2 if cfg.in_upsample else 1
@@ -92,11 +102,11 @@
     if cfg.stride != 1:
         assert not (pool or cfg.in_upsample), "upsample / pooling fusion is stride-1 only"
         return conv2d_raw(dy, bank.w_dgrad(slot, rt), rt.rows_pad, Cin, cfg.R, cfg.S, cfg.stride, cfg.pad_h, cfg.pad_w, L.PIX_TRANSPOSED, 0,
-                          mask=x if cfg.in_relu else None, res=res, transposed_out_hw=(Hin, Win), ldx=dy.shape[3])
+                          mask=x if cfg.in_relu else None, res=res, transposed_out_hw=(Hin, Win), ldx=dy.shape[3], mask_bits=x_bits)
     pf = L.PIX_UPSAMPLE if pool else 0
     ef = L.EPI_POOL if cfg.in_upsample else 0
     return conv2d_raw(dy, bank.w_dgrad(slot, rt), rt.rows_pad, Cin, cfg.R, cfg.S, 1, cfg.R - 1 - cfg.pad_h, cfg.S - 1 - cfg.pad_w, pf, ef,
-                      mask=x if cfg.in_relu else None, res=res, alpha=cfg.scale, ldx=dy.shape[3])
+                      mask=x if cfg.in_relu else None, res=res, alpha=cfg.scale, ldx=dy.shape[3], mask_bits=x_bits)
 
 
 class ConvDgradFn(torch.autograd.Function):
@@ -133,9 +143,10 @@
 class ConvFn(torch.autograd.Function):
 
     @staticmethod
-    def forward(ctx, x, weight, bias, res, rt, slot, cfg, link=None):
+    def forward(ctx, x, weight, bias, res, rt, slot, cfg, link=None, x_plane=None, out_plane=None):
         bank = rt.bank()
         x = _c(x)
+        ctx.x_bits = x_plane.bits_for(x) if (x_plane is not None and cfg.in_relu) else None
         N, Hs, Ws, Cin = x.shape
         assert Cin == rt.cin_pad, f"conv input channels {Cin} != {rt.cin_pad}"
         ctx.link = link
@@ -148,7 +159,7 @@
             bias_k = zeros_small(rt.rows_pad, torch.float32, x.device)
             bias_k[:rt.rows].copy_(bias.detach())
         _tick()
-        y = _conv_fwd(x, rt, slot, cfg, bias_k, res, stats=cfg.stats)
+        y = _conv_fwd(x, rt, slot, cfg, bias_k, res, stats=cfg.stats, out_plane=out_plane)
         ctx.save_for_backward(x)
         ctx.rt, ctx.slot, ctx.cfg = rt, slot, cfg
         ctx.bias = bias
@@ -165,12 +176,12 @@
             if _param_grad_wanted(ctx.weight, ctx.bias):
                 raise NotImplementedError("create_graph=True is supported for input gradients only (WGAN-GP path)")
             dx = ConvDgradFn.apply(dy, x, ctx.weight, rt, slot, cfg) if ctx.needs_input_grad[0] else None
-            return dx, None, None, (dy if ctx.has_res else None), None, None, None, None
+            return dx, None, None, (dy if ctx.has_res else None), None, None, None, None, None, None
         dy = _c(dy)
         dx = None
         skip_dx = ctx.link.take() if ctx.link is not None else None
         if ctx.needs_input_grad[0]:
-            dx = _conv_dgrad(dy, x, rt, slot, cfg, res=skip_dx)
+            dx = _dgrad(dy, x, rt, slot, cfg, res=skip_dx, x_bits=ctx.x_bits)
         elif skip_dx is not None:
             raise RuntimeError("GradLink: a skip gradient was handed over but this convolution's input needs no gradient")
         if ctx.link is not None and ctx.link.chain:
@@ -187,16 +198,18 @@
             rows = dy.shape[0] * dy.shape[1] * dy.shape[2]
             L.call("sg_colsum", L.dt(dy), L.ptr(dy), dy.shape[3], None, 0, rows, rt.rows, L.ptr(g), 1.0, L.stream())
         dres = dy if ctx.has_res else None
-        return dx, None, None, dres, None, None, None, None
+        return dx, None, None, dres, None, None, None, None, None, None
 
 
 class ConvSkipFn(torch.autograd.Function):
 
     @staticmethod
-    def forward(ctx, h, x, w2, b2, w0, b0, rt2, rt0, slot, cfg2, cfg0, link=None):
+    def forward(ctx, h, x, w2, b2, w0, b0, rt2, rt0, slot, cfg2, cfg0, link=None, h_plane=None, x_plane=None, out_plane=None):
         bank = rt2.bank()
         ctx.link = link
         h, x = _c(h), _c(x)
+        ctx.h_bits = h_plane.bits_for(h) if (h_plane is not None and cfg2.in_relu) else None
+        ctx.x_bits = x_plane.bits_for(x) if (x_plane is not None and cfg0.in_relu) else None
         _tick()
         assert cfg2.R == 3 and cfg0.R == 1 and cfg2.out_pool == cfg0.out_pool and not cfg2.in_upsample and (cfg0.in_relu == cfg2.in_relu or not cfg0.in_relu)
         pf, ef, al = cfg2.pix_flags(), cfg2.epi_flags(), cfg2.scale
@@ -205,13 +218,13 @@
         plain = rt2.rows_pad == rt2.rows and rt0.rows_pad == rt0.rows and b2 is not None and b0 is not None
         if plain and same_relu and h.dtype == torch.bfloat16 and _SKIP_FUSION[0] and (h.shape[1] >= 16 or _SKIP_FUSION[0] == "all") and _quad_form(rt2, cfg2, h) is None:
             y = conv2d_skip_raw(h, bank.w_fwd(slot, rt2), h.shape[3], rt2.rows, x, bank.w_fwd(slot, rt0), x.shape[3], cfg0.in_upsample, pf, ef,
-                                bias=b2, bias2=b0, alpha=al, stats=cfg2.stats and _BN_FUSED_STATS[0])
+                                bias=b2, bias2=b0, alpha=al, stats=cfg2.stats and _BN_FUSED_STATS[0], out_plane=out_plane)
         if y is None and plain and _quad_form(rt2, cfg2, h) == L.Q_POOL and _SKIP_FUSION[0] and (rt0.cin_pad % 32 == 0 or rt0.cin_pad == 8) and not cfg0.in_upsample:
             y = conv2d_q_raw(h, bank.w_quad(slot, rt2, L.Q_POOL), L.Q_POOL, h.shape[3], rt2.rows, pf, 0, bias=b2,
-                             x2=x, w2q_ptr=bank.w_quad(slot, rt0, 5 if rt0.cin_pad == 8 else 4), bias2=b0, x2_norelu=not same_relu)
+                             x2=x, w2q_ptr=bank.w_quad(slot, rt0, 5 if rt0.cin_pad == 8 else 4), bias2=b0, x2_norelu=not same_relu, out_plane=out_plane)
         if y is None:
             hh = _conv_fwd(h, rt2, slot, cfg2, b2)
-            y = conv2d_raw(x, bank.w_fwd(slot, rt0), x.shape[3], rt0.rows_pad, 1, 1, 1, 0, 0, cfg0.pix_flags(), ef, bias=b0, res=hh, alpha=al)
+            y = conv2d_raw(x, bank.w_fwd(slot, rt0), x.shape[3], rt0.rows_pad, 1, 1, 1, 0, 0, cfg0.pix_flags(), ef, bias=b0, res=hh, alpha=al, out_plane=out_plane)
         ctx.save_for_backward(h, x)
         ctx.rt2, ctx.rt0, ctx.slot, ctx.cfg2, ctx.cfg0 = rt2, rt0, slot, cfg2, cfg0
         ctx.w2, ctx.b2, ctx.w0, ctx.b0 = w2, b2, w0, b0
@@ -226,7 +239,7 @@
                 raise NotImplementedError("create_graph=True is supported for input gradients only (WGAN-GP path)")
             dh = ConvDgradFn.apply(dy, h, ctx.w2, rt2, slot, cfg2) if ctx.needs_input_grad[0] else None
             dx = ConvDgradFn.apply(dy, x, ctx.w0, rt0, slot, cfg0) if ctx.needs_input_grad[1] else None
-            return (dh, dx) + (None,) * 10
+            return (dh, dx) + (None,) * 13
         dy = _c(dy)
         bank = rt2.bank()
         outs = []
@@ -237,7 +250,7 @@
             shared_db = zeros_small(rt2.rows, torch.float32, dy.device)
         for inp, rt, cfg, w_i, b_i, wp, bp in ((h, rt2, cfg2, 2, 3, ctx.w2, ctx.b2), (x, rt0, cfg0, 4, 5, ctx.w0, ctx.b0)):
             k = 0 if inp is h else 1
-            outs.append(_conv_dgrad(dy, inp, rt, slot, cfg) if ctx.needs_input_grad[k] else None)
+            outs.append(_dgrad(dy, inp, rt, slot, cfg, x_bits=ctx.h_bits if k == 0 else ctx.x_bits) if ctx.needs_input_grad[k] else None)
             want_db = bp is not None and ctx.needs_input_grad[b_i]
             db_done = False
             if ctx.needs_input_grad[w_i]:
@@ -261,7 +274,7 @@
         if ctx.link is not None and outs[1] is not None and _GRAD_LINK[0]:
             ctx.link.dx = outs[1]
             outs[1] = None
-        return (outs[0], outs[1]) + (None,) * 10
+        return (outs[0], outs[1]) + (None,) * 13
 
 
 _SKIP_FUSION = [{"0": False, "all": "all"}.get(os.environ.get("SG_SKIP_FUSION", "1"), True)]
@@ -754,4 +767,4 @@
         return None, None, None, None
 
 
-__all__ = ['CatConvDgradFn', 'CatConvFn', 'CbnAffineDgradFn', 'CbnAffineFn', 'CbnAffineGroupFn', 'cbn_prefetch', '_CBN_GROUP', 'ConvCfg', 'ConvDgradFn', 'ConvFn', 'ConvSkipFn', 'ConvTransposeFn', 'EmbeddingFn', 'GradLink', 'LinearDgradFn', 'LinearFn', 'SNEmbeddingFn', 'SliceUpBwdFn', 'SliceUpFn', '_GRAD_LINK', '_QUAD', '_SKIP_FUSION', '_conv_dgrad', '_conv_fwd', '_conv_wgrad', '_quad_form']
+__all__ = ['CatConvDgradFn', 'CatConvFn', 'CbnAffineDgradFn', 'CbnAffineFn', 'CbnAffineGroupFn', 'cbn_prefetch', '_CBN_GROUP', 'ConvCfg', 'ConvDgradFn', 'ConvFn', 'ConvSkipFn', 'ConvTransposeFn', 'EmbeddingFn', 'GradLink', 'LinearDgradFn', 'LinearFn', 'SNEmbeddingFn', 'SliceUpBwdFn', 'SliceUpFn', '_GRAD_LINK', '_QUAD', '_SKIP_FUSION', '_conv_dgrad', '_conv_dgrad_bits', '_dgrad', '_conv_fwd', '_conv_wgrad', '_quad_form']
diff --git a/pytorch-studiogan_amd/ops.py b/pytorch-studiogan_amd/ops.py
--- a/pytorch-studiogan_amd/ops.py
+++ b/pytorch-studiogan_amd/ops.py
@@ -98,12 +98,12 @@
         self._sg_dgrad_noflip = self.stride[0] != 1
         self._sg_setup("conv", out_channels, in_channels * kh * kw, in_channels, kh * kw, sn)
 
-    def forward_nhwc(self, x, slot=None, in_relu=False, in_upsample=False, out_pool=False, res=None, link=None, stats=False):
+    def forward_nhwc(self, x, slot=None, in_relu=False, in_upsample=False, out_pool=False, res=None, link=None, stats=False, x_plane=None, out_plane=None):
         rt = self._sg_rt
         slot = slot if slot is not None else rt.bank().current
         kh, kw = self.kernel_size
         cfg = F.ConvCfg(kh, kw, self.stride[0], self.padding[0], self.padding[1], in_relu, in_upsample, out_pool, stats and self.training)
-        return F.ConvFn.apply(x, self.master_weight, self.bias, res, rt, slot, cfg, link)
+        return F.ConvFn.apply(x, self.master_weight, self.bias, res, rt, slot, cfg, link, x_plane, out_plane)
 
     def forward(self, x):
         slot = _standalone_slot(self, x)
@@ -114,12 +114,13 @@
         return to_nchw(y)
 
 
-def conv_skip_nhwc(conv_main, conv_skip, h, x, slot=None, in_relu=False, out_pool=False, skip_upsample=False, link=None, stats=False, skip_relu=None):
+def conv_skip_nhwc(conv_main, conv_skip, h, x, slot=None, in_relu=False, out_pool=False, skip_upsample=False, link=None, stats=False, skip_relu=None,
+                   h_plane=None, x_plane=None, out_plane=None):
     rt2, rt0 = conv_main._sg_rt, conv_skip._sg_rt
     slot = slot if slot is not None else rt2.bank().current
     cfg2 = F.ConvCfg(3, 3, 1, 1, 1, in_relu, False, out_pool, stats)
     cfg0 = F.ConvCfg(1, 1, 1, 0, 0, in_relu if skip_relu is None else skip_relu, skip_upsample, out_pool)
-    return F.ConvSkipFn.apply(h, x, conv_main.master_weight, conv_main.bias, conv_skip.master_weight, conv_skip.bias, rt2, rt0, slot, cfg2, cfg0, link)
+    return F.ConvSkipFn.apply(h, x, conv_main.master_weight, conv_main.bias, conv_skip.master_weight, conv_skip.bias, rt2, rt0, slot, cfg2, cfg0, link, h_plane, x_plane, out_plane)
 
 
 class ConvTranspose2d(_WeightLayerMixin, nn.ConvTranspose2d):
```

Result: faster. 2093, median of 6 (+1.1%).
